# microsoft/SEAL

Hardware: AMD Instinct MI355X
Metric: CKKS multiply+relinearize+rescale ciphertexts/sec @ N=2^16, L=16 (higher is better)
Workload: dtype u64

## Files before the change

include/sealhip.h:

```cpp
#ifndef SEALHIP_H
#define SEALHIP_H

#include <stdbool.h>
#include <stddef.h>
#include <stdint.h>

#ifdef __cplusplus
extern "C" {
#endif

typedef long SHL_HRESULT;
#define SHL_S_OK ((SHL_HRESULT)0L)
#define SHL_S_FALSE ((SHL_HRESULT)1L)
#define SHL_E_POINTER ((SHL_HRESULT)0x80004003L)
#define SHL_E_INVALIDARG ((SHL_HRESULT)0x80070057L)
#define SHL_E_OUTOFMEMORY ((SHL_HRESULT)0x8007000EL)
#define SHL_E_UNEXPECTED ((SHL_HRESULT)0x8000FFFFL)
#define SHL_COR_E_IO ((SHL_HRESULT)0x80131620L)
#define SHL_COR_E_INVALIDOPERATION ((SHL_HRESULT)0x80131509L)
#define SHL_E_INVALID_INDEX ((SHL_HRESULT)0x80070585L)

#define SHL_FUNC SHL_HRESULT


// ... 217 lines not shown
SHL_FUNC Evaluator_ModReduceToNext(void *thisptr, void *encrypted, void *destination, void *pool);
SHL_FUNC Evaluator_ModReduceTo(void *thisptr, void *encrypted, uint64_t *parms_id, void *destination, void *pool);
SHL_FUNC Evaluator_TransformToNTT2(void *thisptr, void *encrypted, void *destination_ntt);
SHL_FUNC Evaluator_TransformFromNTT(void *thisptr, void *encrypted_ntt, void *destination);
SHL_FUNC Evaluator_ApplyGalois(void *thisptr, void *encrypted, uint32_t galois_elt, void *galoisKeys, void *destination, void *pool);
SHL_FUNC Evaluator_RotateRows(void *thisptr, void *encrypted, int steps, void *galoisKeys, void *destination, void *pool);
SHL_FUNC Evaluator_RotateColumns(void *thisptr, void *encrypted, void *galois_keys, void *destination, void *pool);
SHL_FUNC Evaluator_RotateVector(void *thisptr, void *encrypted, int steps, void *galoisKeys, void *destination, void *pool);
SHL_FUNC Evaluator_ComplexConjugate(void *thisptr, void *encrypted, void *galoisKeys, void *destination, void *pool);
SHL_FUNC Evaluator_ContextUsingKeyswitching(void *thisptr, bool *using_keyswitching);

SHL_FUNC Evaluator_SwitchKeyAccWords(void *thisptr, void *encrypted, uint64_t *words);
SHL_FUNC Evaluator_RelinearizePartial(void *thisptr, void *encrypted , void *relinKeys, uint64_t digit_first,
                                      uint64_t digit_count, uint64_t *device_acc);
SHL_FUNC Evaluator_RelinearizeFinish(void *thisptr, void *encrypted, uint64_t *device_acc, uint64_t parts);
SHL_FUNC Evaluator_ApplyGaloisPartial(void *thisptr, void *encrypted , uint32_t galois_elt, void *galoisKeys,
                                      uint64_t digit_first, uint64_t digit_count, uint64_t *device_acc);
SHL_FUNC Evaluator_ApplyGaloisFinish(void *thisptr, void *encrypted, uint64_t *device_acc, uint64_t parts);

SHL_FUNC Comm_GetUniqueId(uint8_t *id128);
SHL_FUNC Comm_RcclAvailable(bool *available);
SHL_FUNC Comm_Create(const uint8_t *id128, int nranks, int rank, void **comm);
SHL_FUNC Comm_Destroy(void *comm);
SHL_FUNC Comm_Info(void *comm, int *nranks, int *rank, bool *loopback);
SHL_FUNC Comm_DigitRange(void *comm, uint64_t digits, uint64_t *first, uint64_t *count);
SHL_FUNC Comm_AllReduceWords(void *comm, uint64_t *device_words, uint64_t count, void *hip_stream);
SHL_FUNC Comm_BroadcastWords(void *comm, uint64_t *device_words, uint64_t count, int root, void *hip_stream);
SHL_FUNC Evaluator_RelinearizeDigitParallel(void *thisptr, void *encrypted, void *relinKeys, void *comm, int exchange, void *destination);
SHL_FUNC Evaluator_ApplyGaloisDigitParallel(void *thisptr, void *encrypted, uint32_t galois_elt, void *galoisKeys, void *comm, int exchange,
                                            void *destination);
SHL_FUNC Evaluator_RotateVectorDigitParallel(void *thisptr, void *encrypted, int steps, void *galoisKeys, void *comm, int exchange,
                                             void *destination);
SHL_FUNC Evaluator_BroadcastKeyDigits(void *thisptr, void *kswitch_keys, uint64_t index, uint64_t *device_staging, void *comm, int root);
SHL_FUNC Evaluator_SwitchKeySlots(void *thisptr, void *encrypted, uint64_t nranks, uint64_t *slots);
SHL_FUNC Evaluator_SwitchKeyPackTargets(void *thisptr, void *encrypted, const uint64_t *device_acc, uint64_t nranks, uint64_t *device_send,
                                        uint64_t *device_special);
SHL_FUNC Evaluator_SwitchKeyFinishOwned(void *thisptr, void *encrypted, const uint64_t *device_recv, const uint64_t *device_special,
                                        uint64_t nranks, uint64_t rank, uint64_t *device_own);
SHL_FUNC Evaluator_SwitchKeyAddGathered(void *thisptr, void *encrypted, const uint64_t *device_all, uint64_t nranks);


SHL_FUNC shl_ntt_forward(void *context, uint64_t *data, uint64_t polys, uint64_t comps, uint64_t first_prime, int lazy, void *stream);
SHL_FUNC shl_ntt_inverse(void *context, uint64_t *data, uint64_t polys, uint64_t comps, uint64_t first_prime, int lazy, void *stream);
SHL_FUNC shl_dyadic_product(void *context, const uint64_t *a, const uint64_t *b, uint64_t *r, uint64_t polys, uint64_t comps, uint64_t first_prime, void *stream);
SHL_FUNC shl_reduce_items(void *context, uint64_t chain_index, const uint64_t *a, const uint64_t *plain, uint64_t *r, uint64_t size,
                          uint64_t batch, uint64_t group, uint64_t slices, uint64_t *scratch, uint64_t *slices_used, void *stream);
SHL_FUNC shl_reduce_flush_intervals(uint64_t *sum_terms, uint64_t *dot_terms);
SHL_FUNC shl_dot_items(void *context, uint64_t chain_index, const uint64_t *x, const uint64_t *y, uint64_t *r, uint64_t batch,
                       uint64_t group, uint64_t slices, uint64_t *scratch, uint64_t *slices_used, void *stream);
SHL_FUNC shl_dot_items_flush_interval(uint64_t *items);
SHL_FUNC shl_reduce_mapped(void *context, uint64_t chain_index, int kind, const uint64_t *a, uint64_t a_batch, const uint64_t *b,
                           uint64_t b_batch, uint64_t *r, uint64_t size, void *item_map, uint64_t slices, uint64_t *scratch,
                           uint64_t *slices_used, void *stream);
SHL_FUNC shl_dot_scalars(void *context, uint64_t chain_index, const uint64_t *a, const uint64_t *scalars, uint64_t *r, uint64_t size,
                         uint64_t rows, uint64_t batch, uint64_t slices, uint64_t *slices_used);
SHL_FUNC shl_dot_scalars_tile(void *context, uint64_t chain_index, const uint64_t *a, const uint64_t *scalars, uint64_t *r, uint64_t size,
                              uint64_t rows, uint64_t batch, uint64_t slices, uint64_t *slices_used, uint64_t row_tile, void *stream);
SHL_FUNC shl_dot_scalars_info(uint64_t *row_tile, uint64_t *flush);
SHL_FUNC shl_matmul_items(void *context, uint64_t chain_index, const uint64_t *x, const uint64_t *y, uint64_t *r, uint64_t rows, uint64_t inner,
                          uint64_t cols, int y_transposed, uint64_t slices, uint64_t *slices_used);
SHL_FUNC shl_matmul_items_tile(void *context, uint64_t chain_index, const uint64_t *x, const uint64_t *y, uint64_t *r, uint64_t rows,
                               uint64_t inner, uint64_t cols, int y_transposed, uint64_t slices, uint64_t *slices_used, uint64_t tile,
                               void *stream);
SHL_FUNC shl_matmul_items_info(uint64_t *tile_rows, uint64_t *tile_cols, uint64_t *flush);
SHL_FUNC shl_matmul_plain_items(void *context, uint64_t chain_index, const uint64_t *pl, const uint64_t *a, uint64_t *r, uint64_t size,
                                uint64_t rows, uint64_t inner, uint64_t cols, uint64_t flags, uint64_t slices, uint64_t *slices_used);
SHL_FUNC shl_matmul_plain_items_tile(void *context, uint64_t chain_index, const uint64_t *pl, const uint64_t *a, uint64_t *r, uint64_t size,
                                     uint64_t rows, uint64_t inner, uint64_t cols, uint64_t flags, uint64_t slices, uint64_t *slices_used,
                                     uint64_t tile, void *stream);
SHL_FUNC shl_matmul_plain_items_info(uint64_t *tile_rows, uint64_t *tile_cols, uint64_t *flush);
SHL_FUNC shl_matmul_scalars(void *context, uint64_t chain_index, const void *weights, const uint64_t *a, uint64_t *r, uint64_t size,
                            uint64_t rows, uint64_t inner, uint64_t cols, uint64_t flags, uint64_t slices, uint64_t *slices_used);
SHL_FUNC shl_matmul_scalars_tile(void *context, uint64_t chain_index, const void *weights, const uint64_t *a, uint64_t *r, uint64_t size,
                                 uint64_t rows, uint64_t inner, uint64_t cols, uint64_t flags, uint64_t slices, uint64_t *slices_used,
                                 uint64_t row_tile, void *stream);
SHL_FUNC shl_matmul_scalars_info(uint64_t *row_tile, uint64_t *narrow_row_tile, uint64_t *flush, uint64_t *narrow_flush);
SHL_FUNC shl_apply_galois(void *context, uint64_t chain_index, int ntt_form, uint32_t galois_elt, const uint64_t *in, uint64_t *out, uint64_t polys, void *stream);
SHL_FUNC shl_rns_stage(void *context, uint64_t chain_index, int which, const uint64_t *in, uint64_t *out, uint64_t polys, void *stream);
SHL_FUNC Ciphertext_Create4(void *context, uint64_t *parms_id, void *pool, void **cipher);
SHL_FUNC Ciphertext_Create5(void *context, uint64_t *parms_id, uint64_t capacity, void *pool, void **cipher);
SHL_FUNC Ciphertext_Reserve1(void *thisptr, void *context, uint64_t *parms_id, uint64_t size_capacity);
SHL_FUNC Ciphertext_Reserve2(void *thisptr, void *context, uint64_t size_capacity);
SHL_FUNC Ciphertext_Reserve3(void *thisptr, uint64_t size_capacity);
SHL_FUNC Ciphertext_SizeCapacity(void *thisptr, uint64_t *size_capacity);
SHL_FUNC Ciphertext_SetParmsId(void *thisptr, uint64_t *parms_id);
SHL_FUNC Ciphertext_Resize2(void *thisptr, void *context, uint64_t size);
SHL_FUNC Ciphertext_Resize3(void *thisptr, uint64_t size);
SHL_FUNC Ciphertext_Resize4(void *thisptr, uint64_t size, uint64_t polyModulusDegree, uint64_t coeffModCount);
SHL_FUNC Ciphertext_GetDataAt1(void *thisptr, uint64_t index, uint64_t *data);
SHL_FUNC Ciphertext_GetDataAt2(void *thisptr, uint64_t poly_index, uint64_t coeff_index, uint64_t *data);
SHL_FUNC Ciphertext_SetDataAt(void *thisptr, uint64_t index, uint64_t value);
SHL_FUNC Ciphertext_Release(void *thisptr);
SHL_FUNC KSwitchKeys_Create2(void *copy, void **kswitch_keys);
SHL_FUNC KSwitchKeys_Set(void *thisptr, void *assign);
SHL_FUNC KSwitchKeys_RawSize(void *thisptr, uint64_t *key_count);
SHL_FUNC KSwitchKeys_GetKeyList(void *thisptr, uint64_t index, uint64_t *count, void **key_list);
SHL_FUNC KSwitchKeys_ClearDataAndReserve(void *thisptr, uint64_t size);
SHL_FUNC KSwitchKeys_AddKeyList(void *thisptr, uint64_t count, void **key_list);
SHL_FUNC KSwitchKeys_GetParmsId(void *thisptr, uint64_t *parms_id);
SHL_FUNC KSwitchKeys_SetParmsId(void *thisptr, uint64_t *parms_id);
SHL_FUNC SEALContext_ParametersSet(void *thisptr, bool *params_set);
SHL_FUNC SEALContext_ParameterErrorName(void *thisptr, char *outstr, uint64_t *length);
SHL_FUNC SEALContext_ParameterErrorMessage(void *thisptr, char *outstr, uint64_t *length);
SHL_FUNC SEALContext_KeyContextData(void *thisptr, void **context_data);
SHL_FUNC SEALContext_FirstContextData(void *thisptr, void **context_data);
SHL_FUNC SEALContext_LastContextData(void *thisptr, void **context_data);
SHL_FUNC SEALContext_GetContextData(void *thisptr, uint64_t *parms_id, void **context_data);
SHL_FUNC ContextData_Destroy(void *thisptr);
SHL_FUNC ContextData_TotalCoeffModulus(void *thisptr, uint64_t *count, uint64_t *total_coeff_modulus);
SHL_FUNC ContextData_TotalCoeffModulusBitCount(void *thisptr, int *bit_count);
SHL_FUNC ContextData_Parms(void *thisptr, void **parms);
SHL_FUNC ContextData_Qualifiers(void *thisptr, void **epq);
SHL_FUNC ContextData_CoeffDivPlainModulus(void *thisptr, uint64_t *count, uint64_t *coeff_div);
SHL_FUNC ContextData_PlainUpperHalfThreshold(void *thisptr, uint64_t *puht);
SHL_FUNC ContextData_PlainUpperHalfIncrement(void *thisptr, uint64_t *count, uint64_t *puhi);
SHL_FUNC ContextData_UpperHalfThreshold(void *thisptr, uint64_t *count, uint64_t *uht);
SHL_FUNC ContextData_UpperHalfIncrement(void *thisptr, uint64_t *count, uint64_t *uhi);
SHL_FUNC ContextData_PrevContextData(void *thisptr, void **prev_data);
SHL_FUNC ContextData_NextContextData(void *thisptr, void **next_data);
SHL_FUNC ContextData_ChainIndex(void *thisptr, uint64_t *index);
SHL_FUNC ContextData_ParmsId(void *thisptr, uint64_t *parms_id);
SHL_FUNC EPQ_Destroy(void *thisptr);
SHL_FUNC EPQ_ParametersSet(void *thisptr, bool *parameters_set);
SHL_FUNC EPQ_UsingFFT(void *thisptr, bool *using_fft);
SHL_FUNC EPQ_UsingNTT(void *thisptr, bool *using_ntt);
SHL_FUNC EPQ_UsingBatching(void *thisptr, bool *using_batching);
SHL_FUNC EPQ_UsingFastPlainLift(void *thisptr, bool *using_fast_plain_lift);
SHL_FUNC EPQ_UsingDescendingModulusChain(void *thisptr, bool *using_descending_modulus_chain);
SHL_FUNC EPQ_SecLevel(void *thisptr, int *sec_level);
SHL_FUNC EncParams_Create2(void *copy, void **enc_params);
SHL_FUNC EncParams_Set(void *thisptr, void *assign);
SHL_FUNC EncParams_GetParmsId(void *thisptr, uint64_t *parms_id);
SHL_FUNC EncParams_GetPlainModulus(void *thisptr, uint64_t *plain_modulus);
SHL_FUNC EncParams_Equals(void *thisptr, void *otherptr, bool *result);
SHL_FUNC EncParams_SaveSize(void *thisptr, uint8_t compr_mode, int64_t *result);
SHL_FUNC EncParams_Save(void *thisptr, uint8_t *outptr, uint64_t size, uint8_t compr_mode, int64_t *out_bytes);
SHL_FUNC EncParams_Load(void *thisptr, uint8_t *inptr, uint64_t size, int64_t *in_bytes);
SHL_FUNC SecretKey_Create2(void *copy, void **secret_key);
SHL_FUNC SecretKey_Assign(void *thisptr, void *assign);
SHL_FUNC SecretKey_ParmsId(void *thisptr, uint64_t *parms_id);
SHL_FUNC SecretKey_SaveSize(void *thisptr, uint8_t compr_mode, int64_t *result);
SHL_FUNC SecretKey_Save(void *thisptr, uint8_t *outptr, uint64_t size, uint8_t compr_mode, int64_t *out_bytes);
SHL_FUNC PublicKey_Create2(void *copy, void **public_key);
SHL_FUNC PublicKey_Assign(void *thisptr, void *assign);
SHL_FUNC PublicKey_ParmsId(void *thisptr, uint64_t *parms_id);
SHL_FUNC PublicKey_SaveSize(void *thisptr, uint8_t compr_mode, int64_t *result);
SHL_FUNC PublicKey_Save(void *thisptr, uint8_t *outptr, uint64_t size, uint8_t compr_mode, int64_t *out_bytes);
SHL_FUNC SealHip_ReleasePool(void);
SHL_FUNC SealHip_SetStagedHostCopies(bool enabled);
SHL_FUNC SealHip_PoolStats(uint64_t *bytes_held, uint64_t *cross_stream_waits);
SHL_FUNC SealHip_InstallAbortTrace(const char *path);
SHL_FUNC SealHip_KsChunkStats(uint64_t *calls, uint64_t *chunks, uint64_t *scratch_bytes_max);
SHL_FUNC SealHip_TailStats(uint64_t *folded, uint64_t *plain, uint64_t *dropped);
SHL_FUNC SealHip_ProductStats(uint64_t *fused, uint64_t *formed, uint64_t *dropped);
SHL_FUNC SealHip_GaloisStats(uint64_t *gathered, uint64_t *permuted);
SHL_FUNC SealHip_XofStats(uint64_t *polynomials, uint64_t *replaced_words, uint64_t *host_walk_ns, uint64_t *total_ns);
SHL_FUNC shl_device_count(int *count);
SHL_FUNC shl_set_device(int device);
SHL_FUNC shl_stream_create(bool non_blocking, void **hip_stream);
SHL_FUNC shl_stream_destroy(void *hip_stream);
SHL_FUNC shl_malloc(uint64_t bytes, void **device_ptr);
SHL_FUNC shl_free(void *device_ptr);
SHL_FUNC shl_memcpy_h2d(void *device_dst, const void *host_src, uint64_t bytes);
SHL_FUNC KeyGenerator_Create1(void *context, const uint64_t *seed8, void **key_generator);
SHL_FUNC KeyGenerator_Create2(void *context, void *secret_key, const uint64_t *seed8, void **key_generator);
SHL_FUNC KeyGenerator_Destroy(void *thisptr);
SHL_FUNC KeyGenerator_SecretKey(void *thisptr, void *secret_key);
SHL_FUNC KeyGenerator_CreatePublicKey(void *thisptr, void *public_key);
SHL_FUNC KeyGenerator_CreateRelinKeys(void *thisptr, void *relin_keys);
SHL_FUNC KeyGenerator_CreateGaloisKeysFromElts(void *thisptr, uint64_t count, const uint32_t *galois_elts, void *galois_keys);
SHL_FUNC KeyGenerator_CreateGaloisKeysFromSteps(void *thisptr, uint64_t count, const int *steps, void *galois_keys);
SHL_FUNC KeyGenerator_CreateGaloisKeysAll(void *thisptr, void *galois_keys);
SHL_FUNC KeyGenerator_SeededSaveSize(void *thisptr, bool galois, uint64_t key_count, int64_t *result);
SHL_FUNC KeyGenerator_CreateRelinKeysSave(void *thisptr, uint8_t *outptr, uint64_t size, int64_t *out_bytes);
SHL_FUNC KeyGenerator_CreateGaloisKeysFromEltsSave(void *thisptr, uint64_t count, const uint32_t *galois_elts, uint8_t *outptr, uint64_t size,
                                                   int64_t *out_bytes);
SHL_FUNC KeyGenerator_KeyToHost(void *thisptr, uint32_t galois_elt, uint64_t *host_words, uint64_t capacity_words);
SHL_FUNC SecretKey_Get(void *thisptr, uint64_t *host_words);
SHL_FUNC PublicKey_Get(void *thisptr, uint64_t *host_words);
SHL_FUNC shl_memcpy_d2h(void *host_dst, const void *device_src, uint64_t bytes);
SHL_FUNC shl_device_synchronize(void);
SHL_FUNC shl_timer_create(void **timer);
SHL_FUNC shl_timer_destroy(void *timer);
SHL_FUNC shl_timer_start(void *timer, void *stream);
SHL_FUNC shl_timer_stop(void *timer, void *stream, float *milliseconds);

#ifdef __cplusplus
}
#endif
#endif
```

seal_amd/__init__.py:

```python
from .api import (CoeffModulus, PlainModulus, EncryptionParameters, SEALContext, ContextData, Ciphertext, Plaintext, KSwitchKeys,
                  RelinKeys, GaloisKeys, Evaluator, SecretKey, PublicKey, KeyGenerator, Decryptor, Encryptor, BatchEncoder, CKKSEncoder, Graph, ItemMap, DeviceBuffer, HipTimer, ntt_forward, ntt_inverse,
                  dyadic_product, apply_galois, rns_stage, device_synchronize, device_info, release_pool, pool_stats, tail_stats, product_stats, galois_stats, ks_chunk_stats, xof_stats, Stream, Comm, device_count, set_device,
                  set_staged_host_copies, install_abort_trace)
from ._native import SealHipError, InvalidArgument, LogicError, OutOfRange, DeviceError, load

__all__ = [
    "CoeffModulus", "PlainModulus", "EncryptionParameters", "SEALContext", "ContextData", "Ciphertext", "Plaintext", "KSwitchKeys",
    "RelinKeys", "GaloisKeys", "Evaluator", "SecretKey", "PublicKey", "KeyGenerator", "Decryptor", "Encryptor", "BatchEncoder", "CKKSEncoder", "Graph", "ItemMap", "DeviceBuffer", "HipTimer", "ntt_forward", "ntt_inverse",
    "dyadic_product", "apply_galois", "rns_stage", "device_synchronize", "device_info", "release_pool", "pool_stats", "tail_stats", "product_stats", "galois_stats", "ks_chunk_stats", "xof_stats", "Stream", "Comm", "device_count", "set_device", "set_staged_host_copies", "install_abort_trace", "SealHipError",
    "InvalidArgument", "LogicError", "OutOfRange", "DeviceError", "load",
]
```

seal_amd/_native.py:

```python
import ctypes as C
import os

_HERE = os.path.dirname(os.path.abspath(__file__))
DEFAULT_LIB = os.path.join(_HERE, "lib", "libsealhip.so")

S_OK = 0
E_POINTER = 0x80004003
E_INVALIDARG = 0x80070057
E_OUTOFMEMORY = 0x8007000E
E_UNEXPECTED = 0x8000FFFF
COR_E_IO = 0x80131620
COR_E_INVALIDOPERATION = 0x80131509
E_INVALID_INDEX = 0x80070585


class SealHipError(Exception):

    def __init__(self, hr, message):
        super().__init__("%s (HRESULT 0x%08X)" % (message, hr & 0xFFFFFFFF))
        self.hresult = hr & 0xFFFFFFFF
        self.message = message


class InvalidArgument(SealHipError, ValueError):
    pass


class LogicError(SealHipError, RuntimeError):
    pass


class OutOfRange(SealHipError, IndexError):
    pass


class DeviceError(SealHipError, OSError):
    pass


_ERR = {E_INVALIDARG: InvalidArgument, COR_E_INVALIDOPERATION: LogicError, E_INVALID_INDEX: OutOfRange,
        COR_E_IO: DeviceError}

SYMBOLS = """
SealHip_Version SealHip_DeviceInfo SealHip_LastError CoeffModulus_Create1 PlainModulus_Batching
EncParams_Create1 EncParams_Destroy EncParams_SetPolyModulusDegree EncParams_GetPolyModulusDegree
EncParams_SetCoeffModulus EncParams_GetCoeffModulus EncParams_SetPlainModulus2 EncParams_GetScheme
SEALContext_Create SEALContext_Destroy SEALContext_KeyParmsId SEALContext_FirstParmsId SEALContext_LastParmsId
SEALContext_UsingKeyswitching SEALContext_ChainIndex SEALContext_ParmsIdAt SEALContext_CoeffModulusAt
SEALContext_TotalCoeffModulusBitCount SEALContext_SetParmsId SEALContext_NTTRoot SEALContext_BaseBsk
Ciphertext_Create3 Ciphertext_CreateBatch Ciphertext_Create2 Ciphertext_Set Ciphertext_Destroy Ciphertext_Resize1
Ciphertext_Size Ciphertext_BatchCount Ciphertext_PolyModulusDegree Ciphertext_CoeffModulusSize Ciphertext_ParmsId
Ciphertext_IsNTTForm Ciphertext_SetIsNTTForm Ciphertext_Scale Ciphertext_SetScale Ciphertext_CorrectionFactor
Ciphertext_SetCorrectionFactor Ciphertext_IsTransparent Ciphertext_DevicePtr Ciphertext_CopyFromHost
Ciphertext_CopyToHost Ciphertext_CopyWordsToHost Ciphertext_CopyFromDevice
Ciphertext_SaveSize Ciphertext_Save Ciphertext_UnsafeLoad Ciphertext_Load Ciphertext_LoadItem Ciphertext_SaveItem
KSwitchKeys_UnsafeLoad KSwitchKeys_Load KSwitchKeys_SaveSize KSwitchKeys_Save
KeyGenerator_Create1 KeyGenerator_Create2 KeyGenerator_Destroy KeyGenerator_SecretKey KeyGenerator_CreatePublicKey
KeyGenerator_CreateRelinKeys KeyGenerator_CreateGaloisKeysFromSteps KeyGenerator_CreateGaloisKeysAll KeyGenerator_CreateGaloisKeysFromElts KeyGenerator_KeyToHost KeyGenerator_SeededSaveSize KeyGenerator_CreateRelinKeysSave KeyGenerator_CreateGaloisKeysFromEltsSave SecretKey_Get PublicKey_Get
SecretKey_Create SecretKey_Destroy SecretKey_Set SecretKey_UnsafeLoad SecretKey_Load Decryptor_Create Decryptor_Destroy
Decryptor_Decrypt Decryptor_InvariantNoiseBudget Decryptor_DecryptBatchWords Decryptor_DecryptBatch
CKKSEncoder_Create CKKSEncoder_Destroy CKKSEncoder_SlotCount CKKSEncoder_Encode1 CKKSEncoder_Encode2 CKKSEncoder_Encode3 CKKSEncoder_Encode4 CKKSEncoder_Encode5 CKKSEncoder_Decode1 CKKSEncoder_Decode2
CKKSEncoder_EncodeDevice CKKSEncoder_DecodeDevice
BatchEncoder_Create BatchEncoder_Destroy BatchEncoder_GetSlotCount BatchEncoder_Encode1 BatchEncoder_Encode2 BatchEncoder_Decode1
BatchEncoder_Decode2 BatchEncoder_EncodeDevice BatchEncoder_DecodeDevice
PublicKey_Create PublicKey_Destroy PublicKey_Set PublicKey_UnsafeLoad PublicKey_Load Encryptor_Encrypt Encryptor_EncryptZero1 Encryptor_EncryptZero2 Encryptor_EncryptZeroSymmetric2
Encryptor_Create Encryptor_Destroy Encryptor_SetSeed Encryptor_EncryptZeroSymmetric1 Encryptor_EncryptSymmetric
Encryptor_SymmetricSaveSize Encryptor_EncryptZeroSymmetricSave Encryptor_EncryptSymmetricSave
Encryptor_EncryptSymmetricDevice Encryptor_EncryptDevice
Plaintext_Create1 Plaintext_Create5 Plaintext_Destroy Plaintext_Set4 Plaintext_SetFromDevice Plaintext_CoeffCount
Plaintext_IsNTTForm Plaintext_GetParmsId Plaintext_SetParmsId Plaintext_Scale Plaintext_SetScale Plaintext_CopyToHost
Plaintext_SaveSize Plaintext_Save Plaintext_UnsafeLoad Plaintext_Load
Evaluator_AddMany Evaluator_AddPlain Evaluator_SubPlain Evaluator_MultiplyMany Evaluator_MultiplyPlain Evaluator_Exponentiate
Evaluator_TransformToNTT1 Evaluator_ModSwitchToNext2 Evaluator_ModSwitchTo2
Evaluator_AddPlainDevice Evaluator_SubPlainDevice Evaluator_MultiplyPlainDevice Evaluator_TransformPlainToNTTDevice
Evaluator_SumItems Evaluator_DotPlainDevice shl_reduce_items shl_reduce_flush_intervals
Evaluator_DotItems shl_dot_items shl_dot_items_flush_interval
ItemMap_Create ItemMap_Destroy ItemMap_Info Evaluator_SumItemsMapped Evaluator_DotPlainMapped Evaluator_DotItemsMapped shl_reduce_mapped
CKKSEncoder_EncodeScalars CKKSEncoder_EncodeIntegerScalars Evaluator_LiftScalars Evaluator_DotScalarsDevice
shl_dot_scalars shl_dot_scalars_tile shl_dot_scalars_info
Evaluator_MatMulItems shl_matmul_items shl_matmul_items_tile shl_matmul_items_info
Evaluator_MatMulPlainItems shl_matmul_plain_items shl_matmul_plain_items_tile shl_matmul_plain_items_info
Evaluator_MatMulScalarsItems shl_matmul_scalars shl_matmul_scalars_tile shl_matmul_scalars_info
KSwitchKeys_Create1 KSwitchKeys_Destroy KSwitchKeys_Size KSwitchKeys_SetKey KSwitchKeys_SetKeyFromDevice
KSwitchKeys_SetKeyDigits KSwitchKeys_HasKey KSwitchKeys_DeviceBytes RelinKeys_GetIndex GaloisKeys_GetIndex GaloisTool_GetEltFromStep
Evaluator_Create Evaluator_Destroy Evaluator_SetStream Evaluator_Synchronize Evaluator_CopyTo Evaluator_SetTransparentCheck
Evaluator_BeginCapture Evaluator_EndCapture Evaluator_LaunchGraph Graph_Destroy
Evaluator_Negate Evaluator_Add Evaluator_Sub Evaluator_Multiply Evaluator_Square Evaluator_Relinearize
Evaluator_ModSwitchToNext1 Evaluator_ModSwitchTo1 Evaluator_RescaleToNext Evaluator_RescaleTo
Evaluator_ModReduceToNext Evaluator_ModReduceTo Evaluator_TransformToNTT2 Evaluator_TransformFromNTT Evaluator_ApplyGalois
Evaluator_RotateRows Evaluator_RotateColumns Evaluator_RotateVector Evaluator_ComplexConjugate
Evaluator_ContextUsingKeyswitching
Evaluator_SwitchKeyAccWords Evaluator_RelinearizePartial Evaluator_RelinearizeFinish Evaluator_ApplyGaloisPartial
Evaluator_ApplyGaloisFinish
Comm_GetUniqueId Comm_RcclAvailable Comm_Create Comm_Destroy Comm_Info Comm_DigitRange Comm_AllReduceWords Comm_BroadcastWords
Evaluator_RelinearizeDigitParallel Evaluator_ApplyGaloisDigitParallel Evaluator_RotateVectorDigitParallel
Evaluator_BroadcastKeyDigits Evaluator_SwitchKeySlots Evaluator_SwitchKeyPackTargets Evaluator_SwitchKeyFinishOwned
Evaluator_SwitchKeyAddGathered
SealHip_ReleasePool SealHip_PoolStats SealHip_TailStats SealHip_ProductStats SealHip_GaloisStats SealHip_XofStats SealHip_KsChunkStats SealHip_SetStagedHostCopies SealHip_InstallAbortTrace shl_stream_create shl_stream_destroy shl_device_count shl_set_device
shl_ntt_forward shl_ntt_inverse shl_dyadic_product shl_apply_galois shl_rns_stage shl_malloc shl_free
shl_memcpy_h2d shl_memcpy_d2h shl_device_synchronize shl_timer_create shl_timer_destroy shl_timer_start
shl_timer_stop
Ciphertext_Create4 Ciphertext_Create5 Ciphertext_GetDataAt1 Ciphertext_GetDataAt2 Ciphertext_Release Ciphertext_Reserve1
Ciphertext_Reserve2 Ciphertext_Reserve3 Ciphertext_Resize2 Ciphertext_Resize3 Ciphertext_Resize4 Ciphertext_SetDataAt
Ciphertext_SetParmsId Ciphertext_SizeCapacity ContextData_ChainIndex ContextData_CoeffDivPlainModulus ContextData_Destroy ContextData_NextContextData
ContextData_Parms ContextData_ParmsId ContextData_PlainUpperHalfIncrement ContextData_PlainUpperHalfThreshold ContextData_PrevContextData ContextData_Qualifiers
ContextData_TotalCoeffModulus ContextData_TotalCoeffModulusBitCount ContextData_UpperHalfIncrement ContextData_UpperHalfThreshold EPQ_Destroy EPQ_ParametersSet
EPQ_SecLevel EPQ_UsingBatching EPQ_UsingDescendingModulusChain EPQ_UsingFFT EPQ_UsingFastPlainLift EPQ_UsingNTT
EncParams_Create2 EncParams_Equals EncParams_GetParmsId EncParams_GetPlainModulus EncParams_Load EncParams_Save
EncParams_SaveSize EncParams_Set KSwitchKeys_AddKeyList KSwitchKeys_ClearDataAndReserve KSwitchKeys_Create2 KSwitchKeys_GetKeyList
KSwitchKeys_GetParmsId KSwitchKeys_RawSize KSwitchKeys_Set KSwitchKeys_SetParmsId PublicKey_Assign PublicKey_Create2
PublicKey_ParmsId PublicKey_Save PublicKey_SaveSize SEALContext_FirstContextData SEALContext_GetContextData SEALContext_KeyContextData
SEALContext_LastContextData SEALContext_ParameterErrorMessage SEALContext_ParameterErrorName SEALContext_ParametersSet SecretKey_Assign SecretKey_Create2
SecretKey_ParmsId SecretKey_Save SecretKey_SaveSize
""".split()

_lib = None
_lib_path = None


def load(path=None):
    global _lib, _lib_path
    want = os.path.abspath(path or DEFAULT_LIB)
    if _lib is not None and _lib_path == want:
        return _lib
    if not os.path.exists(want):
        raise ImportError(
            "seal_amd: %s not found. Build it with `python -c 'import __graft_entry__ as g; g.build()'` "
            "(hipcc --offload-arch=gfx950). There is no CPU fallback." % want)
    lib = C.CDLL(want)
    for name in SYMBOLS:
        getattr(lib, name).restype = C.c_long
    _lib, _lib_path = lib, want
    return lib


def lib():
    return _lib if _lib is not None else load()


def check(hr):
    hr &= 0xFFFFFFFF
    if hr == S_OK:
        return
    n = C.c_uint64(0)
    lib().SealHip_LastError(None, C.byref(n))
    buf = C.create_string_buffer(max(int(n.value), 1))
    lib().SealHip_LastError(buf, C.byref(n))
    cls = _ERR.get(hr, SealHipError)
    if hr == E_OUTOFMEMORY:
        raise MemoryError(buf.value.decode())
    raise cls(hr, buf.value.decode(errors="replace"))
```

seal_amd/api.py:

```python
import ctypes as C
import os

import numpy as np

from . import _native as N

SCHEME = {"none": 0, "bfv": 1, "ckks": 2, "bgv": 3}


def _p(a):
    return a.ctypes.data_as(C.c_void_p)


class CoeffModulus:
    @staticmethod
    def Create(poly_modulus_degree, bit_sizes):
        bits = (C.c_int * len(bit_sizes))(*bit_sizes)
        out = np.zeros(len(bit_sizes), dtype=np.uint64)
        N.check(N.lib().CoeffModulus_Create1(C.c_uint64(poly_modulus_degree), C.c_uint64(len(bit_sizes)), bits, _p(out)))
        return [int(x) for x in out]


class PlainModulus:
    @staticmethod
# ... 1582 lines not shown

    def __del__(self):
        if getattr(self, "_h", None):
            N.lib().Comm_Destroy(self._h)
            self._h = None

    def loopback(self):
        v = C.c_bool()
        N.check(N.lib().Comm_Info(self._h, None, None, C.byref(v)))
        return v.value

    def digit_range(self, digits):
        a, b = C.c_uint64(), C.c_uint64()
        N.check(N.lib().Comm_DigitRange(self._h, C.c_uint64(digits), C.byref(a), C.byref(b)))
        return a.value, b.value

    def all_reduce(self, device_ptr, words, stream=None):
        N.check(N.lib().Comm_AllReduceWords(self._h, C.c_void_p(device_ptr), C.c_uint64(words), C.c_void_p(stream or 0)))

    def broadcast(self, device_ptr, words, root=0, stream=None):
        N.check(N.lib().Comm_BroadcastWords(self._h, C.c_void_p(device_ptr), C.c_uint64(words), C.c_int(root), C.c_void_p(stream or 0)))


class DeviceBuffer:

    def __init__(self, words):
        self.words = int(words)
        self._ptr = C.c_void_p()
        N.check(N.lib().shl_malloc(C.c_uint64(self.words * 8), C.byref(self._ptr)))

    def __del__(self):
        if getattr(self, "_ptr", None) and self._ptr.value:
            N.lib().shl_free(self._ptr)
            self._ptr = None

    @property
    def ptr(self):
        return self._ptr.value

    @staticmethod
    def from_numpy(a):
        a = np.ascontiguousarray(a, dtype=np.uint64)
        b = DeviceBuffer(a.size)
        N.check(N.lib().shl_memcpy_h2d(b._ptr, _p(a), C.c_uint64(a.size * 8)))
        return b

    def to_numpy(self, shape):
        out = np.zeros(shape, dtype=np.uint64)
        N.check(N.lib().shl_memcpy_d2h(_p(out), self._ptr, C.c_uint64(out.size * 8)))
        return out

    @staticmethod
    def from_array(a):
        a = np.ascontiguousarray(a)
        if a.dtype.itemsize not in (8, 16):
            raise TypeError("from_array takes 8-byte or complex128 elements, not %s" % a.dtype)
        b = DeviceBuffer(max(a.nbytes // 8, 1))
        N.check(N.lib().shl_memcpy_h2d(b._ptr, _p(a), C.c_uint64(a.nbytes)))
        return b

    @staticmethod
    def from_int32(a):
        a = np.ascontiguousarray(a, dtype=np.int32)
        b = DeviceBuffer(max((a.size + 1) // 2, 1))
        N.check(N.lib().shl_memcpy_h2d(b._ptr, _p(a), C.c_uint64(a.nbytes)))
        return b

    def to_array(self, shape, dtype=np.float64):
        out = np.zeros(shape, dtype=dtype)
        N.check(N.lib().shl_memcpy_d2h(_p(out), self._ptr, C.c_uint64(out.nbytes)))
        return out


def ntt_forward(context, buf, polys, comps, first_prime=0, lazy=False, stream=None):
    N.check(N.lib().shl_ntt_forward(context._h, C.c_void_p(buf.ptr), C.c_uint64(polys), C.c_uint64(comps),
                                    C.c_uint64(first_prime), C.c_int(int(lazy)), C.c_void_p(stream or 0)))


def ntt_inverse(context, buf, polys, comps, first_prime=0, lazy=False, stream=None):
    N.check(N.lib().shl_ntt_inverse(context._h, C.c_void_p(buf.ptr), C.c_uint64(polys), C.c_uint64(comps),
                                    C.c_uint64(first_prime), C.c_int(int(lazy)), C.c_void_p(stream or 0)))


def dyadic_product(context, a, b, r, polys, comps, first_prime=0, stream=None):
    N.check(N.lib().shl_dyadic_product(context._h, C.c_void_p(a.ptr), C.c_void_p(b.ptr), C.c_void_p(r.ptr),
                                       C.c_uint64(polys), C.c_uint64(comps), C.c_uint64(first_prime),
                                       C.c_void_p(stream or 0)))


def apply_galois(context, chain_index, ntt_form, galois_elt, src, dst, polys, stream=None):
    N.check(N.lib().shl_apply_galois(context._h, C.c_uint64(chain_index), C.c_int(int(ntt_form)), C.c_uint32(galois_elt),
                                     C.c_void_p(src.ptr), C.c_void_p(dst.ptr), C.c_uint64(polys), C.c_void_p(stream or 0)))


RNS_STAGE = {"fastbconv_m_tilde": 0, "sm_mrq": 1, "fast_floor": 2, "fastbconv_sk": 3,
             "divide_and_round_q_last": 4, "divide_and_round_q_last_ntt": 5}


def rns_stage(context, chain_index, which, src, dst, polys, stream=None):
    N.check(N.lib().shl_rns_stage(context._h, C.c_uint64(chain_index), C.c_int(RNS_STAGE[which]), C.c_void_p(src.ptr),
                                  C.c_void_p(dst.ptr), C.c_uint64(polys), C.c_void_p(stream or 0)))


class Stream:

    def __init__(self, non_blocking=True):
        self._h = C.c_void_p()
        N.check(N.lib().shl_stream_create(C.c_bool(non_blocking), C.byref(self._h)))

    @property
    def handle(self):
        return self._h.value

    def __del__(self):
        if getattr(self, "_h", None) and self._h.value:
            N.lib().shl_stream_destroy(self._h)
            self._h = None


def device_count():
    n = C.c_int()
    N.check(N.lib().shl_device_count(C.byref(n)))
    return n.value


def set_device(index):
    N.check(N.lib().shl_set_device(C.c_int(index)))


def release_pool():
    N.check(N.lib().SealHip_ReleasePool())


def set_staged_host_copies(enabled):
    N.check(N.lib().SealHip_SetStagedHostCopies(C.c_bool(enabled)))


def install_abort_trace(path):
    N.check(N.lib().SealHip_InstallAbortTrace(C.c_char_p(os.fsencode(path))))


def pool_stats():
    a, b = C.c_uint64(), C.c_uint64()
    N.check(N.lib().SealHip_PoolStats(C.byref(a), C.byref(b)))
    return a.value, b.value


def tail_stats():
    a, b, c = C.c_uint64(), C.c_uint64(), C.c_uint64()
    N.check(N.lib().SealHip_TailStats(C.byref(a), C.byref(b), C.byref(c)))
    return a.value, b.value, c.value


def product_stats():
    a, b, c = C.c_uint64(), C.c_uint64(), C.c_uint64()
    N.check(N.lib().SealHip_ProductStats(C.byref(a), C.byref(b), C.byref(c)))
    return a.value, b.value, c.value


def galois_stats():
    a, b = C.c_uint64(), C.c_uint64()
    N.check(N.lib().SealHip_GaloisStats(C.byref(a), C.byref(b)))
    return a.value, b.value


def xof_stats():
    v = [C.c_uint64() for _ in range(4)]
    N.check(N.lib().SealHip_XofStats(*[C.byref(x) for x in v]))
    return tuple(x.value for x in v)


def ks_chunk_stats():
    a, b, c = C.c_uint64(), C.c_uint64(), C.c_uint64()
    N.check(N.lib().SealHip_KsChunkStats(C.byref(a), C.byref(b), C.byref(c)))
    return a.value, b.value, c.value


def device_synchronize():
    N.check(N.lib().shl_device_synchronize())


def device_info():
    name = C.create_string_buffer(256)
    cus = C.c_int()
    mem = C.c_uint64()
    N.check(N.lib().SealHip_DeviceInfo(name, C.c_uint64(256), C.byref(cus), C.byref(mem)))
    return name.value.decode(), cus.value, mem.value


class HipTimer:

    def __init__(self):
        self._h = C.c_void_p()
        N.check(N.lib().shl_timer_create(C.byref(self._h)))

    def __del__(self):
        if getattr(self, "_h", None):
            N.lib().shl_timer_destroy(self._h)
            self._h = None

    def start(self, stream=None):
        N.check(N.lib().shl_timer_start(self._h, C.c_void_p(stream or 0)))

    def stop(self, stream=None):
        ms = C.c_float()
        N.check(N.lib().shl_timer_stop(self._h, C.c_void_p(stream or 0), C.byref(ms)))
        return ms.value
```

seal_amd/csrc/capi_kernels.cpp:

```cpp
#include "capi_common.h"
#include "batch_reduce_kernels.h"
#include <memory>

namespace
{
    template <class Launch>
    SHL_HRESULT raw_reduce(void *context, uint64_t chain_index, const char *shape_error, uint64_t grid_planes, uint64_t out_items,
                           const ItemWalk &walk, uint64_t slices, uint64_t *slices_used, const uint64_t *r, bool operands,
                           const uint64_t *scratch, Launch launch)
    {
        IfNullRet(context, SHL_E_POINTER);
        SHL_TRY
        auto c = as<Context>(context);
        auto l = c->level_by_chain_index(chain_index);
        if (!l)
            throw std::out_of_range("chain_index");
        if (shape_error)
            throw std::invalid_argument(shape_error);
        const size_t words = (size_t)l->K * c->n();
        if (!slices)
            slices = batch_reduce_slices(grid_planes * out_items * words / 2, walk);
        if (slices > walk.longest || slices > 64)
            throw std::invalid_argument("1 <= slices <= min(group or longest row, 64)");
        if (slices_used)
// ... 374 lines not shown
    }
    SHL_FUNC shl_apply_galois(
        void *context, uint64_t chain_index, int ntt_form, uint32_t galois_elt, const uint64_t *in, uint64_t *out, uint64_t polys,
        void *stream)
    {
        IfNullRet(context, SHL_E_POINTER);
        IfNullRet(in, SHL_E_POINTER);
        IfNullRet(out, SHL_E_POINTER);
        SHL_TRY
        auto c = as<Context>(context);
        auto l = c->level_by_chain_index(chain_index);
        if (!l)
            throw std::out_of_range("chain_index");
        if (!(galois_elt & 1) || galois_elt >= 2 * c->n())
            throw std::invalid_argument("Galois element is not valid");
        if (in == out)
            throw std::invalid_argument("result cannot point to the same value as operand");
        PlaneGeom g{ (unsigned)c->log_n(), l->K, (unsigned)polys };
        hip_ok(k_apply_galois(c->dev_mods(), in, out, galois_elt, ntt_form, g, 1, (hipStream_t)stream), "apply_galois");
        SHL_CATCH
    }
    SHL_FUNC shl_rns_stage(void *context, uint64_t chain_index, int which, const uint64_t *in, uint64_t *out, uint64_t polys, void *stream)
    {
        IfNullRet(context, SHL_E_POINTER);
        IfNullRet(in, SHL_E_POINTER);
        IfNullRet(out, SHL_E_POINTER);
        SHL_TRY
        auto c = as<Context>(context);
        auto l = c->level_by_chain_index(chain_index);
        if (!l)
            throw std::out_of_range("chain_index");
        hipStream_t s = (hipStream_t)stream;
        const unsigned n_log = (unsigned)c->log_n();
        if (which >= 0 && which <= 3)
        {
            if (c->scheme() != Scheme::bfv)
                throw std::logic_error("BEHZ stages exist only for BFV contexts");
            hip_ok(k_behz_stage(c->dev_mods(), l->dev, which, in, out, n_log, polys, s), "behz stage");
        }
        else if (which == 4)
        {
            if (l->K < 2)
                throw std::invalid_argument("level has a single modulus");
            hip_ok(k_bfv_modswitch(c->dev_mods(), l->dev, in, out, n_log, polys, s), "divide_and_round_q_last");
        }
        else if (which == 5)
        {
            if (l->K < 2)
                throw std::invalid_argument("level has a single modulus");
            const unsigned K = l->K;
            const size_t N = c->n();
            Scratch copy(polys * K * N), tt(polys * (K - 1) * N);
            hip_ok(hipMemcpyAsync(copy.p, in, polys * K * N * 8, hipMemcpyDeviceToDevice, s), "copy");
            uint64_t *last = copy.p + (size_t)(K - 1) * N;
            NttBatch bi{};
            bi.data = last;
            bi.outer_stride = (size_t)K * N;
            bi.ncomp = 1;
            bi.nouter = (unsigned)polys;
            bi.prime_first = K - 1;
            hip_ok(ntt_inverse(c->ntt_tables(), bi, 0, s), "intt last");
            NttBatch b{};
            b.data = tt.p;
            b.outer_stride = (size_t)(K - 1) * N;
            b.ncomp = K - 1;
            b.nouter = (unsigned)polys;
            b.src = last;
            b.src_outer_stride = (size_t)K * N;
            b.src_ncomp = 1;
            b.src_mode = 2;
            b.src_half = l->dev.half_q_last;
            b.src_q = l->dev.q_last;
            b.src_fix = l->dev.round_fix;
            hip_ok(ntt_forward(c->ntt_tables(), b, 1, s), "ntt correction");
            hip_ok(k_rescale_combine(c->dev_mods(), l->dev.inv_q_last_mod_q, copy.p, tt.p, out, n_log, K, polys, s), "combine");
            hip_ok(hipStreamSynchronize(s), "sync");
        }
        else
            throw std::invalid_argument("unknown stage");
        SHL_CATCH
    }
    SHL_FUNC SealHip_SetStagedHostCopies(bool enabled)
    {
        set_staged_host_copies(enabled);
        return SHL_S_OK;
    }
    SHL_FUNC SealHip_ReleasePool(void)
    {
        SHL_TRY
        DevicePool::global().release_all();
        SHL_CATCH
    }
    SHL_FUNC SealHip_PoolStats(uint64_t *bytes_held, uint64_t *cross_stream_waits)
    {
        SHL_TRY
        if (bytes_held)
            *bytes_held = DevicePool::global().bytes_held();
        if (cross_stream_waits)
            *cross_stream_waits = DevicePool::global().cross_stream_waits();
        SHL_CATCH
    }
    SHL_FUNC SealHip_KsChunkStats(uint64_t *calls, uint64_t *chunks, uint64_t *scratch_bytes_max)
    {
        SHL_TRY
        uint64_t w = 0;
        ks_chunk_stats(calls, chunks, &w);
        if (scratch_bytes_max)
            *scratch_bytes_max = w * 8;
        SHL_CATCH
    }
    SHL_FUNC SealHip_XofStats(uint64_t *polynomials, uint64_t *replaced_words, uint64_t *host_walk_ns, uint64_t *total_ns)
    {
        SHL_TRY
        xof_stats(polynomials, replaced_words, host_walk_ns, total_ns);
        SHL_CATCH
    }
    SHL_FUNC SealHip_ProductStats(uint64_t *fused, uint64_t *formed, uint64_t *dropped)
    {
        SHL_TRY
        uint64_t f, p, d;
        lazy_product_stats(f, p, d);
        if (fused)
            *fused = f;
        if (formed)
            *formed = p;
        if (dropped)
            *dropped = d;
        SHL_CATCH
    }
    SHL_FUNC SealHip_GaloisStats(uint64_t *gathered, uint64_t *permuted)
    {
        SHL_TRY
        uint64_t g, p;
        galois_path_stats(g, p);
        if (gathered)
            *gathered = g;
        if (permuted)
            *permuted = p;
        SHL_CATCH
    }
    SHL_FUNC SealHip_TailStats(uint64_t *folded, uint64_t *plain, uint64_t *dropped)
    {
        SHL_TRY
        uint64_t f, p, d;
        lazy_tail_stats(f, p, d);
        if (folded)
            *folded = f;
        if (plain)
            *plain = p;
        if (dropped)
            *dropped = d;
        SHL_CATCH
    }
    SHL_FUNC shl_device_count(int *count)
    {
        IfNullRet(count, SHL_E_POINTER);
        SHL_TRY
        *count = 0;
        if (hipGetDeviceCount(count) != hipSuccess)
            *count = 0;
        SHL_CATCH
    }
    SHL_FUNC shl_set_device(int device)
    {
        SHL_TRY
        hip_ok(hipSetDevice(device), "hipSetDevice");
        SHL_CATCH
    }
    SHL_FUNC shl_stream_create(bool non_blocking, void **hip_stream)
    {
        IfNullRet(hip_stream, SHL_E_POINTER);
        SHL_TRY
        hipStream_t s = nullptr;
        hip_ok(hipStreamCreateWithFlags(&s, non_blocking ? hipStreamNonBlocking : hipStreamDefault), "hipStreamCreateWithFlags");
        *hip_stream = s;
        SHL_CATCH
    }
    SHL_FUNC shl_stream_destroy(void *hip_stream)
    {
        SHL_TRY
        hip_ok(hipStreamSynchronize((hipStream_t)hip_stream), "hipStreamSynchronize");
        hip_ok(hipStreamDestroy((hipStream_t)hip_stream), "hipStreamDestroy");
        SHL_CATCH
    }
    SHL_FUNC shl_malloc(uint64_t bytes, void **device_ptr)
    {
        IfNullRet(device_ptr, SHL_E_POINTER);
        SHL_TRY
        if (hipMalloc(device_ptr, bytes) != hipSuccess)
            throw std::bad_alloc();
        SHL_CATCH
    }
    SHL_FUNC shl_free(void *device_ptr)
    {
        SHL_TRY
        hip_ok(hipFree(device_ptr), "hipFree");
        SHL_CATCH
    }
    SHL_FUNC shl_memcpy_h2d(void *device_dst, const void *host_src, uint64_t bytes)
    {
        SHL_TRY
        hip_ok(hipMemcpy(device_dst, host_src, bytes, hipMemcpyHostToDevice), "H2D");
        SHL_CATCH
    }
    SHL_FUNC shl_memcpy_d2h(void *host_dst, const void *device_src, uint64_t bytes)
    {
        SHL_TRY
        hip_ok(hipDeviceSynchronize(), "sync");
        hip_ok(hipMemcpy(host_dst, device_src, bytes, hipMemcpyDeviceToHost), "D2H");
        SHL_CATCH
    }
    SHL_FUNC shl_device_synchronize(void)
    {
        SHL_TRY
        hip_ok(hipDeviceSynchronize(), "hipDeviceSynchronize");
        SHL_CATCH
    }
    SHL_FUNC shl_timer_create(void **timer)
    {
        IfNullRet(timer, SHL_E_POINTER);
        SHL_TRY
        auto t = new Timer();
        hip_ok(hipEventCreate(&t->e0), "hipEventCreate");
        hip_ok(hipEventCreate(&t->e1), "hipEventCreate");
        *timer = t;
        SHL_CATCH
    }
    SHL_FUNC shl_timer_destroy(void *timer)
    {
        IfNullRet(timer, SHL_E_POINTER);
        auto t = as<Timer>(timer);
        (void)hipEventDestroy(t->e0);
        (void)hipEventDestroy(t->e1);
        delete t;
        return SHL_S_OK;
    }
    SHL_FUNC shl_timer_start(void *timer, void *stream)
    {
        IfNullRet(timer, SHL_E_POINTER);
        SHL_TRY
        hip_ok(hipEventRecord(as<Timer>(timer)->e0, (hipStream_t)stream), "hipEventRecord");
        SHL_CATCH
    }
    SHL_FUNC shl_timer_stop(void *timer, void *stream, float *milliseconds)
    {
        IfNullRet(timer, SHL_E_POINTER);
        IfNullRet(milliseconds, SHL_E_POINTER);
        SHL_TRY
        auto t = as<Timer>(timer);
        hip_ok(hipEventRecord(t->e1, (hipStream_t)stream), "hipEventRecord");
        hip_ok(hipEventSynchronize(t->e1), "hipEventSynchronize");
        hip_ok(hipEventElapsedTime(milliseconds, t->e0, t->e1), "hipEventElapsedTime");
        SHL_CATCH
    }
}
```

seal_amd/csrc/ntt2_device.h:

```cpp
#pragma once
#include "ntt2_kernels.h"
#include <cstdlib>
#include <type_traits>

#ifndef SEALHIP_FP_WAVES_P1
#define SEALHIP_FP_WAVES_P1 4
#endif
#ifndef SEALHIP_FP_WAVES_P2
#define SEALHIP_FP_WAVES_P2 4
#endif

namespace sealhip
{
    namespace
    {
        constexpr int kThreads = 256;
        constexpr unsigned kMaxKeyComps = 64;
#ifndef SEALHIP_KS_NT
#define SEALHIP_KS_NT 31
#endif
#ifndef SEALHIP_PRIO
#define SEALHIP_PRIO 0
#endif
        template <int WHEN>
        __device__ __forceinline__ void prio_phase()
        {
#if defined(__HIP_DEVICE_COMPILE__)
            if constexpr (SEALHIP_PRIO != 0)
                __builtin_amdgcn_s_setprio(SEALHIP_PRIO == WHEN ? 1 : 0);
#endif
        }
        template <int BIT>
        __device__ __forceinline__ uint64_t mid_ld(const uint64_t *p)
        {
#if defined(__HIP_DEVICE_COMPILE__)
            if constexpr ((SEALHIP_KS_NT & BIT) != 0)
                return __builtin_nontemporal_load(p);
#endif
            return *p;
        }
        template <int BIT>
        __device__ __forceinline__ void mid_st(uint64_t *p, uint64_t v)
        {
#if defined(__HIP_DEVICE_COMPILE__)
            if constexpr ((SEALHIP_KS_NT & BIT) != 0)
            {
                __builtin_nontemporal_store(v, p);
                return;
            }
#endif
            *p = v;
        }
        template <int BIT>
        __device__ __forceinline__ void mid_ld2(const uint64_t *p, uint64_t &a, uint64_t &b)
        {
#if defined(__HIP_DEVICE_COMPILE__)
            typedef uint64_t u64x2 __attribute__((ext_vector_type(2)));
            const u64x2 *q = reinterpret_cast<const u64x2 *>(p);
            const u64x2 v = (SEALHIP_KS_NT & BIT) != 0 ? __builtin_nontemporal_load(q) : *q;
            a = v.x;
            b = v.y;
#else
            a = p[0];
            b = p[1];
#endif
        }
        template <int BIT>
        __device__ __forceinline__ void mid_st2(uint64_t *p, uint64_t a, uint64_t b)
        {
#if defined(__HIP_DEVICE_COMPILE__)
            typedef uint64_t u64x2 __attribute__((ext_vector_type(2)));
            u64x2 *q = reinterpret_cast<u64x2 *>(p);
            const u64x2 v = { a, b };
            if constexpr ((SEALHIP_KS_NT & BIT) != 0)
                __builtin_nontemporal_store(v, q);
            else
                *q = v;
#else
            p[0] = a;
            p[1] = b;
#endif
        }
#ifdef SEALHIP_MID_WAVE_MAJOR
        __device__ __forceinline__ unsigned mid_lane(unsigned tid) { return (tid >> 6) * 1024 + (tid & 63); }
        constexpr unsigned kMidRow = 64;
#else
        __device__ __forceinline__ unsigned mid_lane(unsigned tid) { return tid; }
        constexpr unsigned kMidRow = 256;
#endif
        template <int D1>
        struct Geo
        {
            static constexpr int rA = D1 - 4;
            static constexpr int LC = 12 - D1;
            static constexpr int C = 1 << LC;
            static constexpr int CP = C + (C == 16 ? 1 : 0);
            static constexpr int ROWS = 1 << D1;
            static constexpr int TILES = 1 << (D1 - 4);
            static constexpr int n = D1 + 8;
            static constexpr size_t lds1_words = (size_t)ROWS * CP;
        };
        constexpr int kRowWords = 16 * 18;
        constexpr size_t kLds2Words = 16 * kRowWords;

        constexpr unsigned kPackWords = 13, kPackBlock = kPackWords * 16;
#ifndef SEALHIP_PACK_VEC16
#define SEALHIP_PACK_VEC16 1
#endif
        constexpr double kPackMagic = 6755399441055744.0;
        constexpr unsigned kPackLdsRow = 272;
        __device__ __forceinline__ void pack52(const double (&x)[16], uint64_t (&w)[13])
        {
            uint32_t lo[16], hi[16];
#pragma unroll
            for (int r = 0; r < 16; r++)
            {
                const uint64_t b = fp_to_bits(x[r] + kPackMagic);
                lo[r] = (uint32_t)b;
                hi[r] = (uint32_t)(b >> 32) & 0xFFFFFu;
            }
#pragma unroll
            for (int k = 0; k < 8; k++)
                w[k] = (uint64_t)lo[2 * k] | ((uint64_t)lo[2 * k + 1] << 32);
#pragma unroll
            for (int k = 0; k < 4; k++)
            {
                const uint32_t d0 = (hi[4 * k] & 0xFFFFu) | (hi[4 * k + 1] << 16), d1 = (hi[4 * k + 2] & 0xFFFFu) | (hi[4 * k + 3] << 16);
                w[8 + k] = (uint64_t)d0 | ((uint64_t)d1 << 32);
            }
            uint32_t t0 = 0, t1 = 0;
#pragma unroll
            for (int r = 0; r < 8; r++)
            {
                t0 |= (hi[r] >> 16) << (4 * r);
                t1 |= (hi[r + 8] >> 16) << (4 * r);
            }
            w[12] = (uint64_t)t0 | ((uint64_t)t1 << 32);
        }
        __device__ __forceinline__ void unpack52(const uint64_t (&w)[13], double (&x)[16])
        {
#pragma unroll
            for (int r = 0; r < 16; r++)
            {
                const uint32_t lo = (uint32_t)(w[r >> 1] >> (32 * (r & 1)));
                const uint32_t mid = (uint32_t)(w[8 + (r >> 2)] >> (16 * (r & 3))) & 0xFFFFu;
                const uint32_t top = (uint32_t)(w[12] >> (4 * r)) & 0xFu;
                const uint64_t b = (uint64_t)lo | ((uint64_t)(0x43300000u | (top << 16) | mid) << 32);
                x[r] = fp_from_bits(b) - kPackMagic;
            }
        }

        __device__ __forceinline__ int int_class(const NttTables &t, unsigned prime)
        {
            const uint64_t q = SHL_UCONST(reinterpret_cast<const uint64_t *>(&t.mods[prime]))[0];
            return (q >> 60) ? 2 : (q >> 58) ? 0 : 1;
        }
        template <class Body>
        __device__ __forceinline__ void with_int_class(const NttTables &t, unsigned prime, Body body)
        {
            const int c = int_class(t, prime);
            if (c == 0)
                body(std::integral_constant<int, 0>());
            else if (c == 1)
                body(std::integral_constant<int, 1>());
            else
                body(std::integral_constant<int, 2>());
        }
#ifndef SEALHIP_XCD_SPREAD
#define SEALHIP_XCD_SPREAD 0
#endif
        struct Blk
        {
            unsigned tile, y, z;
        };
        __device__ __forceinline__ Blk spread_blocks()
        {
#if SEALHIP_XCD_SPREAD
            const unsigned tiles = gridDim.x, slots = gridDim.y * gridDim.z;
            const unsigned L = blockIdx.x + tiles * (blockIdx.y + gridDim.y * blockIdx.z);
            const unsigned group = 8 * tiles, full = (slots / 8) * group;
            unsigned tile, slot;
            if (L < full)
            {
                const unsigned x = L & 7, r = L >> 3;
                tile = r % tiles;
                slot = (r / tiles) * 8 + x;
            }
            else
            {
                tile = L % tiles;
                slot = L / tiles;
            }
            return Blk{ tile, slot % gridDim.y, slot / gridDim.y };
#else
            return Blk{ blockIdx.x, blockIdx.y, blockIdx.z };
#endif
        }

        template <bool FP>
        __device__ __forceinline__ const typename Field<FP>::tw_t *tw_table(const NttTables &t, bool inverse, unsigned prime)
        {
            if constexpr (FP)
                return (inverse ? t.inv_d : t.fwd_d) + ((size_t)prime << t.log_n);
            else
                return (inverse ? t.inv : t.fwd) + ((size_t)prime << t.log_n);
        }

        template <int ICLS>
        __device__ __forceinline__ void int_fix_all(uint64_t (&x)[16], const Field<false>::Mod &m)
        {
#pragma unroll
            for (int a = 0; a < 16; a++)
                Field<false>::fix4<IntBounds<ICLS>::hi32>(x[a], m);
        }

        template <bool FP, int BIT, int ICLS = 0, int B = 4, class TwFn>
        __device__ __forceinline__ void stage_fwd(typename Field<FP>::elem (&x)[16], const typename Field<FP>::Mod &m, TwFn tw)
        {
            if constexpr (!FP)
            {
                if constexpr (IntBounds<ICLS>::fwd_fix_before(B))
                    int_fix_all<ICLS>(x, m);
            }
#pragma unroll
            for (int g = 0; g < (8 >> BIT); g++)
            {
                const auto w = tw(g);
#pragma unroll
                for (int k = 0; k < (1 << BIT); k++)
                {
                    const int e0 = (g << (BIT + 1)) | k;
                    if constexpr (!FP && ICLS == 2)
                        Field<FP>::bfly_fwd_guarded(x[e0], x[e0 | (1 << BIT)], w, m);
                    else
                        Field<FP>::bfly_fwd(x[e0], x[e0 | (1 << BIT)], w, m);
                }
            }
        }

        template <bool FP, int R, int ICLS = 0, int B = 4, class TwFn>
        __device__ __forceinline__ void phase_fwd(typename Field<FP>::elem (&x)[16], const typename Field<FP>::Mod &m, TwFn tw)
        {
            typedef IntBounds<ICLS> IB;
            if constexpr (R >= 1)
                stage_fwd<FP, 3, ICLS, B>(x, m, [&](int g) { return tw(0, g); });
            if constexpr (R >= 2)
                stage_fwd<FP, 2, ICLS, IB::fwd_after(B, 1)>(x, m, [&](int g) { return tw(1, g); });
            if constexpr (R >= 3)
                stage_fwd<FP, 1, ICLS, IB::fwd_after(B, 2)>(x, m, [&](int g) { return tw(2, g); });
            if constexpr (R >= 4)
                stage_fwd<FP, 0, ICLS, IB::fwd_after(B, 3)>(x, m, [&](int g) { return tw(3, g); });
        }

        template <bool FP, int R, bool FIX, int ICLS = 0, int B = 4, class TwFn>
        __device__ __forceinline__ void phase_fwd_end(typename Field<FP>::elem (&x)[16], const typename Field<FP>::Mod &m, TwFn tw)
        {
            phase_fwd<FP, R, ICLS, B>(x, m, tw);
            if constexpr (FP && FIX)
            {
#pragma unroll
                for (int a = 0; a < 16; a++)
                    Field<FP>::fix(x[a], m);
            }
        }
        template <bool FP, int ICLS, int B>
        __device__ __forceinline__ uint64_t fwd_out_lazy(typename Field<FP>::elem x, const typename Field<FP>::Mod &m)
        {
            if constexpr (!FP && B > 4)
                Field<FP>::template fix4<IntBounds<ICLS>::hi32>(x, m);
            return Field<FP>::fwd_to_lazy(x, m);
        }
        template <bool FP, int ICLS, int B>
        __device__ __forceinline__ uint64_t fwd_out_canon(typename Field<FP>::elem x, const typename Field<FP>::Mod &m)
        {
            if constexpr (!FP && ICLS != 2)
                return Field<FP>::template canon_any<IntBounds<ICLS>::hi32>(x, m);
            else
                return Field<FP>::fwd_to_canon(x, m);
        }
        template <int ICLS, int D1>
        constexpr int kP1Out = IntBounds<ICLS>::fwd_after(4, D1);
        template <int ICLS, int D1>
        constexpr int kP2Out = IntBounds<ICLS>::fwd_after(kP1Out<ICLS, D1>, 8);

        template <bool FP, int R, int FIXAT, class TwFn>
        __device__ __forceinline__ void phase_fwd_fix(typename Field<FP>::elem (&x)[16], const typename Field<FP>::Mod &m, TwFn tw)
        {
            static_assert(FP && R == 4 && FIXAT >= 1 && FIXAT <= 3, "a four-stage double-precision phase with the fix inside it");
            stage_fwd<FP, 3>(x, m, [&](int g) { return tw(0, g); });
            if constexpr (FIXAT == 1)
            {
#pragma unroll
                for (int a = 0; a < 16; a++)
                    Field<FP>::fix(x[a], m);
            }
            stage_fwd<FP, 2>(x, m, [&](int g) { return tw(1, g); });
            if constexpr (FIXAT == 2)
            {
#pragma unroll
                for (int a = 0; a < 16; a++)
                    Field<FP>::fix(x[a], m);
            }
// ... 481 lines not shown
```

seal_amd/csrc/ntt2_kernels.h:

```cpp
#pragma once
#include "ntt_kernels.h"

namespace sealhip
{
    bool ntt2_supports(int log_n);

    size_t ntt2_ring_words(const NttTables &t, const NttBatch &b);
    hipError_t ntt2_forward(const NttTables &t, const NttBatch &b, int out_lazy, uint64_t *mid, hipStream_t stream, uint64_t *ring = nullptr, size_t ring_words = 0);

    struct NttRingRun
    {
        uint64_t *data;
        size_t outer_stride;
        const uint32_t *comp_prime;
        unsigned prime_first, ncomp, c0, nc, nouter;
        int lazy;
        unsigned teams_per_comp;
        uint64_t *ring;
        size_t ring_words;
    };
    unsigned ntt2_ring_teams(unsigned nc, unsigned nouter);
    size_t ntt2_ring_run_words(unsigned nc, unsigned teams_per_comp);
    bool ntt2_ring_stream_ok(hipStream_t stream);
    hipError_t ntt2_ring_launch(const NttTables &t, const NttRingRun &run, hipStream_t stream);

    hipError_t ntt2_inverse(const NttTables &t, const NttBatch &b, int out_lazy, uint64_t *mid, hipStream_t stream);

    struct KsFusedArgs
    {
        const uint64_t *t;
        const uint64_t *target_ntt;
        const uint64_t *key;
        uint64_t *mid;
        uint64_t *acc;
        const uint32_t *targets1, *targets2;
        unsigned ntargets, n_int;
        unsigned K, L, batch;
        unsigned j0, j1, key_digit0;
        unsigned parts;
        const uint64_t *fold_c0 = nullptr, *fold_c1 = nullptr;
        const ShoupOp *fold_pm = nullptr;
        const uint64_t *fold_x = nullptr, *fold_y = nullptr;
        size_t fold_plane = 0;
        uint32_t galois_elt = 0;
        int order1 = -1;
        bool no_class_fork = false;
    };
    hipError_t ks_fused(const NttTables &t, const KsFusedArgs &k, hipStream_t stream);

    inline unsigned key_comp_units(const NttTables &t, unsigned comp)
    {
        return t.fp_host && t.fp_host[comp] ? 2u : 4u;
    }
    inline unsigned key_comp_offset_units(const NttTables &t, unsigned comp)
    {
        unsigned u = 0;
        for (unsigned c = 0; c < comp; c++)
            u += key_comp_units(t, c);
        return u;
    }
    inline unsigned key_digit_units(const NttTables &t, unsigned L)
    {
        return key_comp_offset_units(t, L);
    }
    inline size_t key_register_order_words(const NttTables &t, unsigned L, size_t digits)
    {
        return (digits * key_digit_units(t, L)) << t.log_n;
    }
    hipError_t key_to_register_order(const NttTables &t, const uint64_t *in, uint64_t *out, unsigned L, size_t digits, hipStream_t stream);
    hipError_t key_from_register_order(const NttTables &t, const uint64_t *in, uint64_t *out, unsigned L, size_t digits, hipStream_t stream);
}
```

seal_amd/csrc/ntt2_kernels.hip:

```cpp
#include "ntt2_device.h"
#include <algorithm>
#include <atomic>
#include <cstdio>
#include <mutex>
#include <cstdlib>
#include <type_traits>
#include <vector>



namespace sealhip
{
    namespace
    {

        template <bool FP, int D1, int ICLS = 0, bool PACK = false>
        __device__ __forceinline__ void fwd_p1_body(const FwdArgs &a, unsigned prime, unsigned comp, unsigned outer, uint64_t *lds, unsigned tile)
        {
            typedef Field<FP> F;
            typedef Geo<D1> G;
            const unsigned tid = threadIdx.x, cg = tile;
            const typename F::Mod m = F::make_mod(ld_uniform_mod(&a.t.mods[prime]), ld_uniform_fpd(&a.t.fpd[prime]));
            const typename F::tw_t *tab = tw_table<FP>(a.t, false, prime);
            SrcMap sm{ 0, 0, 0, 0 };
// ... 146 lines not shown
                    lds[r * kPackLdsRow + tid] = fp_to_bits(y[r]);
                __syncthreads();
#pragma unroll
                for (int e = 0; e < 16; e++)
                    x[e] = fp_from_bits(lds[(tid >> 4) * kPackLdsRow + e * 16 + (tid & 15)]);
                __syncthreads();
            }
            else
            {
#pragma unroll
            for (int e = 0; e < 16; e++)
                x[e] = F::unraw(nxt[e]);
            prio_phase<2>();
            if (outer + ostride < a.nouter)
                fetch(outer + ostride);
            prio_phase<1>();
            }
            if constexpr (HOIST_LDS)
                p2_tile<FP, D1, false, false, true, true>(x, m, tab, twa, nullptr, lds_wave, hg, tid, &pre_a, &pre_b);
            else if constexpr (HOIST)
                p2_tile<FP, D1, false, false, true>(x, m, tab, nullptr, nullptr, lds_wave, hg, tid, &pre_a, &pre_b);
            else
                p2_tile<FP, D1, false, false, false, false, false, ICLS, kP1Out<ICLS, D1>>(x, m, tab, nullptr, nullptr, lds_wave, hg, tid);
            constexpr int BOUT = kP2Out<ICLS, D1>;
            uint64_t val[16];
            const size_t row0 = ((size_t)comp << G::n) + ((size_t)(hg * 16 + (tid >> 6) * 4) << 8);
            if ((HOIST || HOIST_LDS) || a.epi == 0)
            {
#pragma unroll
                for (int e = 0; e < 16; e++)
                    val[e] = a.lazy ? fwd_out_lazy<FP, ICLS, BOUT>(x[e], m) : fwd_out_canon<FP, ICLS, BOUT>(x[e], m);
                store_rows(val, lds_wave, a.data + (size_t)outer * a.outer_stride + row0, tid);
            }
            else
            {
#pragma unroll
                for (int e = 0; e < 16; e++)
                    val[e] = fwd_out_lazy<FP, ICLS, BOUT>(x[e], m);
                const uint64_t q = a.t.mods[prime].q;
                const ShoupOp mul = a.epi_mul[comp];
                const uint64_t *A = a.epi_a + (size_t)outer * a.epi_a_stride + row0;
                if (a.epi == 1)
                {
                    uint64_t *O = a.epi_out0 + (size_t)outer * a.epi_out_stride + row0;
                    emit_rows(val, lds_wave, tid, [&](unsigned off, uint64_t tv) { O[off] = mul_shoup(A[off] + 4 * q - tv, mul.w, mul.wq, q); });
                }
                else if (a.epi == 3)
                {
                    uint64_t *O = ((outer & 1) ? a.epi_out1 : a.epi_out0) + (size_t)(outer >> 1) * a.epi_out_stride + row0;
                    emit_rows(val, lds_wave, tid, [&](unsigned off, uint64_t tv) {
                        O[off] = sub_mod(mid_ld<16>(A + off), mul_shoup(tv, mul.w, mul.wq, q), q);
                    });
                }
                else
                {
                    uint64_t *O = ((outer & 1) ? a.epi_out1 : a.epi_out0) + (size_t)(outer >> 1) * a.epi_out_stride + row0;
                    emit_rows(val, lds_wave, tid, [&](unsigned off, uint64_t tv) {
                        O[off] = add_mod(O[off], mul_shoup(A[off] + 4 * q - tv, mul.w, mul.wq, q), q);
                    });
                }
            }
            }
        }

        template <int D1, int CLS>
        __global__ void __launch_bounds__(kThreads, (CLS == 1 || CLS == 4 || CLS == 5) ? SEALHIP_FP_WAVES_P2 : 2) ntt2_fwd_p2(FwdArgs a)
        {
            HIP_DYNAMIC_SHARED(uint64_t, lds)
            const Blk blk = spread_blocks();
            const unsigned comp = blk.y + a.comp0, outer = blk.z;
            const unsigned prime = SHL_UNIFORM(a.comp_prime ? a.comp_prime[comp] : a.prime_first + comp);
            if constexpr (CLS == 5)
                fwd_p2_body<true, D1, false, true, 0, D1 == 8>(a, prime, comp, outer, lds, blk.tile);
            else if constexpr (CLS == 4)
                fwd_p2_body<true, D1, false, true>(a, prime, comp, outer, lds, blk.tile);
            else if constexpr (CLS == 3)
                fwd_p2_body<true, D1, true>(a, prime, comp, outer, lds, blk.tile);
            else if constexpr (CLS == 1)
                fwd_p2_body<true, D1>(a, prime, comp, outer, lds, blk.tile);
            else if constexpr (CLS == 0)
                with_int_class(a.t, prime, [&](auto ic) { fwd_p2_body<false, D1, false, false, decltype(ic)::value>(a, prime, comp, outer, lds, blk.tile); });
            else if (a.t.fpd[prime].qi)
                fwd_p2_body<true, D1>(a, prime, comp, outer, lds, blk.tile);
            else
                fwd_p2_body<false, D1, false, false, 2>(a, prime, comp, outer, lds, blk.tile);
        }

        struct Tail2Args
        {
            FwdArgs f;
            NttTail2 x;
        };

        template <bool FP, int D1, int ICLS>
        __device__ __forceinline__ void tail2_p1_body(const Tail2Args &t2, unsigned prime, unsigned comp, unsigned outer, uint64_t *lds, unsigned tile)
        {
            typedef Field<FP> F;
            typedef Geo<D1> G;
            const FwdArgs &a = t2.f;
            const unsigned tid = threadIdx.x, cg = tile;
            const typename F::Mod m = F::make_mod(ld_uniform_mod(&a.t.mods[prime]), ld_uniform_fpd(&a.t.fpd[prime]));
            const typename F::tw_t *tab = tw_table<FP>(a.t, false, prime);
            const int mode = t2.x.halves_added ? 3 : 2;
            const SrcMap s1{ mode, a.src_half, a.src_q, a.src_fix[comp] }, s2{ mode, t2.x.src2_half, t2.x.src2_q, t2.x.src2_fix[comp] };
            const ShoupOp pm = t2.x.pmul[comp];
            const uint64_t q = a.t.mods[prime].q;
            const unsigned c = tid & (G::C - 1), rbl = tid >> G::LC;
            const size_t col = (size_t)cg * G::C + c;
            TwRegs<FP> tw;
            p1_load_tw<FP, D1>(tw, tab, tid);
            const unsigned ostride = gridDim.z;
            for (; outer < a.nouter; outer += ostride)
            {
                const uint64_t *in1 = a.src + (size_t)outer * a.src_outer_stride + col;
                const uint64_t *in2 = ((outer & 1) ? t2.x.src2_1 : t2.x.src2_0) + (size_t)(outer >> 1) * t2.x.src2_stride + col;
                uint64_t n1[16], n2[16];
#pragma unroll
                for (int e = 0; e < 16; e++)
                {
                    const unsigned ra = e >> (4 - G::rA), rbh = e & ((1 << (4 - G::rA)) - 1);
                    const unsigned R = ra * 16 + (rbh << G::rA) + rbl;
                    n1[e] = in1[(size_t)R * 256];
                    n2[e] = in2[(size_t)R * 256];
                }
                typename F::elem x[16];
                if constexpr (FP)
                {
                    const double pinv = pm.w > q / 2 ? -(double)(q - pm.w) : (double)pm.w;
                    const double f1 = fp_from_u52(s1.fix), f2 = fp_from_u52(s2.fix);
                    const bool u_small = !(s2.src_q >> 52);
#pragma unroll
                    for (int e = 0; e < 16; e++)
                    {
                        const uint64_t r1 = mode == 3 ? n1[e] : csub(n1[e] + s1.half, s1.src_q), r2 = mode == 3 ? n2[e] : csub(n2[e] + s2.half, s2.src_q);
                        const double v = F::from_any(r1, m) + f1, u = (u_small ? fp_from_u52(r2) : F::from_any(r2, m)) + f2;
                        x[e] = fp_mulmod(v, pinv, m.q, m.qinv) + u;
                        F::fix(x[e], m);
                    }
                }
                else
                {
#pragma unroll
                    for (int e = 0; e < 16; e++)
                    {
                        const typename F::elem v = map_src<FP>(n1[e], s1, m), u = map_src<FP>(n2[e], s2, m);
                        x[e] = mul_shoup(v, pm.w, pm.wq, q) + u;
                    }
                }
                uint64_t *mid_tr = a.mid + (((size_t)outer * a.ncomp + comp) << G::n);
                p1_tile<FP, D1, 256, FP && G::rA == 4, ICLS>(x, m, tab, tw, lds, mid_tr, cg, tid);
            }
        }

        template <bool FP, int D1, int ICLS>
        __device__ __forceinline__ void tail2_p2_body(const Tail2Args &t2, unsigned prime, unsigned comp, unsigned outer, uint64_t *lds, unsigned tile)
        {
            typedef Field<FP> F;
            typedef Geo<D1> G;
            const FwdArgs &a = t2.f;
            const unsigned tid = threadIdx.x, hg = tile;
            const typename F::Mod m = F::make_mod(ld_uniform_mod(&a.t.mods[prime]), ld_uniform_fpd(&a.t.fpd[prime]));
            const typename F::tw_t *tab = tw_table<FP>(a.t, false, prime);
            const uint64_t *mid0 = a.mid + ((size_t)comp << G::n) + ((size_t)hg << 12) + mid_lane(tid);
            uint64_t *lds_wave = lds + (tid >> 6) * (4 * kRowWords);
            const uint64_t q = a.t.mods[prime].q;
            const ShoupOp mul = a.epi_mul[comp], pm = t2.x.pmul[comp];
            [[maybe_unused]] const double pm_fp = pm.w > q / 2 ? -(double)(q - pm.w) : (double)pm.w;
            [[maybe_unused]] const double mul_fp = mul.w > q / 2 ? -(double)(q - mul.w) : (double)mul.w;
            const size_t row0 = ((size_t)comp << G::n) + ((size_t)(hg * 16 + (tid >> 6) * 4) << 8);
            uint64_t nxt[16];
            auto fetch = [&](unsigned z) {
                const uint64_t *mp = mid0 + (((size_t)z * a.ncomp) << G::n);
#pragma unroll
                for (int e = 0; e < 16; e++)
                    nxt[e] = mid_ld<4>(mp + e * kMidRow);
            };
            const unsigned ostride = gridDim.z;
            fetch(outer);
            for (; outer < a.nouter; outer += ostride)
            {
                typename F::elem x[16];
#pragma unroll
                for (int e = 0; e < 16; e++)
                    x[e] = F::unraw(nxt[e]);
                if (outer + ostride < a.nouter)
                    fetch(outer + ostride);
                const uint64_t *A = a.epi_a + (size_t)outer * a.epi_a_stride + row0;
                const uint64_t *C = ((outer & 1) ? t2.x.c1 : t2.x.c0) + (size_t)(outer >> 1) * t2.x.c_stride + row0;
                const bool folded = t2.x.a_has_c;
                uint64_t av[16], cv[16];
#pragma unroll
                for (int k = 0; k < 16; k++)
                {
                    const unsigned off = (k >> 2) * 256 + (k & 3) * 64 + (tid & 63);
                    av[k] = mid_ld<16>(A + off);
                    cv[k] = folded ? 0 : mid_ld<16>(C + off);
                }
                p2_tile<FP, D1, false, false, false, false, false, ICLS, kP1Out<ICLS, D1>>(x, m, tab, nullptr, nullptr, lds_wave, hg, tid);
                uint64_t val[16];
                uint64_t *O = ((outer & 1) ? a.epi_out1 : a.epi_out0) + (size_t)(outer >> 1) * a.epi_out_stride + row0;
                if constexpr (FP)
                {
#pragma unroll
                    for (int e = 0; e < 16; e++)
                        val[e] = F::raw(x[e]);
                    emit_rows_k(val, lds_wave, tid, [&](int k, unsigned off, uint64_t tv) {
                        const double s = folded ? fp_from_u52(av[k]) : fp_mulmod(fp_from_u52(av[k]), pm_fp, m.q, m.qinv) + fp_from_u52(cv[k]);
                        const double r = fp_mulmod(s - fp_from_bits(tv), mul_fp, m.q, m.qinv);
                        O[off] = fp_to_canon(fp_fix(r, m.q, m.qinv), m);
                    });
                }
                else
                {
#pragma unroll
                    for (int e = 0; e < 16; e++)
                        val[e] = fwd_out_lazy<FP, ICLS, kP2Out<ICLS, D1>>(x[e], m);
                    emit_rows_k(val, lds_wave, tid, [&](int k, unsigned off, uint64_t tv) {
                        const uint64_t s = folded ? av[k] : add_mod(mul_shoup(av[k], pm.w, pm.wq, q), cv[k], q);
                        O[off] = mul_shoup(s + 4 * q - tv, mul.w, mul.wq, q);
                    });
                }
            }
        }

        template <int D1, int CLS>
        __global__ void __launch_bounds__(kThreads, 2) ntt2_tail2_p1(Tail2Args a)
        {
            HIP_DYNAMIC_SHARED(uint64_t, lds)
            const Blk blk = spread_blocks();
            const unsigned comp = blk.y + a.f.comp0, outer = blk.z;
            const unsigned prime = SHL_UNIFORM(a.f.prime_first + comp);
            if constexpr (CLS == 1)
                tail2_p1_body<true, D1, 0>(a, prime, comp, outer, lds, blk.tile);
            else if constexpr (CLS == 0)
                with_int_class(a.f.t, prime, [&](auto ic) { tail2_p1_body<false, D1, decltype(ic)::value>(a, prime, comp, outer, lds, blk.tile); });
            else if (a.f.t.fpd[prime].qi)
                tail2_p1_body<true, D1, 0>(a, prime, comp, outer, lds, blk.tile);
            else
                tail2_p1_body<false, D1, 2>(a, prime, comp, outer, lds, blk.tile);
        }
        template <int D1, int CLS>
        __global__ void __launch_bounds__(kThreads, 2) ntt2_tail2_p2(Tail2Args a)
        {
            HIP_DYNAMIC_SHARED(uint64_t, lds)
            const Blk blk = spread_blocks();
            const unsigned comp = blk.y + a.f.comp0, outer = blk.z;
            const unsigned prime = SHL_UNIFORM(a.f.prime_first + comp);
            if constexpr (CLS == 1)
                tail2_p2_body<true, D1, 0>(a, prime, comp, outer, lds, blk.tile);
            else if constexpr (CLS == 0)
                with_int_class(a.f.t, prime, [&](auto ic) { tail2_p2_body<false, D1, decltype(ic)::value>(a, prime, comp, outer, lds, blk.tile); });
            else if (a.f.t.fpd[prime].qi)
                tail2_p2_body<true, D1, 0>(a, prime, comp, outer, lds, blk.tile);
            else
                tail2_p2_body<false, D1, 2>(a, prime, comp, outer, lds, blk.tile);
        }

        __device__ __forceinline__ uint64_t resident_word(uint64_t v)
        {
#if defined(__HIP_DEVICE_COMPILE__)
            asm volatile("" : "+v"(v));
#endif
            return v;
        }

        template <bool FP, int D1, bool TWO, bool SMALL2>
        __device__ __forceinline__ void src_p1t_body(const Tail2Args &t2, unsigned nc, uint64_t *lds)
        {
            static_assert(!SMALL2 || (FP && TWO), "SMALL2 is a property of the double-precision launch of the folded tail");
            typedef Field<FP> F;
            typedef Geo<D1> G;
            const FwdArgs &a = t2.f;
            const unsigned tid = threadIdx.x;
            const unsigned grp = blockIdx.x;
            if (grp >= a.nouter * G::TILES)
                return;
            const unsigned cg = grp % G::TILES, outer = grp / G::TILES;
            const unsigned c = tid & (G::C - 1), rbl = tid >> G::LC;
            const size_t col = (size_t)cg * G::C + c;
            const uint64_t *in1 = a.src + (size_t)outer * a.src_outer_stride + col;
            [[maybe_unused]] const uint64_t *in2 = nullptr;
            if constexpr (TWO)
                in2 = ((outer & 1) ? t2.x.src2_1 : t2.x.src2_0) + (size_t)(outer >> 1) * t2.x.src2_stride + col;
            uint64_t r1[16];
            [[maybe_unused]] uint64_t r2[16];
#pragma unroll
            for (int e = 0; e < 16; e++)
            {
                const unsigned ra = e >> (4 - G::rA), rbh = e & ((1 << (4 - G::rA)) - 1);
                const unsigned R = ra * 16 + (rbh << G::rA) + rbl;
                r1[e] = in1[(size_t)R * 256];
                if constexpr (TWO)
                    r2[e] = in2[(size_t)R * 256];
            }
            const bool add_half = TWO ? !t2.x.halves_added : a.src_mode == 2;
            if (add_half)
            {
#pragma unroll
                for (int e = 0; e < 16; e++)
                {
                    r1[e] = csub(r1[e] + a.src_half, a.src_q);
                    if constexpr (TWO)
                        r2[e] = csub(r2[e] + t2.x.src2_half, t2.x.src2_q);
                }
            }
            if constexpr (SMALL2)
            {
#pragma unroll
                for (int e = 0; e < 16; e++)
                    r2[e] = fp_to_bits(fp_from_u52(r2[e]));
            }
#pragma nounroll
            for (unsigned it = 0; it < nc; it++)
            {
                const unsigned comp = a.comp0 + it;
                const unsigned prime = SHL_UNIFORM(a.comp_prime ? a.comp_prime[comp] : a.prime_first + comp);
                uint64_t *mid_tr = a.mid + (((size_t)outer * a.ncomp + comp) << G::n);
                auto one = [&](auto ic) {
                    constexpr int ICLS = decltype(ic)::value;
                    const typename F::Mod m = F::make_mod(ld_uniform_mod(&a.t.mods[prime]), ld_uniform_fpd(&a.t.fpd[prime]));
                    const typename F::tw_t *tab = tw_table<FP>(a.t, false, prime);
                    TwRegs<FP> tw;
                    p1_load_tw<FP, D1>(tw, tab, tid);
                    const SrcMap s1{ 3, 0, 0, a.src_fix[comp] };
                    typename F::elem x[16];
                    if constexpr (!TWO)
                    {
#pragma unroll
                        for (int e = 0; e < 16; e++)
                            x[e] = map_src<FP>(resident_word(r1[e]), s1, m);
                        p1_tile<FP, D1, 256, SEALHIP_P1_PLAIN_LEAN && FP && G::rA == 4, ICLS>(x, m, tab, tw, lds, mid_tr, cg, tid);
                    }
                    else
                    {
                        const ShoupOp pm = t2.x.pmul[comp];
                        const uint64_t q = a.t.mods[prime].q;
                        if constexpr (FP)
                        {
                            const double pinv = pm.w > q / 2 ? -(double)(q - pm.w) : (double)pm.w;
                            const double f1 = fp_from_u52(s1.fix), f2 = fp_from_u52(t2.x.src2_fix[comp]);
#pragma unroll
                            for (int e = 0; e < 16; e++)
                            {
                                const double v = F::from_any(resident_word(r1[e]), m) + f1;
                                const double u = (SMALL2 ? fp_from_bits(r2[e]) : F::from_any(resident_word(r2[e]), m)) + f2;
                                x[e] = fp_mulmod(v, pinv, m.q, m.qinv) + u;
                                F::fix(x[e], m);
                            }
                        }
                        else
                        {
                            const SrcMap s2{ 3, 0, 0, t2.x.src2_fix[comp] };
#pragma unroll
                            for (int e = 0; e < 16; e++)
                            {
                                const typename F::elem v = map_src<FP>(resident_word(r1[e]), s1, m), u = map_src<FP>(resident_word(r2[e]), s2, m);
                                x[e] = mul_shoup(v, pm.w, pm.wq, q) + u;
                            }
                        }
                        p1_tile<FP, D1, 256, FP && G::rA == 4, ICLS>(x, m, tab, tw, lds, mid_tr, cg, tid);
                    }
                };
                if constexpr (FP)
                    one(std::integral_constant<int, 0>());
                else
                    with_int_class(a.t, prime, one);
            }
        }

#ifndef SEALHIP_SRC_P1T_FP2_WGS
#define SEALHIP_SRC_P1T_FP2_WGS 2
#endif
        template <int D1, int CLS, bool TWO, bool SMALL2 = false>
        __global__ void __launch_bounds__(kThreads, SMALL2 ? SEALHIP_SRC_P1T_FP2_WGS : 2) ntt2_src_p1t(Tail2Args a, unsigned nc)
        {
            static_assert(CLS == 0 || CLS == 1, "single-class runs only");
            HIP_DYNAMIC_SHARED(uint64_t, lds)
            src_p1t_body<CLS == 1, D1, TWO, SMALL2>(a, nc, lds);
        }

        struct InvArgs
        {
            uint64_t *data;
            size_t outer_stride;
            const uint64_t *src;
            size_t src_outer_stride;
            uint64_t *mid;
            const uint32_t *comp_prime;
            int cls_hint;
            unsigned prime_first;
            unsigned ncomp;
            unsigned comp0;
            unsigned nouter;
            int lazy;
            uint64_t out_add;
            const uint64_t *prod_x, *prod_y;
            unsigned prod_batch, prod_outer0;
            uint64_t *prod_out;
            size_t prod_out_stride;
            uint32_t src_gal;
            NttTables t;
        };

        template <int ICLS>
        constexpr int kInvE1 = inv_phase_exp<ICLS>(0, 4, 0);
        template <int ICLS>
        constexpr int kInvE2 = inv_phase_exp<ICLS>(kInvE1<ICLS>, 4, 0);
        template <int ICLS>
        constexpr int kInvE3 = inv_phase_exp<ICLS>(kInvE2<ICLS>, 4, 0);

        template <bool FP, int D1, int ICLS = 2>
        __device__ __forceinline__ void inv_pa_body(const InvArgs &a, unsigned prime, unsigned comp, unsigned outer, uint64_t *lds, unsigned tile)
        {
            typedef Field<FP> F;
            typedef Geo<D1> G;
            const unsigned tid = threadIdx.x, hg = tile;
            const unsigned v = tid & 15, u = tid >> 4, ul = u & 3;
            const unsigned h = hg * 16 + u;
            const typename F::Mod m = F::make_mod(ld_uniform_mod(&a.t.mods[prime]), ld_uniform_fpd(&a.t.fpd[prime]));
            const typename F::tw_t *tab = tw_table<FP>(a.t, true, prime);
            uint64_t *lds_wave = lds + (tid >> 6) * (4 * kRowWords);
            uint64_t raw[16];
            typename F::elem x[16];
            bool have_x = false;
            const size_t rows = ((size_t)comp << G::n) + ((size_t)(hg * 16 + (tid >> 6) * 4) << 8);
            if (a.prod_x)
            {
                const unsigned go = outer + a.prod_outer0, pp = go / a.prod_batch, b = go - pp * a.prod_batch;
                const size_t plane = (size_t)a.prod_batch * a.src_outer_stride, off = (size_t)b * a.src_outer_stride + rows;
                [[maybe_unused]] const ModDesc md = ld_uniform_mod(&a.t.mods[prime]);
                uint64_t rb[16];
                load_rows(raw, lds_wave, a.prod_x + (pp == 2 ? plane : 0) + off, tid);
                load_rows(rb, lds_wave, a.prod_y + (pp == 0 ? 0 : plane) + off, tid);
                if constexpr (FP)
                {
#pragma unroll
                    for (int e = 0; e < 16; e++)
                        x[e] = fp_mulmod(fp_from_u52(raw[e]), fp_from_u52(rb[e]), m.q, m.qinv);
                    if (pp == 1)
                    {
                        uint64_t rc[16];
                        load_rows(rc, lds_wave, a.prod_x + plane + off, tid);
                        load_rows(rb, lds_wave, a.prod_y + off, tid);
#pragma unroll
                        for (int e = 0; e < 16; e++)
                            x[e] += fp_mulmod(fp_from_u52(rc[e]), fp_from_u52(rb[e]), m.q, m.qinv);
                    }
#pragma unroll
                    for (int e = 0; e < 16; e++)
                        F::fix(x[e], m);
                    if (a.prod_out)
                    {
#pragma unroll
                        for (int e = 0; e < 16; e++)
                            raw[e] = fp_to_canon(x[e], m);
                        store_rows(raw, lds_wave, a.prod_out + (size_t)outer * a.prod_out_stride + rows, tid);
                    }
                    have_x = true;
                }
                else
                {
#pragma unroll
                    for (int e = 0; e < 16; e++)
                        raw[e] = mul_mod(raw[e], rb[e], md);
                    if (pp == 1)
                    {
                        uint64_t rc[16];
                        load_rows(rc, lds_wave, a.prod_x + plane + off, tid);
                        load_rows(rb, lds_wave, a.prod_y + off, tid);
#pragma unroll
                        for (int e = 0; e < 16; e++)
                            raw[e] = add_mod(raw[e], mul_mod(rc[e], rb[e], md), md.q);
                    }
                    if (a.prod_out)
                        store_rows(raw, lds_wave, a.prod_out + (size_t)outer * a.prod_out_stride + rows, tid);
                }
            }
            else if (a.src_gal)
                load_rows_galois(raw, lds_wave, a.src + (size_t)outer * a.src_outer_stride + ((size_t)comp << G::n), (hg * 16 + (tid >> 6) * 4) << 8, a.src_gal, G::n, tid);
            else
                load_rows(raw, lds_wave, a.src + (size_t)outer * a.src_outer_stride + rows, tid);
            if (!have_x)
            {
#pragma unroll
                for (int e = 0; e < 16; e++)
                {
                    x[e] = F::from_canon(raw[e], m);
                    F::fix(x[e], m);
                }
            }
            {
                TwRegs<FP> tw;
                load_tw<FP, 4>(tw, tab, [&](int t) { return (1u << (D1 + 4 + t)) + ((h * 16 + v) << t); });
                phase_inv<FP, 4, 0, ICLS, 0>(x, m, [&](int t, int g) { return tw.get((1 << t) + g); });
            }
#pragma unroll
            for (int e = 0; e < 16; e++)
                F::fix(x[e], m);
#pragma unroll
            for (int e = 0; e < 16; e++)
                lds_wave[ul * kRowWords + v * 18 + e] = F::raw(x[e]);
            __builtin_amdgcn_wave_barrier();
#pragma unroll
            for (int e = 0; e < 16; e++)
                x[e] = F::unraw(lds_wave[ul * kRowWords + e * 18 + v]);
            {
                TwRegs<FP> tw;
                load_tw<FP, 4>(tw, tab, [&](int t) { return (1u << (D1 + t)) + (h << t); });
                phase_inv<FP, 4, 0, ICLS, kInvE1<ICLS>>(x, m, [&](int t, int g) { return tw.get((1 << t) + g); });
            }
#pragma unroll
            for (int e = 0; e < 16; e++)
                F::fix(x[e], m);
            uint64_t *mid_tr = a.mid + (((size_t)outer * a.ncomp + comp) << G::n) + ((size_t)hg << 12);
#pragma unroll
            for (int e = 0; e < 16; e++)
                mid_st<8>(mid_tr + e * 256 + tid, F::raw(x[e]));
        }

        template <int D1, int CLS>
        __global__ void __launch_bounds__(kThreads) ntt2_inv_pa(InvArgs a)
        {
            HIP_DYNAMIC_SHARED(uint64_t, lds)
            const Blk blk = spread_blocks();
            const unsigned comp = blk.y + a.comp0, outer = blk.z;
            const unsigned prime = SHL_UNIFORM(a.comp_prime ? a.comp_prime[comp] : a.prime_first + comp);
            if constexpr (CLS == 1)
                inv_pa_body<true, D1>(a, prime, comp, outer, lds, blk.tile);
            else if constexpr (CLS == 0)
                with_int_class(a.t, prime, [&](auto ic) { inv_pa_body<false, D1, decltype(ic)::value>(a, prime, comp, outer, lds, blk.tile); });
            else if (a.t.fpd[prime].qi)
                inv_pa_body<true, D1>(a, prime, comp, outer, lds, blk.tile);
            else
                inv_pa_body<false, D1, 2>(a, prime, comp, outer, lds, blk.tile);
        }

        template <bool FP, int D1, int ICLS = 2>
        __device__ __forceinline__ void inv_pb_body(const InvArgs &a, unsigned prime, unsigned comp, unsigned outer, uint64_t *lds, unsigned tile)
        {
            typedef Field<FP> F;
            typedef Geo<D1> G;
            static_assert(G::rA >= 1, "the N^-1 stage is handled in phase A");
            const unsigned tid = threadIdx.x, cg = tile;
            const unsigned c = tid & (G::C - 1), hi = tid >> G::LC;
            const typename F::Mod m = F::make_mod(ld_uniform_mod(&a.t.mods[prime]), ld_uniform_fpd(&a.t.fpd[prime]));
            const typename F::tw_t *tab = tw_table<FP>(a.t, true, prime);
            const unsigned col = cg * G::C + c;
            const uint64_t *i = a.mid + (((size_t)outer * a.ncomp + comp) << G::n) + ((size_t)(hi * 16 + (col >> 4)) << 8) + (col & 15);
            typename F::elem x[16];
#pragma unroll
            for (int rb = 0; rb < 16; rb++)
                x[rb] = F::unraw(mid_ld<8>(i + rb * 16));
            {
                TwRegs<FP> tw;
                load_tw<FP, 4>(tw, tab, [&](int t) { return (1u << (G::rA + t)) + (hi << t); });
                phase_inv<FP, 4, 0, ICLS, kInvE2<ICLS>>(x, m, [&](int t, int g) { return tw.get((1 << t) + g); });
            }
#pragma unroll
            for (int e = 0; e < 16; e++)
                F::fix(x[e], m);
#pragma unroll
            for (int rb = 0; rb < 16; rb++)
                lds[(hi * 16 + rb) * G::CP + c] = F::raw(x[rb]);
            __syncthreads();
#pragma unroll
            for (int e = 0; e < 16; e++)
            {
                const unsigned ra = e >> (4 - G::rA), rbh = e & ((1 << (4 - G::rA)) - 1);
                const unsigned R = ra * 16 + (rbh << G::rA) + hi;
                x[e] = F::unraw(lds[R * G::CP + c]);
            }
            phase_inv<FP, G::rA, 1, ICLS, kInvE3<ICLS>>(x, m, [&](int t, int g) { return ld_uniform(tab, (1u << t) + g); });
            {
                typename F::tw_t ni, nw;
                if constexpr (FP)
                {
                    ni = ld_uniform(a.t.ninv_d, 2 * prime);
                    nw = ld_uniform(a.t.ninv_d, 2 * prime + 1);
                }
                else
                {
                    ni = ld_uniform(a.t.ninv, 2 * prime);
                    nw = ld_uniform(a.t.ninv, 2 * prime + 1);
                }
                inv_last_stage<FP, G::rA, ICLS, kInvE3<ICLS>>(x, m, ni, nw);
            }
            uint64_t *o = a.data + (size_t)outer * a.outer_stride + ((size_t)comp << G::n);
#pragma unroll
            for (int e = 0; e < 16; e++)
            {
                F::fix(x[e], m);
                const unsigned ra = e >> (4 - G::rA), rbh = e & ((1 << (4 - G::rA)) - 1);
                const unsigned R = ra * 16 + (rbh << G::rA) + hi;
                uint64_t v = a.lazy ? F::inv_to_lazy(x[e], m) : F::inv_to_canon(x[e], m);
                if (a.out_add)
                    v = csub(v + a.out_add, a.t.mods[prime].q);
                mid_st<16>(o + (size_t)R * 256 + col, v);
            }
        }

        template <int D1, int CLS>
        __global__ void __launch_bounds__(kThreads) ntt2_inv_pb(InvArgs a)
        {
            HIP_DYNAMIC_SHARED(uint64_t, lds)
            const Blk blk = spread_blocks();
            const unsigned comp = blk.y + a.comp0, outer = blk.z;
            const unsigned prime = SHL_UNIFORM(a.comp_prime ? a.comp_prime[comp] : a.prime_first + comp);
            if constexpr (CLS == 1)
                inv_pb_body<true, D1>(a, prime, comp, outer, lds, blk.tile);
            else if constexpr (CLS == 0)
                with_int_class(a.t, prime, [&](auto ic) { inv_pb_body<false, D1, decltype(ic)::value>(a, prime, comp, outer, lds, blk.tile); });
            else if (a.t.fpd[prime].qi)
                inv_pb_body<true, D1>(a, prime, comp, outer, lds, blk.tile);
            else
                inv_pb_body<false, D1, 2>(a, prime, comp, outer, lds, blk.tile);
        }

        template <int D1, int TWW = 1>
        struct FusedGeo
        {
            typedef Geo<D1> G;
            static_assert(G::LC >= 6, "pass 1's phase-B row index must be wave-uniform");
            static_assert(G::lds1_words <= kLds2Words, "pass 1's exchange buffer lives in the team's pass-2 area");
            static constexpr int TEAMS = G::TILES;
            static constexpr int BS = 272;
            static constexpr size_t mid_words = (size_t)TEAMS * 16 * BS;
            static constexpr size_t xch_words = (size_t)TEAMS * kLds2Words;
            static constexpr size_t main_words = mid_words > xch_words ? mid_words : xch_words;
            static constexpr size_t lds_bytes = (main_words + (size_t)TEAMS * 240 * TWW) * 8;
        };
#ifndef SEALHIP_FINT_FWD_TWB
#define SEALHIP_FINT_FWD_TWB 0
#endif
#ifndef SEALHIP_FINT_FWD_PF13
#define SEALHIP_FINT_FWD_PF13 0
#endif
#ifndef SEALHIP_FINT_FWD_PF14
#define SEALHIP_FINT_FWD_PF14 1
#endif
#ifndef SEALHIP_FINT_FWD_WAVES
#define SEALHIP_FINT_FWD_WAVES 4
#endif
#ifndef SEALHIP_FINT_INV_TWB
#define SEALHIP_FINT_INV_TWB 1
#endif
#ifndef SEALHIP_FINT_INV_PF
#define SEALHIP_FINT_INV_PF 0
#endif
#ifndef SEALHIP_FINT_INV_WAVES
#define SEALHIP_FINT_INV_WAVES 4
#endif

        template <bool FP, int D1, int ICLS = 0>
        __device__ __forceinline__ void fwd_fused2_body(const FwdArgs &a, unsigned prime, unsigned comp, unsigned outer, uint64_t *lds)
        {
            typedef Field<FP> F;
            typedef Geo<D1> G;
            typedef FusedGeo<D1, F::tw_words> FG;
            typedef typename F::tw_t tw_t;
            constexpr bool TWB_REGS = FP || (D1 == 5 && SEALHIP_FINT_FWD_TWB == 2);
            constexpr bool TWB_EARLY = !FP && D1 == 5 && SEALHIP_FINT_FWD_TWB == 1;
#ifndef SEALHIP_FP_FWD_PF13
#define SEALHIP_FP_FWD_PF13 0
#endif
            constexpr bool PF = FP ? (D1 != 5 || SEALHIP_FP_FWD_PF13) : ((D1 == 6 && SEALHIP_FINT_FWD_PF14) || (D1 == 5 && SEALHIP_FINT_FWD_PF13));
            const unsigned team = threadIdx.x >> 8, tid = threadIdx.x & 255;
            const typename F::Mod m = F::make_mod(ld_uniform_mod(&a.t.mods[prime]), ld_uniform_fpd(&a.t.fpd[prime]));
            const tw_t *tab = tw_table<FP>(a.t, false, prime);
            uint64_t *mid = lds;
            uint64_t *xch = lds + team * kLds2Words;
            uint64_t *lds_wave = xch + (tid >> 6) * (4 * kRowWords);
            tw_t *twa = reinterpret_cast<tw_t *>(lds + FG::main_words) + team * 240;
            stage_twa<D1>(twa, tab, team, tid);
            const unsigned c = tid & (G::C - 1);
            const unsigned hi = SHL_UNIFORM(tid >> G::LC);
            TwRegs<FP> twb, unused;
            if constexpr (TWB_REGS)
            {
                const unsigned h = team * 16 + (tid >> 4), v = tid & 15;
                load_tw<FP, 4>(twb, tab, [&](int t) { return (1u << (D1 + 4 + t)) + ((h * 16 + v) << t); });
            }
            uint64_t *base = a.data + ((size_t)comp << G::n);
            const uint64_t *in_base = a.src ? a.src + ((size_t)(comp % a.src_ncomp) << G::n) : base;
            const size_t in_stride = a.src ? a.src_outer_stride : a.outer_stride;
            uint64_t nxt[16];
            auto fetch = [&](unsigned z) {
                const uint64_t *in = in_base + (size_t)z * in_stride + team * G::C + c;
#pragma unroll
                for (int e = 0; e < 16; e++)
                {
                    const unsigned ra = e >> (4 - G::rA), rbh = e & ((1 << (4 - G::rA)) - 1);
                    const unsigned R = ra * 16 + (rbh << G::rA) + hi;
                    nxt[e] = in[(size_t)R * 256];
                }
            };
            const unsigned ostride = gridDim.z;
            if constexpr (PF)
                fetch(outer);
            for (; outer < a.nouter; outer += ostride)
            {
                typename F::elem x[16];
                if constexpr (!PF)
                    fetch(outer);
#pragma unroll
                for (int e = 0; e < 16; e++)
                    x[e] = F::from_canon(nxt[e], m);
                if constexpr (PF)
                {
                    if (outer + ostride < a.nouter)
                        fetch(outer + ostride);
                }
                phase_fwd_end<FP, G::rA, true, ICLS, 4>(x, m, [&](int t, int g) { return ld_uniform(tab, (1u << t) + g); });
                __syncthreads();
#pragma unroll
                for (int e = 0; e < 16; e++)
                {
                    const unsigned ra = e >> (4 - G::rA), rbh = e & ((1 << (4 - G::rA)) - 1);
                    const unsigned R = ra * 16 + (rbh << G::rA) + hi;
                    xch[R * G::CP + c] = F::raw(x[e]);
                }
                __syncthreads();
#pragma unroll
                for (int rb = 0; rb < 16; rb++)
                    x[rb] = F::unraw(xch[(hi * 16 + rb) * G::CP + c]);
                phase_fwd_end<FP, 4, true, ICLS, IntBounds<ICLS>::fwd_after(4, G::rA)>(
                    x, m, [&](int t, int g) { return ld_uniform(tab, (1u << (G::rA + t)) + (hi << t) + g); });
                __syncthreads();
                {
                    const unsigned col = team * G::C + c;
                    uint64_t *o = mid + (size_t)(hi * 16 + (col >> 4)) * FG::BS + (col & 15);
#pragma unroll
                    for (int rb = 0; rb < 16; rb++)
                        o[rb * 16] = F::raw(x[rb]);
                }
                __syncthreads();
                {
                    const uint64_t *mp = mid + (size_t)(team * 16) * FG::BS + tid;
#pragma unroll
                    for (int e = 0; e < 16; e++)
                        x[e] = F::unraw(mp[e * FG::BS]);
                }
                if constexpr (TWB_EARLY)
                {
                    const unsigned h = team * 16 + (tid >> 4), v = tid & 15;
                    load_tw<FP, 4>(twb, tab, [&](int t) { return (1u << (D1 + 4 + t)) + ((h * 16 + v) << t); });
                }
                __syncthreads();
                if constexpr (TWB_REGS || TWB_EARLY)
                    p2_tile<FP, D1, false, false, true, true, false, ICLS, kP1Out<ICLS, D1>>(x, m, tab, twa, nullptr, lds_wave, team, tid, &unused, &twb);
                else
                    p2_tile<FP, D1, false, true, false, true, false, ICLS, kP1Out<ICLS, D1>>(x, m, tab, twa, nullptr, lds_wave, team, tid);
                uint64_t val[16];
#pragma unroll
                for (int e = 0; e < 16; e++)
                    val[e] = a.lazy ? fwd_out_lazy<FP, ICLS, kP2Out<ICLS, D1>>(x[e], m) : fwd_out_canon<FP, ICLS, kP2Out<ICLS, D1>>(x[e], m);
                store_rows(val, lds_wave, base + (size_t)outer * a.outer_stride + ((size_t)(team * 16 + (tid >> 6) * 4) << 8), tid);
            }
        }

        template <int D1, int CLS>
        __global__ void __launch_bounds__(FusedGeo<D1>::TEAMS *kThreads, CLS == 1 ? 4 : SEALHIP_FINT_FWD_WAVES) ntt2_fwd_fused2(FwdArgs a)
// ... 251 lines not shown
            auto fetch = [&](unsigned J) {
                const uint64_t *in = in0 + ((size_t)J << G::n);
#pragma unroll
                for (int e = 0; e < 16; e++)
                {
                    const unsigned ra = e >> (4 - G::rA), rbh = e & ((1 << (4 - G::rA)) - 1);
                    const unsigned R = ra * 16 + (rbh << G::rA) + rbl;
#ifdef SEALHIP_KS_NOMEM
                    nxt[e] = (uint64_t)((tid << 4) + (unsigned)e + J * 4099u + R);
#else
                    nxt[e] = in[(size_t)R * 256];
#endif
                }
            };
            const unsigned Jskip = a.skip_diag ? I : ~0u;
            unsigned J = Jskip == j0 ? j0 + 1 : j0;
            if (J < j1)
                fetch(J);
            while (J < j1)
            {
                const uint64_t src_q = a.tb.mods[J].q;
                typename F::elem x[16];
                ks1_map<FP, D1>(nxt, x, src_q, m);
                unsigned Jn = J + 1;
                if (Jn == Jskip)
                    Jn++;
                if (Jn < j1)
                    fetch(Jn);
                uint64_t *mid_tr = a.mid + ((((size_t)b * (a.K + 1) + I) * a.K + J) << G::n);
                p1_tile<FP, D1, 256, FP && kLeanKs<D1>, ICLS>(x, m, tab, tw, lds, mid_tr, cg, tid);
                J = Jn;
            }
        }

        template <bool FP, int D1>
        __global__ void __launch_bounds__(kThreads) ks1_kernel(Ks1Args a)
        {
            typedef Geo<D1> G;
            HIP_DYNAMIC_SHARED(uint64_t, lds)
            const unsigned bid = blockIdx.x;
            const unsigned low = bid & 7, rest = bid >> 3;
            const unsigned it = rest % a.ntargets, grp = (rest / a.ntargets) * 8 + low;
            if (grp >= a.batch * a.parts * G::TILES)
                return;
            const unsigned vb = grp / G::TILES, cg = grp % G::TILES;
            const unsigned b = vb % a.batch, dg = vb / a.batch;
            const unsigned jlen = (a.j1 - a.j0 + a.parts - 1) / a.parts;
            const unsigned j0 = a.j0 + dg * jlen, j1 = j0 + jlen < a.j1 ? j0 + jlen : a.j1;
            const unsigned I = SHL_UNIFORM(a.targets[2 * it]), prime = SHL_UNIFORM(a.targets[2 * it + 1]);
            if constexpr (FP)
                ks1_body<FP, D1>(a, lds, I, prime, b, cg, j0, j1);
            else
                with_int_class(a.tb, prime, [&](auto ic) { ks1_body<FP, D1, decltype(ic)::value>(a, lds, I, prime, b, cg, j0, j1); });
        }

        template <bool FP, int D1, bool SMALL = false>
        __global__ void __launch_bounds__(kThreads, 2) ks1t_kernel(Ks1Args a)
        {
            static_assert(FP || !SMALL, "SMALL is a property of the double-precision launch");
            typedef Field<FP> F;
            typedef Geo<D1> G;
            HIP_DYNAMIC_SHARED(uint64_t, lds)
            const unsigned tid = threadIdx.x;
            const unsigned ndig = a.j1 - a.j0;
            const unsigned grp = blockIdx.x;
            if (grp >= a.batch * ndig * G::TILES)
                return;
            const unsigned cg = grp % G::TILES, bj = grp / G::TILES;
            const unsigned J = a.j0 + bj % ndig, b = bj / ndig;
            const unsigned c = tid & (G::C - 1), rbl = tid >> G::LC;
            const uint64_t *in = a.t + (((size_t)b * a.K + J) << G::n) + cg * G::C + c;
            uint64_t raw[16];
#pragma unroll
            for (int e = 0; e < 16; e++)
            {
                const unsigned ra = e >> (4 - G::rA), rbh = e & ((1 << (4 - G::rA)) - 1);
                const unsigned R = ra * 16 + (rbh << G::rA) + rbl;
                raw[e] = in[(size_t)R * 256];
            }
            const uint64_t src_q = a.tb.mods[J].q;
            const bool as_doubles = SMALL || (FP && !(src_q >> 52));
            if (as_doubles)
            {
#pragma unroll
                for (int e = 0; e < 16; e++)
                    raw[e] = fp_to_bits(fp_from_u52(raw[e]));
            }
#pragma nounroll
            for (unsigned it = 0; it < a.ntargets; it++)
            {
                const unsigned I = SHL_UNIFORM(a.targets[2 * it]), prime = SHL_UNIFORM(a.targets[2 * it + 1]);
                if (a.skip_diag && I == J)
                    continue;
                uint64_t *mid_tr = a.mid + ((((size_t)b * (a.K + 1) + I) * a.K + J) << G::n);
                auto one = [&](auto ic) {
                    constexpr int ICLS = decltype(ic)::value;
                    const typename F::Mod m = F::make_mod(ld_uniform_mod(&a.tb.mods[prime]), ld_uniform_fpd(&a.tb.fpd[prime]));
                    const typename F::tw_t *tab = tw_table<FP>(a.tb, false, prime);
                    TwRegs<FP> tw;
                    p1_load_tw<FP, D1>(tw, tab, tid);
                    typename F::elem x[16];
                    if constexpr (FP)
                    {
                        if (as_doubles)
                        {
#pragma unroll
                            for (int e = 0; e < 16; e++)
                                x[e] = fp_from_bits(raw[e]);
                            if (!kLeanKs<D1> || (double)src_q > kLeanEntry * m.q)
                            {
#pragma unroll
                                for (int e = 0; e < 16; e++)
                                    F::fix(x[e], m);
                            }
                        }
                        else if constexpr (!SMALL)
                            ks1_map<FP, D1>(raw, x, src_q, m);
                    }
                    else
                        ks1_map<FP, D1>(raw, x, src_q, m);
                    p1_tile<FP, D1, 256, FP && kLeanKs<D1>, ICLS>(x, m, tab, tw, lds, mid_tr, cg, tid);
                };
                if constexpr (FP)
                    one(std::integral_constant<int, 0>());
                else
                    with_int_class(a.tb, prime, one);
            }
        }

        struct Ks2Args
        {
            const uint64_t *mid;
            const uint64_t *target;
            const uint64_t *key;
            size_t key_digit_words;
            uint64_t *acc;
            const uint32_t *targets;
            unsigned ntargets;
            unsigned K, L;
            unsigned batch;
            unsigned j0, j1, key_digit0;
            unsigned parts;
            const uint64_t *fold_c0, *fold_c1;
            const ShoupOp *fold_pm;
            const uint64_t *fold_x, *fold_y;
            size_t fold_plane;
            uint32_t gal;
            NttTables tb;
        };

#ifndef SEALHIP_KS2_INT_TWB3
#define SEALHIP_KS2_INT_TWB3 1
#endif
        template <bool FP, int D1, int ICLS = 0>
        __device__ __forceinline__ void ks2_body(const Ks2Args &a, uint64_t *lds, unsigned I, unsigned prime, unsigned koff, unsigned b, unsigned hg,
                                                 unsigned j0, unsigned j1, uint64_t *acc_part)
        {
            typedef Field<FP> F;
            typedef Geo<D1> G;
            const unsigned tid = threadIdx.x;
            const typename F::Mod m = F::make_mod(ld_uniform_mod(&a.tb.mods[prime]), ld_uniform_fpd(&a.tb.fpd[prime]));
            const typename F::tw_t *tab = tw_table<FP>(a.tb, false, prime);

            uint64_t *lds_wave = lds + (tid >> 6) * (4 * kRowWords);
            const typename F::tw_t *twa = nullptr, *twb = nullptr;
            if constexpr (!FP)
            {
                typename F::tw_t *la = reinterpret_cast<typename F::tw_t *>(lds + kLds2Words);
                if (tid < 240)
                {
                    const unsigned t = 31 - __builtin_clz(tid / 16 + 1);
                    const unsigned r = tid - ((16u << t) - 16u);
                    la[tid] = tab[(1u << (D1 + t)) + ((hg * 16) << t) + r];
                }
                twa = la;
#if SEALHIP_KS2_INT_TWB3
                typename F::tw_t *lb = la + 240;
#pragma unroll
                for (int g = 0; g < 8; g++)
                    lb[g * 256 + tid] = tab[(1u << (D1 + 7)) + ((hg * 256 + tid) << 3) + g];
                twb = lb;
#endif
                __syncthreads();
            }
            if constexpr (FP)
            {
                typename F::tw_t *la = reinterpret_cast<typename F::tw_t *>(lds + kLds2Words);
                typename F::tw_t *lb = la + 240;
                if (tid < 240)
                {
                    const unsigned t = 31 - __builtin_clz(tid / 16 + 1);
                    const unsigned r = tid - ((16u << t) - 16u);
                    la[tid] = tab[(1u << (D1 + t)) + ((hg * 16) << t) + r];
                }
#pragma unroll
                for (int t = 0; t < 4; t++)
#pragma unroll
                    for (int g = 0; g < (1 << t); g++)
                        lb[((256u << t) - 256u) + g * 256 + tid] = tab[(1u << (D1 + 4 + t)) + ((hg * 256 + tid) << t) + g];
                twa = la;
                twb = lb;
                __syncthreads();
            }

            typedef typename std::conditional<FP, typename F::Acc, uint64_t>::type acc_t;
            constexpr unsigned kAccRun = ICLS == 2 ? 1 : IntBounds<ICLS>::lim / 4 - 1;
            acc_t acc0[16], acc1[16];
#pragma unroll
            for (int e = 0; e < 16; e++)
            {
                if constexpr (FP)
                {
                    acc0[e] = F::acc_zero();
                    acc1[e] = F::acc_zero();
                }
                else
                {
                    acc0[e] = 0;
                    acc1[e] = 0;
                }
            }
            const size_t N = (size_t)1 << G::n;
            const uint64_t *mid0 = a.mid + ((((size_t)b * (a.K + 1) + I) * a.K) << G::n) + ((size_t)hg << 12);
            const uint64_t *mid0_lane = mid0 + mid_lane(tid);
            const bool diag_prod = a.fold_x && !a.target && I < a.K;
            const bool has_diag = (a.target || diag_prod) && I < a.K;
            const size_t diag_off = (((size_t)b * a.K + I) << G::n) + ((size_t)hg << 12);
            const UniformView diag_view = uniform_view(diag_prod ? a.fold_x + a.fold_plane + diag_off : has_diag ? a.target + diag_off : a.mid);
            uint64_t nxt[16];
            auto fetch = [&](unsigned J) {
                if (has_diag && J == I)
                {
                    if (a.gal)
                    {
                        const uint64_t *poly = a.target + (((size_t)b * a.K + I) << G::n);
#pragma unroll
                        for (int e = 0; e < 16; e++)
                            nxt[e] = poly[galois_src_index((hg << 12) + tid * 16 + e, a.gal, G::n)];
                    }
                    else
                    {
#pragma unroll
                        for (int e = 0; e < 16; e += 2)
                            view_load128(diag_view, tid * 128, e * 8, nxt[e], nxt[e + 1]);
                    }
                }
                else if constexpr (FP)
                {
                    const UniformView mv = uniform_view(mid0 + ((size_t)J << G::n));
#pragma unroll
                    for (int e = 0; e < 16; e++)
                    {
#ifdef SEALHIP_KS_NOMEM
                        nxt[e] = fp_to_bits((double)(int)((tid * 16 + e + J * 4099u) & 0xFFFFF) - 524288.0);
#else
                        if constexpr ((SEALHIP_KS_NT & 2) != 0)
                            nxt[e] = view_load64_nt(mv, mid_lane(tid) * 8, e * (kMidRow * 8));
                        else
                            nxt[e] = view_load64(mv, mid_lane(tid) * 8, e * (kMidRow * 8));
#endif
                    }
                }
                else
                {
                    const uint64_t *mp = mid0_lane + ((size_t)J << G::n);
#pragma unroll
                    for (int e = 0; e < 16; e++)
                    {
#ifdef SEALHIP_KS_NOMEM
                        nxt[e] = ((uint64_t)(tid * 16 + e + J * 4099u) * 0x9E3779B97F4A7C15ull) >> 6;
#else
                        nxt[e] = mid_ld<4>(mp + e * kMidRow);
#endif
                    }
                }
            };
#ifndef SEALHIP_KS2_INT_PF
#define SEALHIP_KS2_INT_PF 1
#endif
            constexpr bool PF = FP || SEALHIP_KS2_INT_PF;
            if constexpr (PF)
            {
                if (j0 < j1)
                    fetch(j0);
            }
            for (unsigned J = j0; J < j1; J++)
            {
                typename F::elem x[16];
                const bool is_diag = has_diag && J == I;
                if constexpr (!PF)
                    fetch(J);
                if (is_diag && diag_prod)
                {
                    const UniformView yv = uniform_view(a.fold_y + a.fold_plane + diag_off);
                    uint64_t yw[16];
#pragma unroll
                    for (int e = 0; e < 16; e += 2)
                        view_load128(yv, tid * 128, e * 8, yw[e], yw[e + 1]);
                    [[maybe_unused]] const ModDesc mdd = ld_uniform_mod(&a.tb.mods[prime]);
#pragma unroll
                    for (int e = 0; e < 16; e++)
                    {
                        if constexpr (FP)
                        {
                            x[e] = fp_mulmod(fp_from_u52(nxt[e]), fp_from_u52(yw[e]), m.q, m.qinv);
                            F::fix(x[e], m);
                        }
                        else
                            x[e] = F::from_canon(mul_mod(nxt[e], yw[e], mdd), m);
                    }
                }
                else if (is_diag)
                {
#pragma unroll
                    for (int e = 0; e < 16; e++)
                        x[e] = F::from_canon(nxt[e], m);
                }
                else
                {
#pragma unroll
                    for (int e = 0; e < 16; e++)
                        x[e] = F::unraw(nxt[e]);
                }
                const size_t kslab = (size_t)(J - a.key_digit0) * a.key_digit_words + (size_t)koff * N;
                typename F::key_t kr0[16], kr1[16];
                prio_phase<2>();
                if constexpr (FP)
                {
                    const UniformView kv = uniform_view(a.key + kslab + ((size_t)hg << 13));
#pragma unroll
                    for (int e = 0; e < 16; e++)
                    {
                        uint64_t w0, w1;
#ifdef SEALHIP_KS_NOMEM
                        w0 = fp_to_bits((double)(int)((tid * 7 + e * 31 + J) & 0xFFFFF) - 500000.0), w1 = fp_to_bits((double)(int)((tid * 3 + e * 17 + J) & 0xFFFFF) - 400000.0);
#else
                        view_load128(kv, tid * 16, e * 4096, w0, w1);
#endif
                        kr0[e] = fp_from_bits(w0);
                        kr1[e] = fp_from_bits(w1);
                    }
                    if (J + 1 < j1)
                        fetch(J + 1);
                }
                else if constexpr (PF)
                {
                    if (J + 1 < j1)
                        fetch(J + 1);
                }
                prio_phase<1>();
                if (!is_diag)
                {
                    p2_tile<FP, D1, FP, true, false, !FP, FP && kLeanKs<D1>, ICLS, kP1Out<ICLS, D1>, !FP && SEALHIP_KS2_INT_TWB3>(x, m, tab, twa, twb, lds_wave, hg, tid);
                }
                if constexpr (FP)
                {
#pragma unroll
                    for (int e = 0; e < 16; e++)
                    {
                        F::mac(acc0[e], x[e], kr0[e], m);
                        F::mac(acc1[e], x[e], kr1[e], m);
                    }
                }
                else
                {
                    const ShoupOp *p0 = reinterpret_cast<const ShoupOp *>(a.key + kslab) + ((size_t)hg << 12) + tid;
                    const ShoupOp *p1 = p0 + N;
#pragma unroll
                    for (int e = 0; e < 16; e++)
                    {
#ifdef SEALHIP_KS_NOMEM
                        const ShoupOp w0{ (uint64_t)(tid * 7 + e * 31 + J) * 0x9E3779B97F4A7C15ull >> 5, (uint64_t)(tid + e) * 0xD1B54A32D192ED03ull }, w1{ w0.wq >> 4, w0.w << 3 };
#else
                        const ShoupOp w0 = p0[e * 256], w1 = p1[e * 256];
#endif
                        if constexpr (ICLS == 2)
                        {
                            acc0[e] = F::guard(acc0[e] + F::mul_lazy(x[e], w0, m), m);
                            acc1[e] = F::guard(acc1[e] + F::mul_lazy(x[e], w1, m), m);
                        }
                        else
                        {
                            acc0[e] = F::mul_rem(x[e], w0, F::mul_hi_approx(x[e], w0), acc0[e], m);
                            acc1[e] = F::mul_rem(x[e], w1, F::mul_hi_approx(x[e], w1), acc1[e], m);
                        }
                    }
                }
                if constexpr (FP)
                {
                    if ((J - j0) % 7 == 6)
                    {
#pragma unroll
                        for (int e = 0; e < 16; e++)
                        {
                            F::acc_fix(acc0[e], m);
                            F::acc_fix(acc1[e], m);
                        }
                    }
                }
                else if constexpr (ICLS != 2)
                {
                    if ((J - j0) % kAccRun == kAccRun - 1)
                    {
#pragma unroll
                        for (int e = 0; e < 16; e++)
                        {
                            F::template fix4<IntBounds<ICLS>::hi32>(acc0[e], m);
                            F::template fix4<IntBounds<ICLS>::hi32>(acc1[e], m);
                        }
                    }
                }
            }
            uint64_t val[16];
            uint64_t *out = acc_part + ((((size_t)b * 2 + 0) * (a.K + 1) + I) << G::n) + ((size_t)(hg * 16 + (tid >> 6) * 4) << 8);
            auto sum_to_canon = [&](const acc_t &s) {
                if constexpr (FP)
                    return F::acc_to_canon(s, m);
                else if constexpr (ICLS == 2)
                    return csub(s, m.q);
                else
                    return F::template canon_any<IntBounds<ICLS>::hi32>(s, m);
            };
            if (a.fold_x && I < a.K)
            {
                const size_t crow = ((((size_t)b * a.K + I) << G::n)) + ((size_t)(hg * 16 + (tid >> 6) * 4) << 8);
                const uint64_t *X0 = a.fold_x + crow, *X1 = X0 + a.fold_plane, *Y0 = a.fold_y + crow, *Y1 = Y0 + a.fold_plane;
                const ShoupOp pm = a.fold_pm[I];
                const uint64_t q = a.tb.mods[prime].q;
                [[maybe_unused]] const ModDesc md = ld_uniform_mod(&a.tb.mods[prime]);
                auto load16 = [&](const uint64_t *P, uint64_t (&v)[16]) {
#pragma unroll
                    for (int k = 0; k < 16; k++)
                        v[k] = mid_ld<16>(P + (k >> 2) * 256 + (k & 3) * 64 + (tid & 63));
                };
                uint64_t p0[16], p1[16];
                uint64_t *out1 = out + ((size_t)(a.K + 1) << G::n);
                if constexpr (FP)
                {
                    const double pmd = pm.w > q / 2 ? -(double)(q - pm.w) : (double)pm.w;
                    double cd[16];
                    load16(X0, p0);
                    load16(Y0, p1);
#pragma unroll
                    for (int k = 0; k < 16; k++)
                        cd[k] = fp_mulmod(fp_from_u52(p0[k]), fp_from_u52(p1[k]), m.q, m.qinv);
#pragma unroll
                    for (int e = 0; e < 16; e++)
                        val[e] = fp_to_bits(fp_mulmod(fp_fix(acc0[e], m.q, m.qinv), pmd, m.q, m.qinv));
                    emit_rows_k(val, lds_wave, tid, [&](int k, unsigned off, uint64_t sv) {
                        mid_st<16>(out + off, fp_to_canon(fp_fix(fp_from_bits(sv) + cd[k], m.q, m.qinv), m));
                    });
                    load16(Y1, p1);
#pragma unroll
                    for (int k = 0; k < 16; k++)
                        cd[k] = fp_mulmod(fp_from_u52(p0[k]), fp_from_u52(p1[k]), m.q, m.qinv);
                    load16(X1, p0);
                    load16(Y0, p1);
#pragma unroll
                    for (int k = 0; k < 16; k++)
                        cd[k] += fp_mulmod(fp_from_u52(p0[k]), fp_from_u52(p1[k]), m.q, m.qinv);
#pragma unroll
                    for (int e = 0; e < 16; e++)
                        val[e] = fp_to_bits(fp_mulmod(fp_fix(acc1[e], m.q, m.qinv), pmd, m.q, m.qinv));
                    emit_rows_k(val, lds_wave, tid, [&](int k, unsigned off, uint64_t sv) {
                        mid_st<16>(out1 + off, fp_to_canon(fp_fix(fp_from_bits(sv) + cd[k], m.q, m.qinv), m));
                    });
                    return;
                }
                uint64_t cv[16];
                load16(X0, p0);
                load16(Y0, p1);
#pragma unroll
                for (int k = 0; k < 16; k++)
                    cv[k] = mul_mod(p0[k], p1[k], md);
#pragma unroll
                for (int e = 0; e < 16; e++)
                    val[e] = sum_to_canon(acc0[e]);
                emit_rows_k(val, lds_wave, tid, [&](int k, unsigned off, uint64_t sv) {
                    mid_st<16>(out + off, add_mod(mul_shoup(sv, pm.w, pm.wq, q), cv[k], q));
                });
                load16(Y1, p1);
#pragma unroll
                for (int k = 0; k < 16; k++)
                    cv[k] = mul_mod(p0[k], p1[k], md);
                load16(X1, p0);
                load16(Y0, p1);
#pragma unroll
                for (int k = 0; k < 16; k++)
                    cv[k] = add_mod(cv[k], mul_mod(p0[k], p1[k], md), q);
#pragma unroll
                for (int e = 0; e < 16; e++)
                    val[e] = sum_to_canon(acc1[e]);
                emit_rows_k(val, lds_wave, tid, [&](int k, unsigned off, uint64_t sv) {
                    mid_st<16>(out1 + off, add_mod(mul_shoup(sv, pm.w, pm.wq, q), cv[k], q));
                });
                return;
            }
            if (a.fold_c0 && I < a.K)
            {
                const size_t crow = ((((size_t)b * a.K + I) << G::n)) + ((size_t)(hg * 16 + (tid >> 6) * 4) << 8);
                const uint64_t *C0 = a.fold_c0 + crow, *C1 = a.fold_c1 ? a.fold_c1 + crow : nullptr;
                const ShoupOp pm = a.fold_pm[I];
                const uint64_t q = a.tb.mods[prime].q;
                uint64_t cv0[16], cv1[16];
#pragma unroll
                for (int k = 0; k < 16; k++)
                {
                    const unsigned off = (k >> 2) * 256 + (k & 3) * 64 + (tid & 63);
                    if (a.gal)
                        cv0[k] = mid_ld<16>(a.fold_c0 + (((size_t)b * a.K + I) << G::n) + galois_src_index(((hg * 16 + (tid >> 6) * 4) << 8) + off, a.gal, G::n));
                    else
                        cv0[k] = mid_ld<16>(C0 + off);
                    cv1[k] = C1 ? mid_ld<16>(C1 + off) : 0;
                }
                uint64_t *out1 = out + ((size_t)(a.K + 1) << G::n);
                if constexpr (FP)
                {
                    const double pmd = pm.w > q / 2 ? -(double)(q - pm.w) : (double)pm.w;
#pragma unroll
                    for (int e = 0; e < 16; e++)
                        val[e] = fp_to_bits(fp_mulmod(fp_fix(acc0[e], m.q, m.qinv), pmd, m.q, m.qinv));
                    emit_rows_k(val, lds_wave, tid, [&](int k, unsigned off, uint64_t sv) {
                        mid_st<16>(out + off, fp_to_canon(fp_fix(fp_from_bits(sv) + fp_from_u52(cv0[k]), m.q, m.qinv), m));
                    });
#pragma unroll
                    for (int e = 0; e < 16; e++)
                        val[e] = fp_to_bits(fp_mulmod(fp_fix(acc1[e], m.q, m.qinv), pmd, m.q, m.qinv));
                    emit_rows_k(val, lds_wave, tid, [&](int k, unsigned off, uint64_t sv) {
                        mid_st<16>(out1 + off, fp_to_canon(fp_fix(fp_from_bits(sv) + fp_from_u52(cv1[k]), m.q, m.qinv), m));
                    });
                    return;
                }
#pragma unroll
                for (int e = 0; e < 16; e++)
                    val[e] = sum_to_canon(acc0[e]);
                emit_rows_k(val, lds_wave, tid, [&](int k, unsigned off, uint64_t sv) {
                    mid_st<16>(out + off, add_mod(mul_shoup(sv, pm.w, pm.wq, q), cv0[k], q));
                });
#pragma unroll
                for (int e = 0; e < 16; e++)
                    val[e] = sum_to_canon(acc1[e]);
                emit_rows_k(val, lds_wave, tid, [&](int k, unsigned off, uint64_t sv) {
                    mid_st<16>(out1 + off, add_mod(mul_shoup(sv, pm.w, pm.wq, q), cv1[k], q));
                });
                return;
            }
#pragma unroll
            for (int e = 0; e < 16; e++)
                val[e] = sum_to_canon(acc0[e]);
            store_rows(val, lds_wave, out, tid);
#pragma unroll
            for (int e = 0; e < 16; e++)
                val[e] = sum_to_canon(acc1[e]);
            store_rows(val, lds_wave, out + ((size_t)(a.K + 1) << G::n), tid);
        }

        template <int D1, int CLS>
#ifndef SEALHIP_KS2_INT_WAVES
#define SEALHIP_KS2_INT_WAVES 2
#endif
        __global__ void __launch_bounds__(kThreads, CLS == 0 ? SEALHIP_KS2_INT_WAVES : 2) ks2_kernel(Ks2Args a)
        {
            typedef Geo<D1> G;
            HIP_DYNAMIC_SHARED(uint64_t, lds)
            const unsigned ntile = a.ntargets * G::TILES;
            const unsigned bid = blockIdx.x;
            const unsigned xcd = bid & 7, rest = bid >> 3;
            const unsigned vbatch = a.batch * a.parts;
            const unsigned vb = rest % vbatch, tile_hi = rest / vbatch;
            const unsigned b = vb % a.batch, dg = vb / a.batch;
            const unsigned jlen = (a.j1 - a.j0 + a.parts - 1) / a.parts;
            const unsigned j0 = a.j0 + dg * jlen, j1 = j0 + jlen < a.j1 ? j0 + jlen : a.j1;
            uint64_t *acc_part = a.acc + (((size_t)dg * a.batch * 2 * (a.K + 1)) << G::n);
            const unsigned tile = tile_hi * 8 + xcd;
            if (tile >= ntile)
                return;
            const unsigned it = tile / G::TILES, hg = tile % G::TILES;
            const unsigned I = SHL_UNIFORM(a.targets[4 * it]), prime = SHL_UNIFORM(a.targets[4 * it + 1]), koff = SHL_UNIFORM(a.targets[4 * it + 3]);
            if constexpr (CLS == 1)
                ks2_body<true, D1>(a, lds, I, prime, koff, b, hg, j0, j1, acc_part);
            else
                with_int_class(a.tb, prime, [&](auto ic) { ks2_body<false, D1, decltype(ic)::value>(a, lds, I, prime, koff, b, hg, j0, j1, acc_part); });
        }

        __device__ __forceinline__ void key_offsets(unsigned *off, const FpDesc *fpd, unsigned L)
        {
            if (threadIdx.x == 0)
            {
                unsigned u = 0;
                for (unsigned c = 0; c < L; c++)
                {
                    off[c] = u;
                    u += fpd[c].qi ? 2u : 4u;
                }
                off[L] = u;
            }
            __syncthreads();
        }
        __global__ void __launch_bounds__(kThreads) key_layout_kernel(
            const uint64_t *in, uint64_t *out, const FpDesc *fpd, const ModDesc *mods, unsigned L, unsigned n_log, size_t polys)
        {
            __shared__ unsigned off[kMaxKeyComps + 1];
            key_offsets(off, fpd, L);
            const size_t N = (size_t)1 << n_log;
            const size_t total = polys * L * N;
            for (size_t i = blockIdx.x * (size_t)kThreads + threadIdx.x; i < total; i += (size_t)gridDim.x * kThreads)
            {
                const size_t p = i & (N - 1), slab = i >> n_log;
                const unsigned comp = (unsigned)(slab % L);
                const size_t poly = slab / L, digit = poly >> 1;
                const unsigned k = (unsigned)(poly & 1);
                const size_t hg = p >> 12;
                const unsigned e = (unsigned)(p >> 8) & 15, tid = (unsigned)p & 255;
                size_t nat = (hg << 12) + ((size_t)(tid >> 4) << 8) + ((tid & 15) << 4) + e;
                const uint64_t v = in[(slab << n_log) + nat];
                uint64_t *o = out + ((digit * off[L] + off[comp]) << n_log);
                if (fpd[comp].qi)
                {
                    double d = fp_from_u52(v);
                    if (v > fpd[comp].qi / 2)
                        d -= fpd[comp].q;
                    o[2 * p + k] = fp_to_bits(d);
                }
                else
                {
                    typedef unsigned __int128 u128;
                    const ModDesc md = mods[comp];
                    const u128 vr = (u128)v * md.ratio_hi + (((u128)v * md.ratio_lo) >> 64);
                    uint64_t est = vr > (u128)~(uint64_t)0 ? ~(uint64_t)0 : (uint64_t)vr;
                    u128 rem = ((u128)v << 64) - (u128)est * md.q;
                    while (rem >= md.q)
                    {
                        rem -= md.q;
                        est++;
                    }
                    o += (size_t)k << (n_log + 1);
                    o[2 * p] = v;
                    o[2 * p + 1] = est;
                }
            }
        }

        __global__ void __launch_bounds__(kThreads) key_unlayout_kernel(
            const uint64_t *in, uint64_t *out, const FpDesc *fpd, unsigned L, unsigned n_log, size_t polys)
        {
            __shared__ unsigned off[kMaxKeyComps + 1];
            key_offsets(off, fpd, L);
            const size_t N = (size_t)1 << n_log;
            const size_t total = polys * L * N;
            for (size_t i = blockIdx.x * (size_t)kThreads + threadIdx.x; i < total; i += (size_t)gridDim.x * kThreads)
            {
                const size_t p = i & (N - 1), slab = i >> n_log;
                const unsigned comp = (unsigned)(slab % L);
                const size_t poly = slab / L, digit = poly >> 1;
                const unsigned k = (unsigned)(poly & 1);
                const size_t hg = p >> 12;
                const unsigned e = (unsigned)(p >> 8) & 15, tid = (unsigned)p & 255;
                const size_t nat = (hg << 12) + ((size_t)(tid >> 4) << 8) + ((tid & 15) << 4) + e;
                const uint64_t *o = in + ((digit * off[L] + off[comp]) << n_log);
                uint64_t v;
                if (fpd[comp].qi)
                {
                    double d = fp_from_bits(o[2 * p + k]);
                    if (d < 0)
                        d += fpd[comp].q;
                    v = (uint64_t)d;
                }
                else
                    v = o[((size_t)k << (n_log + 1)) + 2 * p];
                out[(slab << n_log) + nat] = v;
            }
        }

        struct CompRun
        {
            unsigned c0, nc;
            int cls;
        };
        std::vector<CompRun> comp_runs(const NttTables &t, const uint32_t *comp_prime, unsigned prime_first, unsigned ncomp, int cls_hint = -1)
        {
            std::vector<CompRun> runs;
            if (comp_prime && (cls_hint == 0 || cls_hint == 1))
            {
                runs.push_back(CompRun{ 0, ncomp, cls_hint });
                return runs;
            }
            static const bool split = !shl_ab_getenv("SEALHIP_NTT_NOSPLIT");
            unsigned c = 0;
            while (c < ncomp)
            {
                int cls = 2;
                unsigned e = ncomp;
                if (split && !comp_prime && t.fp_host)
                {
                    cls = t.fp_host[prime_first + c] ? 1 : 0;
                    e = c + 1;
                    while (e < ncomp && (t.fp_host[prime_first + e] ? 1 : 0) == cls)
                        e++;
                }
                runs.push_back(CompRun{ c, e - c, cls });
                c = e;
            }
            return runs;
        }

        struct SideStream
        {
            hipStream_t stream = nullptr;
            hipEvent_t fork = nullptr, join = nullptr;
            bool ok = false;
            SideStream()
            {
                ok = !shl_ab_getenv("SEALHIP_NTT_NOFORK") && hipStreamCreateWithFlags(&stream, hipStreamNonBlocking) == hipSuccess &&
                     hipEventCreateWithFlags(&fork, hipEventDisableTiming) == hipSuccess &&
                     hipEventCreateWithFlags(&join, hipEventDisableTiming) == hipSuccess;
            }
        };
        SideStream &side_stream()
        {
            static thread_local SideStream s;
            return s;
        }
        template <class RunFn>
        hipError_t launch_runs(const std::vector<CompRun> &runs, hipStream_t s, RunFn run, bool may_fork = true)
        {
            size_t longest = 0;
            for (size_t i = 1; i < runs.size(); i++)
                if (runs[i].nc > runs[longest].nc)
                    longest = i;
            SideStream &ss = side_stream();
            const bool fork = may_fork && runs.size() > 1 && ss.ok;
            hipError_t e;
            if (fork)
            {
                if ((e = hipEventRecord(ss.fork, s)) != hipSuccess || (e = hipStreamWaitEvent(ss.stream, ss.fork, 0)) != hipSuccess)
                    return e;
                for (size_t i = 0; i < runs.size(); i++)
                    if (i != longest && (e = run(runs[i], ss.stream)) != hipSuccess)
                        return e;
                if ((e = hipEventRecord(ss.join, ss.stream)) != hipSuccess)
                    return e;
            }
            for (size_t i = 0; i < runs.size(); i++)
                if ((!fork || i == longest) && (e = run(runs[i], s)) != hipSuccess)
                    return e;
            if (fork && (e = hipStreamWaitEvent(s, ss.join, 0)) != hipSuccess)
                return e;
            return hipSuccess;
        }

#ifndef SEALHIP_FUSED_FORK14
#define SEALHIP_FUSED_FORK14 1
#endif
        inline bool fused_int()
        {
            static const bool on = !shl_ab_getenv("SEALHIP_NTT_NOFUSED_INT");
            return on;
        }

#ifndef SEALHIP_SRC_P1T_MIN_WGS
#define SEALHIP_SRC_P1T_MIN_WGS 512
#endif
        inline bool src_resident(unsigned tiles, unsigned nouter, const CompRun &r)
        {
            static const char *order_env = std::getenv("SEALHIP_TAIL_P1_ORDER");
            static const char *min_env = shl_ab_getenv("SEALHIP_TAIL_P1_MIN_WGS");
            static const bool trace = shl_ab_getenv("SEALHIP_TAIL_P1_TRACE") != nullptr;
            static const size_t min_wgs = min_env ? (size_t)std::atol(min_env) : (size_t)SEALHIP_SRC_P1T_MIN_WGS;
            bool yes = false;
            if (r.cls != 0 && r.cls != 1)
                yes = false;
            else if (order_env && (order_env[0] == '0' || order_env[0] == '1'))
                yes = order_env[0] == '1';
            else
                yes = r.nc > 1 && (size_t)tiles * nouter >= min_wgs;
            if (trace)
                std::fprintf(stderr, "[tail] pass 1 %s (%u tiles x %u items, %u targets of class %d)\n", yes ? "source-resident" : "target-resident",
                             tiles, nouter, r.nc, r.cls);
            return yes;
        }
        template <int D1, bool TWO>
        hipError_t launch_src_p1t(const Tail2Args &g, const CompRun &r, unsigned nouter, hipStream_t st)
        {
            typedef Geo<D1> G;
            const size_t l1 = G::rA > 0 ? G::lds1_words * 8 : 8;
            const dim3 grid(G::TILES * nouter);
            if (r.cls == 1 && TWO && !(g.x.src2_q >> 52))
                hipLaunchKernelGGL((ntt2_src_p1t<D1, 1, TWO, TWO>), grid, dim3(kThreads), l1, st, g, r.nc);
            else if (r.cls == 1)
                hipLaunchKernelGGL((ntt2_src_p1t<D1, 1, TWO>), grid, dim3(kThreads), l1, st, g, r.nc);
            else
                hipLaunchKernelGGL((ntt2_src_p1t<D1, 0, TWO>), grid, dim3(kThreads), l1, st, g, r.nc);
            return hipGetLastError();
        }

        template <int D1>
        hipError_t launch_fwd(const FwdArgs &a, unsigned nouter, hipStream_t s)
        {
            typedef Geo<D1> G;
            unsigned per = G::TILES * a.ncomp;
#ifndef SEALHIP_NTT_WG_TARGET
#define SEALHIP_NTT_WG_TARGET 8192
#endif
            unsigned chunks = (SEALHIP_NTT_WG_TARGET + per - 1) / per;
            if (const char *f = shl_ab_getenv("SEALHIP_NTT_CHUNKS"))
                chunks = (unsigned)std::atoi(f) ? (unsigned)std::atoi(f) : 1;
            if (chunks > nouter)
                chunks = nouter;
            if (chunks > 65535)
                chunks = 65535;
            size_t l1 = G::rA > 0 ? G::lds1_words * 8 : 8;
            bool fused = false;
            unsigned fchunks = 1;
            if constexpr (D1 == 5 || D1 == 6)
            {
                static const bool fused_ok = !shl_ab_getenv("SEALHIP_NTT_NOFUSED");
                if (fused_ok && (!a.src || a.src_mode == 0) && a.epi == 0)
                {
                    static bool raised = false;
                    if (!raised)
                    {
                        if (hipFuncSetAttribute(reinterpret_cast<const void *>(&ntt2_fwd_fused2<D1, 1>), hipFuncAttributeMaxDynamicSharedMemorySize, (int)FusedGeo<D1>::lds_bytes) != hipSuccess ||
                            hipFuncSetAttribute(reinterpret_cast<const void *>(&ntt2_fwd_fused2<D1, 0>), hipFuncAttributeMaxDynamicSharedMemorySize, (int)(FusedGeo<D1, 2>::lds_bytes)) != hipSuccess)
                            return hipErrorInvalidValue;
                        raised = true;
                    }
                    fused = true;
                    const unsigned want = D1 == 5 ? 2048 : 1024;
                    fchunks = (want + a.ncomp - 1) / a.ncomp;
                    if (const char *f = std::getenv("SEALHIP_NTT_FCHUNKS"))
                        fchunks = (unsigned)std::atoi(f) ? (unsigned)std::atoi(f) : 1;
                    if (fchunks > nouter)
                        fchunks = nouter;
                    if (fchunks > 65535)
                        fchunks = 65535;
                }
            }
            return launch_runs(comp_runs(a.t, a.comp_prime, a.prime_first, a.ncomp, a.cls_hint), s, [&](const CompRun &r, hipStream_t st) {
                FwdArgs g = a;
                g.comp0 = r.c0;
#ifndef SEALHIP_MID_PACK
#define SEALHIP_MID_PACK 1
#endif
                g.mid_pack = SEALHIP_MID_PACK && D1 == 8 && r.cls == 1 && a.epi == 0 && chunks < nouter ? 1 : 0;
                if constexpr (D1 == 5 || D1 == 6)
                {
                    if (fused && r.cls == 1)
                    {
                        hipLaunchKernelGGL((ntt2_fwd_fused2<D1, 1>), dim3(1, r.nc, fchunks), dim3(FusedGeo<D1>::TEAMS * kThreads), FusedGeo<D1>::lds_bytes, st, g);
                        return hipGetLastError();
                    }
                    if (fused && r.cls == 0 && fused_int())
                    {
                        constexpr size_t lds_int = FusedGeo<D1, 2>::lds_bytes;
                        hipLaunchKernelGGL((ntt2_fwd_fused2<D1, 0>), dim3(1, r.nc, fchunks), dim3(FusedGeo<D1>::TEAMS * kThreads), lds_int, st, g);
                        return hipGetLastError();
                    }
                }
                dim3 grid(G::TILES, r.nc, chunks);
                if constexpr (D1 == 8)
                {
                    if (r.cls == 1 && !a.src && a.epi == 0 && a.ring)
                    {
                        const unsigned z = ntt2_ring_teams(r.nc, nouter);
                        if (z && ntt2_ring_run_words(r.nc, z) <= a.ring_words && ntt2_ring_stream_ok(st))
                        {
                            const NttRingRun run{ a.data, a.outer_stride, a.comp_prime, a.prime_first, a.ncomp, r.c0, r.nc, nouter, a.lazy, z, a.ring, a.ring_words };
                            return ntt2_ring_launch(a.t, run, st);
                        }
                    }
                }
                if constexpr (D1 == 8)
                {
                    if (g.mid_pack)
                    {
                        hipLaunchKernelGGL((ntt2_fwd_p1<D1, 5>), grid, dim3(kThreads), l1, st, g);
                        hipError_t ep = hipGetLastError();
                        if (ep != hipSuccess)
                            return ep;
                        hipLaunchKernelGGL((ntt2_fwd_p2<D1, 5>), grid, dim3(kThreads), (kLds2Words + 240) * 8, st, g);
                        return hipGetLastError();
                    }
                }
                if (a.src && (a.src_mode == 2 || a.src_mode == 3) && a.src_ncomp == 1 && src_resident(G::TILES, nouter, r))
                {
                    hipError_t e1 = launch_src_p1t<D1, false>(Tail2Args{ g, NttTail2{} }, r, nouter, st);
                    if (e1 != hipSuccess)
                        return e1;
                }
                else if (r.cls == 1)
                    hipLaunchKernelGGL((ntt2_fwd_p1<D1, 1>), grid, dim3(kThreads), l1, st, g);
                else if (r.cls == 0)
                    hipLaunchKernelGGL((ntt2_fwd_p1<D1, 0>), grid, dim3(kThreads), l1, st, g);
                else
                    hipLaunchKernelGGL((ntt2_fwd_p1<D1, 2>), grid, dim3(kThreads), l1, st, g);
                hipError_t e = hipGetLastError();
                if (e != hipSuccess)
                    return e;
                static const int p2_hoist = shl_ab_getenv("SEALHIP_P2_HOIST") ? std::atoi(shl_ab_getenv("SEALHIP_P2_HOIST")) : 4;
                if (r.cls == 1 && a.epi == 0 && chunks < nouter && p2_hoist == 4)
                    hipLaunchKernelGGL((ntt2_fwd_p2<D1, 4>), grid, dim3(kThreads), (kLds2Words + 240) * 8, st, g);
                else if (r.cls == 1 && a.epi == 0 && chunks < nouter && p2_hoist == 3)
                    hipLaunchKernelGGL((ntt2_fwd_p2<D1, 3>), grid, dim3(kThreads), kLds2Words * 8, st, g);
                else if (r.cls == 1)
                    hipLaunchKernelGGL((ntt2_fwd_p2<D1, 1>), grid, dim3(kThreads), kLds2Words * 8, st, g);
                else if (r.cls == 0)
                    hipLaunchKernelGGL((ntt2_fwd_p2<D1, 0>), grid, dim3(kThreads), kLds2Words * 8, st, g);
                else
                    hipLaunchKernelGGL((ntt2_fwd_p2<D1, 2>), grid, dim3(kThreads), kLds2Words * 8, st, g);
                return hipGetLastError();
            }, !(fused && fused_int()) || (D1 == 6 && SEALHIP_FUSED_FORK14));
        }

        template <int D1>
        hipError_t launch_tail2(const Tail2Args &a, unsigned nouter, hipStream_t s)
        {
            typedef Geo<D1> G;
            unsigned per = G::TILES * a.f.ncomp;
#ifndef SEALHIP_TAIL2_WG_TARGET
#define SEALHIP_TAIL2_WG_TARGET 4096
#endif
            unsigned chunks = (SEALHIP_TAIL2_WG_TARGET + per - 1) / per;
            if (chunks > nouter)
                chunks = nouter;
            if (chunks > 65535)
                chunks = 65535;
            const size_t l1 = G::rA > 0 ? G::lds1_words * 8 : 8;
            return launch_runs(comp_runs(a.f.t, nullptr, a.f.prime_first, a.f.ncomp), s, [&](const CompRun &r, hipStream_t st) {
                Tail2Args g = a;
                g.f.comp0 = r.c0;
                dim3 grid(G::TILES, r.nc, chunks);
                if (src_resident(G::TILES, nouter, r))
                {
                    hipError_t e1 = launch_src_p1t<D1, true>(g, r, nouter, st);
                    if (e1 != hipSuccess)
                        return e1;
                }
                else if (r.cls == 1)
                    hipLaunchKernelGGL((ntt2_tail2_p1<D1, 1>), grid, dim3(kThreads), l1, st, g);
                else if (r.cls == 0)
                    hipLaunchKernelGGL((ntt2_tail2_p1<D1, 0>), grid, dim3(kThreads), l1, st, g);
                else
                    hipLaunchKernelGGL((ntt2_tail2_p1<D1, 2>), grid, dim3(kThreads), l1, st, g);
                hipError_t e = hipGetLastError();
                if (e != hipSuccess)
                    return e;
                if (r.cls == 1)
                    hipLaunchKernelGGL((ntt2_tail2_p2<D1, 1>), grid, dim3(kThreads), kLds2Words * 8, st, g);
                else if (r.cls == 0)
                    hipLaunchKernelGGL((ntt2_tail2_p2<D1, 0>), grid, dim3(kThreads), kLds2Words * 8, st, g);
                else
                    hipLaunchKernelGGL((ntt2_tail2_p2<D1, 2>), grid, dim3(kThreads), kLds2Words * 8, st, g);
                return hipGetLastError();
            });
        }

        template <int D1>
        hipError_t launch_inv(const InvArgs &a, unsigned nouter, hipStream_t s)
        {
            typedef Geo<D1> G;
            bool fused = false;
            unsigned fchunks = 1;
            if constexpr (D1 == 5 || D1 == 6)
            {
                static const bool fused_ok = !shl_ab_getenv("SEALHIP_NTT_NOFUSED");
                if (fused_ok && !a.prod_x && !a.src_gal)
                {
                    static bool raised = false;
                    if (!raised)
                    {
                        if (hipFuncSetAttribute(reinterpret_cast<const void *>(&ntt2_inv_fused2<D1, 1>), hipFuncAttributeMaxDynamicSharedMemorySize, (int)FusedGeo<D1>::lds_bytes) != hipSuccess ||
                            hipFuncSetAttribute(reinterpret_cast<const void *>(&ntt2_inv_fused2<D1, 0>), hipFuncAttributeMaxDynamicSharedMemorySize, (int)(FusedGeo<D1, 2>::lds_bytes)) != hipSuccess)
                            return hipErrorInvalidValue;
                        raised = true;
                    }
                    fused = true;
                    const unsigned want = D1 == 5 ? 2048 : 1024;
                    fchunks = (want + a.ncomp - 1) / a.ncomp;
                    if (D1 == 5 && nouter / 4 > fchunks)
                        fchunks = nouter / 4;
                    if (const char *f = std::getenv("SEALHIP_NTT_FCHUNKS"))
                        fchunks = (unsigned)std::atoi(f) ? (unsigned)std::atoi(f) : 1;
                    if (fchunks > nouter)
                        fchunks = nouter;
                    if (fchunks > 65535)
                        fchunks = 65535;
                }
            }
            return launch_runs(comp_runs(a.t, a.comp_prime, a.prime_first, a.ncomp, a.cls_hint), s, [&](const CompRun &r, hipStream_t st) {
                InvArgs g = a;
                g.comp0 = r.c0;
                g.nouter = nouter;
                if constexpr (D1 == 5 || D1 == 6)
                {
                    if (fused && r.cls == 1)
                    {
                        hipLaunchKernelGGL((ntt2_inv_fused2<D1, 1>), dim3(1, r.nc, fchunks), dim3(FusedGeo<D1>::TEAMS * kThreads), FusedGeo<D1>::lds_bytes, st, g);
                        return hipGetLastError();
                    }
                    if (fused && r.cls == 0 && fused_int())
                    {
                        constexpr size_t lds_int = FusedGeo<D1, 2>::lds_bytes;
                        hipLaunchKernelGGL((ntt2_inv_fused2<D1, 0>), dim3(1, r.nc, fchunks), dim3(FusedGeo<D1>::TEAMS * kThreads), lds_int, st, g);
                        return hipGetLastError();
                    }
                }
                dim3 grid(G::TILES, r.nc, nouter);
                if (r.cls == 1)
                    hipLaunchKernelGGL((ntt2_inv_pa<D1, 1>), grid, dim3(kThreads), kLds2Words * 8, st, g);
                else if (r.cls == 0)
                    hipLaunchKernelGGL((ntt2_inv_pa<D1, 0>), grid, dim3(kThreads), kLds2Words * 8, st, g);
                else
                    hipLaunchKernelGGL((ntt2_inv_pa<D1, 2>), grid, dim3(kThreads), kLds2Words * 8, st, g);
                hipError_t e = hipGetLastError();
                if (e != hipSuccess)
                    return e;
                static const char *skip_env = shl_ab_getenv("SEALHIP_AB_SKIP_INV_PB");
                static long skip_after = skip_env ? std::atol(skip_env) : -1;
                static std::atomic<long> inv_launches{ 0 };
                if (skip_after >= 0 && inv_launches.fetch_add(1) >= skip_after)
                    return (hipError_t)hipSuccess;
                if (r.cls == 1)
                    hipLaunchKernelGGL((ntt2_inv_pb<D1, 1>), grid, dim3(kThreads), G::lds1_words * 8, st, g);
                else if (r.cls == 0)
                    hipLaunchKernelGGL((ntt2_inv_pb<D1, 0>), grid, dim3(kThreads), G::lds1_words * 8, st, g);
                else
                    hipLaunchKernelGGL((ntt2_inv_pb<D1, 2>), grid, dim3(kThreads), G::lds1_words * 8, st, g);
                return hipGetLastError();
            }, !(fused && fused_int()) || (D1 == 6 && SEALHIP_FUSED_FORK14));
        }

        template <int D1>
        hipError_t launch_ks(const Ks1Args &a1, const Ks2Args &a2, unsigned batch, unsigned n_int, hipStream_t s, int order1, bool no_class_fork)
        {
            typedef Geo<D1> G;
            if (a1.ntargets == 0)
                return hipSuccess;
            const size_t l1 = G::rA > 0 ? G::lds1_words * 8 : 8;
            const unsigned vbatch = batch * a1.parts;
            const unsigned groups = vbatch * G::TILES;
            const unsigned n_fp = a1.ntargets - n_int;
            const size_t l2_fp = kLds2Words * 8 + (240 + 3840) * sizeof(double);
            const size_t l2_int = kLds2Words * 8 + (240 + (SEALHIP_KS2_INT_TWB3 ? 2048 : 0)) * sizeof(ShoupOp);
            if (n_int && l2_int > 65536)
            {
                static bool raised_int = false;
                if (!raised_int)
                {
                    if (hipFuncSetAttribute(reinterpret_cast<const void *>(&ks2_kernel<D1, 0>), hipFuncAttributeMaxDynamicSharedMemorySize, (int)l2_int) != hipSuccess)
                        return hipErrorInvalidValue;
                    raised_int = true;
                }
            }
            if (n_fp && l2_fp > 65536)
            {
                static bool raised = false;
                if (!raised)
                {
                    if (hipFuncSetAttribute(reinterpret_cast<const void *>(&ks2_kernel<D1, 1>), hipFuncAttributeMaxDynamicSharedMemorySize, (int)l2_fp) != hipSuccess)
                        return hipErrorInvalidValue;
                    raised = true;
                }
            }
            auto run_class = [&](bool fp, hipStream_t st) -> hipError_t {
                const unsigned t0 = fp ? n_int : 0, nt = fp ? n_fp : n_int;
                if (!nt)
                    return hipSuccess;
                Ks1Args c1 = a1;
                c1.targets = a1.targets + 2 * t0;
                c1.ntargets = nt;
                const dim3 g1(((groups + 7) / 8) * nt * 8);
                static const char *order_env = shl_ab_getenv("SEALHIP_KS1_ORDER");
                const unsigned g1t = batch * (a1.j1 - a1.j0) * G::TILES;
                const bool digit_resident = order_env ? order_env[0] == '1' : order1 >= 0 ? (order1 == 1 && a1.parts == 1) : (a1.parts == 1 && g1t >= 4096);
                if (digit_resident && fp)
                {
                    const unsigned char *small = a1.tb.fp_host;
                    for (unsigned ja = a1.j0; ja < a1.j1;)
                    {
                        const bool sm = small && small[ja];
                        unsigned jb = ja + 1;
                        while (jb < a1.j1 && (small && small[jb]) == sm)
                            jb++;
                        Ks1Args cr = c1;
                        cr.j0 = ja;
                        cr.j1 = jb;
                        const dim3 gr(batch * (jb - ja) * G::TILES);
                        if (sm)
                            hipLaunchKernelGGL((ks1t_kernel<true, D1, true>), gr, dim3(kThreads), l1, st, cr);
                        else
                            hipLaunchKernelGGL((ks1t_kernel<true, D1, false>), gr, dim3(kThreads), l1, st, cr);
                        ja = jb;
                    }
                }
                else if (digit_resident)
                    hipLaunchKernelGGL((ks1t_kernel<false, D1>), dim3(g1t), dim3(kThreads), l1, st, c1);
                else if (fp)
                    hipLaunchKernelGGL((ks1_kernel<true, D1>), g1, dim3(kThreads), l1, st, c1);
                else
                    hipLaunchKernelGGL((ks1_kernel<false, D1>), g1, dim3(kThreads), l1, st, c1);
                hipError_t e = hipGetLastError();
                if (e != hipSuccess)
                    return e;
                Ks2Args c2 = a2;
                c2.targets = a2.targets + 4 * t0;
                c2.ntargets = nt;
                const unsigned ntile = nt * G::TILES;
                if (fp)
                    hipLaunchKernelGGL((ks2_kernel<D1, 1>), dim3(((ntile + 7) / 8) * vbatch * 8), dim3(kThreads), l2_fp, st, c2);
                else
                    hipLaunchKernelGGL((ks2_kernel<D1, 0>), dim3(((ntile + 7) / 8) * vbatch * 8), dim3(kThreads), l2_int, st, c2);
                return hipGetLastError();
            };
            SideStream &ss = side_stream();
            static const bool fork_ok = !shl_ab_getenv("SEALHIP_KS_NOFORK");
            hipError_t e;
            if (n_int && n_fp && ss.ok && fork_ok && !no_class_fork)
            {
                if ((e = hipEventRecord(ss.fork, s)) != hipSuccess || (e = hipStreamWaitEvent(ss.stream, ss.fork, 0)) != hipSuccess)
                    return e;
                if ((e = run_class(false, ss.stream)) != hipSuccess || (e = hipEventRecord(ss.join, ss.stream)) != hipSuccess)
                    return e;
                if ((e = run_class(true, s)) != hipSuccess)
                    return e;
                return hipStreamWaitEvent(s, ss.join, 0);
            }
            if ((e = run_class(false, s)) != hipSuccess)
                return e;
            return run_class(true, s);
        }
    }

    bool ntt2_supports(int log_n)
    {
        return log_n >= 13 && log_n <= 16;
    }

    size_t ntt2_ring_words(const NttTables &t, const NttBatch &b)
    {
        if (t.log_n != 16 || b.src || b.epi || b.tail2 || b.ncomp == 0 || b.nouter == 0)
            return 0;
        if (!ntt2_ring_teams(1, b.nouter))
            return 0;
        size_t words = 0;
        for (const CompRun &r : comp_runs(t, b.comp_prime, b.prime_first, b.ncomp, b.cls_hint))
            if (r.cls == 1)
            {
                const unsigned z = ntt2_ring_teams(r.nc, b.nouter);
                if (z)
                    words = std::max(words, ntt2_ring_run_words(r.nc, z));
            }
        return words;
    }

    hipError_t ntt2_forward(const NttTables &t, const NttBatch &b, int out_lazy, uint64_t *mid, hipStream_t stream, uint64_t *ring, size_t ring_words)
    {
        if (b.ncomp == 0 || b.nouter == 0)
            return hipSuccess;
        FwdArgs a;
        a.ring = ring;
        a.ring_words = ring ? ring_words : 0;
        a.data = b.data;
        a.outer_stride = b.outer_stride;
        a.mid = mid;
        a.src = b.src;
        a.src_outer_stride = b.src_outer_stride;
        a.src_ncomp = b.src_ncomp ? b.src_ncomp : 1;
        a.src_mode = b.src ? b.src_mode : 0;
        a.src_half = b.src_half;
        a.src_q = b.src_q;
        a.src_fix = b.src_fix;
        a.comp_prime = b.comp_prime;
        a.cls_hint = b.cls_hint;
        a.prime_first = b.prime_first;
        a.ncomp = b.ncomp;
        a.comp0 = 0;
        a.nouter = b.nouter;
        a.lazy = out_lazy;
        a.epi = b.epi;
        a.epi_a = b.epi_a;
        a.epi_a_stride = b.epi_a_stride;
        a.epi_mul = b.epi_mul;
        a.epi_out0 = b.epi_out0;
        a.epi_out1 = b.epi_out1;
        a.epi_out_stride = b.epi_out_stride;
        a.mid_pack = 0;
        a.t = t;
        if (b.tail2)
        {
            if (!b.src || (b.src_mode != 2 && b.src_mode != 3) || b.comp_prime || !b.epi_a || !b.epi_mul || !b.epi_out0 || !b.epi_out1)
                return hipErrorInvalidValue;
            Tail2Args t2{ a, *b.tail2 };
            switch (t.log_n)
            {
            case 13:
                return launch_tail2<5>(t2, b.nouter, stream);
            case 14:
                return launch_tail2<6>(t2, b.nouter, stream);
            case 15:
                return launch_tail2<7>(t2, b.nouter, stream);
            case 16:
                return launch_tail2<8>(t2, b.nouter, stream);
            default:
                return hipErrorInvalidValue;
            }
        }
        switch (t.log_n)
        {
        case 13:
            return launch_fwd<5>(a, b.nouter, stream);
        case 14:
            return launch_fwd<6>(a, b.nouter, stream);
        case 15:
            return launch_fwd<7>(a, b.nouter, stream);
        case 16:
            return launch_fwd<8>(a, b.nouter, stream);
        default:
            return hipErrorInvalidValue;
        }
    }

    hipError_t ntt2_inverse(const NttTables &t, const NttBatch &b, int out_lazy, uint64_t *mid, hipStream_t stream)
    {
        if (b.ncomp == 0 || b.nouter == 0)
            return hipSuccess;
        InvArgs a;
        a.data = b.data;
        a.outer_stride = b.outer_stride;
        a.src = b.src ? b.src : b.data;
        a.src_outer_stride = b.src ? b.src_outer_stride : b.outer_stride;
        a.mid = mid;
        a.comp_prime = b.comp_prime;
        a.cls_hint = b.cls_hint;
        a.prime_first = b.prime_first;
        a.ncomp = b.ncomp;
        a.comp0 = 0;
        a.nouter = 0;
        a.lazy = out_lazy;
        if (b.out_add && out_lazy)
            return hipErrorInvalidValue;
        a.out_add = b.out_add;
        a.prod_x = b.prod_x;
        a.prod_y = b.prod_y;
        a.prod_batch = b.prod_batch;
        a.prod_outer0 = b.prod_outer0;
        a.prod_out = b.prod_out;
        a.prod_out_stride = b.prod_out_stride;
        a.src_gal = b.src_galois_elt;
        if (b.src_galois_elt && (!b.src || b.prod_x || !(b.src_galois_elt & 1)))
            return hipErrorInvalidValue;
        if (b.prod_x && (!b.prod_y || !b.prod_batch || (size_t)b.nouter + b.prod_outer0 > (size_t)3 * b.prod_batch || !b.src_outer_stride))
            return hipErrorInvalidValue;
        if (b.prod_x && !b.prod_outer0 && b.nouter != 3 * b.prod_batch)
            return hipErrorInvalidValue;
        if (b.prod_out && (!b.prod_x || !b.prod_out_stride))
            return hipErrorInvalidValue;
        if (b.prod_x)
            a.src_outer_stride = b.src_outer_stride;
        a.t = t;
        const unsigned zmax = 65535;
        for (unsigned z0 = 0; z0 < b.nouter; z0 += zmax)
        {
            unsigned nz = b.nouter - z0 < zmax ? b.nouter - z0 : zmax;
            InvArgs az = a;
            az.prod_outer0 = b.prod_outer0 + z0;
            if (az.prod_out)
                az.prod_out = a.prod_out + (size_t)z0 * a.prod_out_stride;
            az.data = a.data + (size_t)z0 * a.outer_stride;
            az.src = a.src + (size_t)z0 * a.src_outer_stride;
            az.mid = a.mid + (((size_t)z0 * a.ncomp) << t.log_n);
            hipError_t e;
            switch (t.log_n)
            {
            case 13:
                e = launch_inv<5>(az, nz, stream);
                break;
            case 14:
                e = launch_inv<6>(az, nz, stream);
                break;
            case 15:
                e = launch_inv<7>(az, nz, stream);
                break;
            case 16:
                e = launch_inv<8>(az, nz, stream);
                break;
            default:
                return hipErrorInvalidValue;
            }
// ... 90 lines not shown
```

Baseline: 10350.

## Add packed 52-bit intermediate for N=2^16 NTT mid buffers, reorder ks2 loads

Adds a packed 13-word-per-16-value representation of the double-precision NTT intermediate between pass 1 and pass 2 of the folded tail and the inverse NTT. Each value is shuffled through LDS and packed at 52 bits to cut mid-buffer traffic. The packed paths are gated behind the SEALHIP_PACK_TAIL_MID and SEALHIP_PACK_INV_MID environment switches, which are off by default, and counters are exported through a new stats API. Separately, the ks2 epilogue's X1/Y1 loads are reordered under a default-on macro so the accumulator is written rather than added on the first product.

```diff
diff --git a/include/sealhip.h b/include/sealhip.h
--- a/include/sealhip.h
+++ b/include/sealhip.h
@@ -393,6 +393,7 @@
 SHL_FUNC SealHip_InstallAbortTrace(const char *path);
 SHL_FUNC SealHip_KsChunkStats(uint64_t *calls, uint64_t *chunks, uint64_t *scratch_bytes_max);
 SHL_FUNC SealHip_TailStats(uint64_t *folded, uint64_t *plain, uint64_t *dropped);
+SHL_FUNC SealHip_PackStats(uint64_t *tail_mid, uint64_t *inv_mid);
 SHL_FUNC SealHip_ProductStats(uint64_t *fused, uint64_t *formed, uint64_t *dropped);
 SHL_FUNC SealHip_GaloisStats(uint64_t *gathered, uint64_t *permuted);
 SHL_FUNC SealHip_XofStats(uint64_t *polynomials, uint64_t *replaced_words, uint64_t *host_walk_ns, uint64_t *total_ns);
diff --git a/seal_amd/__init__.py b/seal_amd/__init__.py
--- a/seal_amd/__init__.py
+++ b/seal_amd/__init__.py
@@ -1,12 +1,12 @@
 from .api import (CoeffModulus, PlainModulus, EncryptionParameters, SEALContext, ContextData, Ciphertext, Plaintext, KSwitchKeys,
                   RelinKeys, GaloisKeys, Evaluator, SecretKey, PublicKey, KeyGenerator, Decryptor, Encryptor, BatchEncoder, CKKSEncoder, Graph, ItemMap, DeviceBuffer, HipTimer, ntt_forward, ntt_inverse,
-                  dyadic_product, apply_galois, rns_stage, device_synchronize, device_info, release_pool, pool_stats, tail_stats, product_stats, galois_stats, ks_chunk_stats, xof_stats, Stream, Comm, device_count, set_device,
+                  dyadic_product, apply_galois, rns_stage, device_synchronize, device_info, release_pool, pool_stats, tail_stats, pack_stats, product_stats, galois_stats, ks_chunk_stats, xof_stats, Stream, Comm, device_count, set_device,
                   set_staged_host_copies, install_abort_trace)
 from ._native import SealHipError, InvalidArgument, LogicError, OutOfRange, DeviceError, load
 
 __all__ = [
     "CoeffModulus", "PlainModulus", "EncryptionParameters", "SEALContext", "ContextData", "Ciphertext", "Plaintext", "KSwitchKeys",
     "RelinKeys", "GaloisKeys", "Evaluator", "SecretKey", "PublicKey", "KeyGenerator", "Decryptor", "Encryptor", "BatchEncoder", "CKKSEncoder", "Graph", "ItemMap", "DeviceBuffer", "HipTimer", "ntt_forward", "ntt_inverse",
-    "dyadic_product", "apply_galois", "rns_stage", "device_synchronize", "device_info", "release_pool", "pool_stats", "tail_stats", "product_stats", "galois_stats", "ks_chunk_stats", "xof_stats", "Stream", "Comm", "device_count", "set_device", "set_staged_host_copies", "install_abort_trace", "SealHipError",
+    "dyadic_product", "apply_galois", "rns_stage", "device_synchronize", "device_info", "release_pool", "pool_stats", "tail_stats", "pack_stats", "product_stats", "galois_stats", "ks_chunk_stats", "xof_stats", "Stream", "Comm", "device_count", "set_device", "set_staged_host_copies", "install_abort_trace", "SealHipError",
     "InvalidArgument", "LogicError", "OutOfRange", "DeviceError", "load",
 ]
diff --git a/seal_amd/_native.py b/seal_amd/_native.py
--- a/seal_amd/_native.py
+++ b/seal_amd/_native.py
@@ -96,7 +96,7 @@
 Evaluator_RelinearizeDigitParallel Evaluator_ApplyGaloisDigitParallel Evaluator_RotateVectorDigitParallel
 Evaluator_BroadcastKeyDigits Evaluator_SwitchKeySlots Evaluator_SwitchKeyPackTargets Evaluator_SwitchKeyFinishOwned
 Evaluator_SwitchKeyAddGathered
-SealHip_ReleasePool SealHip_PoolStats SealHip_TailStats SealHip_ProductStats SealHip_GaloisStats SealHip_XofStats SealHip_KsChunkStats SealHip_SetStagedHostCopies SealHip_InstallAbortTrace shl_stream_create shl_stream_destroy shl_device_count shl_set_device
+SealHip_ReleasePool SealHip_PoolStats SealHip_TailStats SealHip_PackStats SealHip_ProductStats SealHip_GaloisStats SealHip_XofStats SealHip_KsChunkStats SealHip_SetStagedHostCopies SealHip_InstallAbortTrace shl_stream_create shl_stream_destroy shl_device_count shl_set_device
 shl_ntt_forward shl_ntt_inverse shl_dyadic_product shl_apply_galois shl_rns_stage shl_malloc shl_free
 shl_memcpy_h2d shl_memcpy_d2h shl_device_synchronize shl_timer_create shl_timer_destroy shl_timer_start
 shl_timer_stop
diff --git a/seal_amd/api.py b/seal_amd/api.py
--- a/seal_amd/api.py
+++ b/seal_amd/api.py
@@ -1758,6 +1758,12 @@
     return a.value, b.value, c.value
 
 
+def pack_stats():
+    a, b = C.c_uint64(), C.c_uint64()
+    N.check(N.lib().SealHip_PackStats(C.byref(a), C.byref(b)))
+    return a.value, b.value
+
+
 def product_stats():
     a, b, c = C.c_uint64(), C.c_uint64(), C.c_uint64()
     N.check(N.lib().SealHip_ProductStats(C.byref(a), C.byref(b), C.byref(c)))
diff --git a/seal_amd/csrc/capi_kernels.cpp b/seal_amd/csrc/capi_kernels.cpp
--- a/seal_amd/csrc/capi_kernels.cpp
+++ b/seal_amd/csrc/capi_kernels.cpp
@@ -550,6 +550,17 @@
             *dropped = d;
         SHL_CATCH
     }
+    SHL_FUNC SealHip_PackStats(uint64_t *tail_mid, uint64_t *inv_mid)
+    {
+        SHL_TRY
+        uint64_t t, i;
+        ntt2_pack_stats(t, i);
+        if (tail_mid)
+            *tail_mid = t;
+        if (inv_mid)
+            *inv_mid = i;
+        SHL_CATCH
+    }
     SHL_FUNC shl_device_count(int *count)
     {
         IfNullRet(count, SHL_E_POINTER);
diff --git a/seal_amd/csrc/ntt2_device.h b/seal_amd/csrc/ntt2_device.h
--- a/seal_amd/csrc/ntt2_device.h
+++ b/seal_amd/csrc/ntt2_device.h
@@ -115,6 +115,13 @@
 #pragma unroll
             for (int r = 0; r < 16; r++)
             {
+#if defined(SEALHIP_CHECK_BOUNDS) && !defined(__HIP_DEVICE_COMPILE__)
+                if (!(x[r] >= -2251799813685248.0 && x[r] < 2251799813685248.0 && x[r] == __builtin_rint(x[r])))
+                {
+                    std::fprintf(stderr, "sealhip: pack52 bound 2^51 violated (%g) at %s:%d\n", x[r], __FILE__, __LINE__);
+                    std::abort();
+                }
+#endif
                 const uint64_t b = fp_to_bits(x[r] + kPackMagic);
                 lo[r] = (uint32_t)b;
                 hi[r] = (uint32_t)(b >> 32) & 0xFFFFFu;
@@ -148,6 +155,46 @@
                 const uint64_t b = (uint64_t)lo | ((uint64_t)(0x43300000u | (top << 16) | mid) << 32);
                 x[r] = fp_from_bits(b) - kPackMagic;
             }
+        }
+        template <int BIT>
+        __device__ __forceinline__ void pack_store(uint64_t *blk, unsigned c, const uint64_t (&w)[13])
+        {
+#if SEALHIP_PACK_VEC16
+#pragma unroll
+            for (int j = 0; j < 6; j++)
+                mid_st2<BIT>(blk + j * 32 + c * 2, w[2 * j], w[2 * j + 1]);
+            mid_st<BIT>(blk + 192 + c, w[12]);
+#else
+#pragma unroll
+            for (int k = 0; k < 13; k++)
+                mid_st<BIT>(blk + k * 16 + c, w[k]);
+#endif
+        }
+        template <int BIT>
+        __device__ __forceinline__ void pack_load(const uint64_t *blk, unsigned c, uint64_t (&w)[13])
+        {
+#if SEALHIP_PACK_VEC16
+#pragma unroll
+            for (int j = 0; j < 6; j++)
+                mid_ld2<BIT>(blk + j * 32 + c * 2, w[2 * j], w[2 * j + 1]);
+            w[12] = mid_ld<BIT>(blk + 192 + c);
+#else
+#pragma unroll
+            for (int k = 0; k < 13; k++)
+                w[k] = mid_ld<BIT>(blk + k * 16 + c);
+#endif
+        }
+        __device__ __forceinline__ void pack_hand_over(const double (&y)[16], double (&x)[16], uint64_t *lds, unsigned tid)
+        {
+            __syncthreads();
+#pragma unroll
+            for (int r = 0; r < 16; r++)
+                lds[r * kPackLdsRow + tid] = fp_to_bits(y[r]);
+            __syncthreads();
+#pragma unroll
+            for (int e = 0; e < 16; e++)
+                x[e] = fp_from_bits(lds[(tid >> 4) * kPackLdsRow + e * 16 + (tid & 15)]);
+            __syncthreads();
         }
 
         __device__ __forceinline__ int int_class(const NttTables &t, unsigned prime)
diff --git a/seal_amd/csrc/ntt2_kernels.h b/seal_amd/csrc/ntt2_kernels.h
--- a/seal_amd/csrc/ntt2_kernels.h
+++ b/seal_amd/csrc/ntt2_kernels.h
@@ -4,6 +4,8 @@
 namespace sealhip
 {
     bool ntt2_supports(int log_n);
+
+    void ntt2_pack_stats(uint64_t &tail_mid, uint64_t &inv_mid);
 
     size_t ntt2_ring_words(const NttTables &t, const NttBatch &b);
     hipError_t ntt2_forward(const NttTables &t, const NttBatch &b, int out_lazy, uint64_t *mid, hipStream_t stream, uint64_t *ring = nullptr, size_t ring_words = 0);
diff --git a/seal_amd/csrc/ntt2_kernels.hip b/seal_amd/csrc/ntt2_kernels.hip
--- a/seal_amd/csrc/ntt2_kernels.hip
+++ b/seal_amd/csrc/ntt2_kernels.hip
@@ -322,11 +322,12 @@
             }
         }
 
-        template <bool FP, int D1, int ICLS>
+        template <bool FP, int D1, int ICLS, bool PACK = false>
         __device__ __forceinline__ void tail2_p2_body(const Tail2Args &t2, unsigned prime, unsigned comp, unsigned outer, uint64_t *lds, unsigned tile)
         {
             typedef Field<FP> F;
             typedef Geo<D1> G;
+            static_assert(!PACK || (FP && D1 == 8), "the packed intermediate is defined for the double-precision pass at N = 2^16");
             const FwdArgs &a = t2.f;
             const unsigned tid = threadIdx.x, hg = tile;
             const typename F::Mod m = F::make_mod(ld_uniform_mod(&a.t.mods[prime]), ld_uniform_fpd(&a.t.fpd[prime]));
@@ -340,21 +341,47 @@
             const size_t row0 = ((size_t)comp << G::n) + ((size_t)(hg * 16 + (tid >> 6) * 4) << 8);
             uint64_t nxt[16];
             auto fetch = [&](unsigned z) {
-                const uint64_t *mp = mid0 + (((size_t)z * a.ncomp) << G::n);
-#pragma unroll
-                for (int e = 0; e < 16; e++)
-                    nxt[e] = mid_ld<4>(mp + e * kMidRow);
+                if constexpr (PACK)
+                {
+                    uint64_t w[13];
+                    pack_load<4>(a.mid + (((size_t)z * a.ncomp + comp) << G::n) + (size_t)(hg * 16 + (tid >> 4)) * kPackBlock, tid & 15, w);
+#pragma unroll
+                    for (int k = 0; k < 13; k++)
+                        nxt[k] = w[k];
+                }
+                else
+                {
+                    const uint64_t *mp = mid0 + (((size_t)z * a.ncomp) << G::n);
+#pragma unroll
+                    for (int e = 0; e < 16; e++)
+                        nxt[e] = mid_ld<4>(mp + e * kMidRow);
+                }
             };
             const unsigned ostride = gridDim.z;
             fetch(outer);
             for (; outer < a.nouter; outer += ostride)
             {
                 typename F::elem x[16];
-#pragma unroll
-                for (int e = 0; e < 16; e++)
-                    x[e] = F::unraw(nxt[e]);
-                if (outer + ostride < a.nouter)
-                    fetch(outer + ostride);
+                if constexpr (PACK)
+                {
+                    uint64_t w[13];
+#pragma unroll
+                    for (int k = 0; k < 13; k++)
+                        w[k] = nxt[k];
+                    if (outer + ostride < a.nouter)
+                        fetch(outer + ostride);
+                    double y[16];
+                    unpack52(w, y);
+                    pack_hand_over(y, x, lds, tid);
+                }
+                else
+                {
+#pragma unroll
+                    for (int e = 0; e < 16; e++)
+                        x[e] = F::unraw(nxt[e]);
+                    if (outer + ostride < a.nouter)
+                        fetch(outer + ostride);
+                }
                 const uint64_t *A = a.epi_a + (size_t)outer * a.epi_a_stride + row0;
                 const uint64_t *C = ((outer & 1) ? t2.x.c1 : t2.x.c0) + (size_t)(outer >> 1) * t2.x.c_stride + row0;
                 const bool folded = t2.x.a_has_c;
@@ -416,7 +443,9 @@
             const Blk blk = spread_blocks();
             const unsigned comp = blk.y + a.f.comp0, outer = blk.z;
             const unsigned prime = SHL_UNIFORM(a.f.prime_first + comp);
-            if constexpr (CLS == 1)
+            if constexpr (CLS == 5)
+                tail2_p2_body<true, D1, 0, D1 == 8>(a, prime, comp, outer, lds, blk.tile);
+            else if constexpr (CLS == 1)
                 tail2_p2_body<true, D1, 0>(a, prime, comp, outer, lds, blk.tile);
             else if constexpr (CLS == 0)
                 with_int_class(a.f.t, prime, [&](auto ic) { tail2_p2_body<false, D1, decltype(ic)::value>(a, prime, comp, outer, lds, blk.tile); });
@@ -434,10 +463,11 @@
             return v;
         }
 
-        template <bool FP, int D1, bool TWO, bool SMALL2>
+        template <bool FP, int D1, bool TWO, bool SMALL2, bool PACK = false>
         __device__ __forceinline__ void src_p1t_body(const Tail2Args &t2, unsigned nc, uint64_t *lds)
         {
             static_assert(!SMALL2 || (FP && TWO), "SMALL2 is a property of the double-precision launch of the folded tail");
+            static_assert(!PACK || (SMALL2 && D1 == 8), "the packed intermediate is defined for the folded tail's double-precision pass at N = 2^16");
             typedef Field<FP> F;
             typedef Geo<D1> G;
             const FwdArgs &a = t2.f;
@@ -528,7 +558,7 @@
                                 x[e] = mul_shoup(v, pm.w, pm.wq, q) + u;
                             }
                         }
-                        p1_tile<FP, D1, 256, FP && G::rA == 4, ICLS>(x, m, tab, tw, lds, mid_tr, cg, tid);
+                        p1_tile<FP, D1, 256, FP && G::rA == 4, ICLS, PACK>(x, m, tab, tw, lds, mid_tr, cg, tid);
                     }
                 };
                 if constexpr (FP)
@@ -541,12 +571,12 @@
 #ifndef SEALHIP_SRC_P1T_FP2_WGS
 #define SEALHIP_SRC_P1T_FP2_WGS 2
 #endif
-        template <int D1, int CLS, bool TWO, bool SMALL2 = false>
+        template <int D1, int CLS, bool TWO, bool SMALL2 = false, bool PACK = false>
         __global__ void __launch_bounds__(kThreads, SMALL2 ? SEALHIP_SRC_P1T_FP2_WGS : 2) ntt2_src_p1t(Tail2Args a, unsigned nc)
         {
             static_assert(CLS == 0 || CLS == 1, "single-class runs only");
             HIP_DYNAMIC_SHARED(uint64_t, lds)
-            src_p1t_body<CLS == 1, D1, TWO, SMALL2>(a, nc, lds);
+            src_p1t_body<CLS == 1, D1, TWO, SMALL2, PACK>(a, nc, lds);
         }
 
         struct InvArgs
@@ -579,7 +609,7 @@
         template <int ICLS>
         constexpr int kInvE3 = inv_phase_exp<ICLS>(kInvE2<ICLS>, 4, 0);
 
-        template <bool FP, int D1, int ICLS = 2>
+        template <bool FP, int D1, int ICLS = 2, bool PACK = false>
         __device__ __forceinline__ void inv_pa_body(const InvArgs &a, unsigned prime, unsigned comp, unsigned outer, uint64_t *lds, unsigned tile)
         {
             typedef Field<FP> F;
@@ -683,6 +713,23 @@
             for (int e = 0; e < 16; e++)
                 F::fix(x[e], m);
             uint64_t *mid_tr = a.mid + (((size_t)outer * a.ncomp + comp) << G::n) + ((size_t)hg << 12);
+            if constexpr (PACK)
+            {
+                static_assert(!PACK || (FP && D1 == 8), "the packed intermediate is defined for the double-precision pass at N = 2^16");
+                __syncthreads();
+#pragma unroll
+                for (int e = 0; e < 16; e++)
+                    lds[e * kPackLdsRow + tid] = F::raw(x[e]);
+                __syncthreads();
+                double y[16];
+#pragma unroll
+                for (int r = 0; r < 16; r++)
+                    y[r] = fp_from_bits(lds[u * kPackLdsRow + r * 16 + v]);
+                uint64_t w[13];
+                pack52(y, w);
+                pack_store<8>(a.mid + (((size_t)outer * a.ncomp + comp) << G::n) + (size_t)(hg * 16 + u) * kPackBlock, v, w);
+                return;
+            }
 #pragma unroll
             for (int e = 0; e < 16; e++)
                 mid_st<8>(mid_tr + e * 256 + tid, F::raw(x[e]));
@@ -695,7 +742,9 @@
             const Blk blk = spread_blocks();
             const unsigned comp = blk.y + a.comp0, outer = blk.z;
             const unsigned prime = SHL_UNIFORM(a.comp_prime ? a.comp_prime[comp] : a.prime_first + comp);
-            if constexpr (CLS == 1)
+            if constexpr (CLS == 5)
+                inv_pa_body<true, D1, 2, D1 == 8>(a, prime, comp, outer, lds, blk.tile);
+            else if constexpr (CLS == 1)
                 inv_pa_body<true, D1>(a, prime, comp, outer, lds, blk.tile);
             else if constexpr (CLS == 0)
                 with_int_class(a.t, prime, [&](auto ic) { inv_pa_body<false, D1, decltype(ic)::value>(a, prime, comp, outer, lds, blk.tile); });
@@ -705,7 +754,7 @@
                 inv_pa_body<false, D1, 2>(a, prime, comp, outer, lds, blk.tile);
         }
 
-        template <bool FP, int D1, int ICLS = 2>
+        template <bool FP, int D1, int ICLS = 2, bool PACK = false>
         __device__ __forceinline__ void inv_pb_body(const InvArgs &a, unsigned prime, unsigned comp, unsigned outer, uint64_t *lds, unsigned tile)
         {
             typedef Field<FP> F;
@@ -718,9 +767,19 @@
             const unsigned col = cg * G::C + c;
             const uint64_t *i = a.mid + (((size_t)outer * a.ncomp + comp) << G::n) + ((size_t)(hi * 16 + (col >> 4)) << 8) + (col & 15);
             typename F::elem x[16];
-#pragma unroll
-            for (int rb = 0; rb < 16; rb++)
-                x[rb] = F::unraw(mid_ld<8>(i + rb * 16));
+            if constexpr (PACK)
+            {
+                static_assert(!PACK || (FP && D1 == 8), "the packed intermediate is defined for the double-precision pass at N = 2^16");
+                uint64_t w[13];
+                pack_load<8>(a.mid + (((size_t)outer * a.ncomp + comp) << G::n) + (size_t)(hi * 16 + cg) * kPackBlock, c, w);
+                unpack52(w, x);
+            }
+            else
+            {
+#pragma unroll
+                for (int rb = 0; rb < 16; rb++)
+                    x[rb] = F::unraw(mid_ld<8>(i + rb * 16));
+            }
             {
                 TwRegs<FP> tw;
                 load_tw<FP, 4>(tw, tab, [&](int t) { return (1u << (G::rA + t)) + (hi << t); });
@@ -776,7 +835,9 @@
             const Blk blk = spread_blocks();
             const unsigned comp = blk.y + a.comp0, outer = blk.z;
             const unsigned prime = SHL_UNIFORM(a.comp_prime ? a.comp_prime[comp] : a.prime_first + comp);
-            if constexpr (CLS == 1)
+            if constexpr (CLS == 5)
+                inv_pb_body<true, D1, 2, D1 == 8>(a, prime, comp, outer, lds, blk.tile);
+            else if constexpr (CLS == 1)
                 inv_pb_body<true, D1>(a, prime, comp, outer, lds, blk.tile);
             else if constexpr (CLS == 0)
                 with_int_class(a.t, prime, [&](auto ic) { inv_pb_body<false, D1, decltype(ic)::value>(a, prime, comp, outer, lds, blk.tile); });
@@ -1334,6 +1395,9 @@
 #ifndef SEALHIP_KS2_INT_TWB3
 #define SEALHIP_KS2_INT_TWB3 1
 #endif
+#ifndef SEALHIP_KS2_Y0_ONCE
+#define SEALHIP_KS2_Y0_ONCE 1
+#endif
         template <bool FP, int D1, int ICLS = 0>
         __device__ __forceinline__ void ks2_body(const Ks2Args &a, uint64_t *lds, unsigned I, unsigned prime, unsigned koff, unsigned b, unsigned hg,
                                                  unsigned j0, unsigned j1, uint64_t *acc_part)
@@ -1632,6 +1696,16 @@
                     emit_rows_k(val, lds_wave, tid, [&](int k, unsigned off, uint64_t sv) {
                         mid_st<16>(out + off, fp_to_canon(fp_fix(fp_from_bits(sv) + cd[k], m.q, m.qinv), m));
                     });
+#if SEALHIP_KS2_Y0_ONCE
+                    load16(X1, val);
+#pragma unroll
+                    for (int k = 0; k < 16; k++)
+                        cd[k] = fp_mulmod(fp_from_u52(val[k]), fp_from_u52(p1[k]), m.q, m.qinv);
+                    load16(Y1, p1);
+#pragma unroll
+                    for (int k = 0; k < 16; k++)
+                        cd[k] = fp_mulmod(fp_from_u52(p0[k]), fp_from_u52(p1[k]), m.q, m.qinv) + cd[k];
+#else
                     load16(Y1, p1);
 #pragma unroll
                     for (int k = 0; k < 16; k++)
@@ -1641,6 +1715,7 @@
 #pragma unroll
                     for (int k = 0; k < 16; k++)
                         cd[k] += fp_mulmod(fp_from_u52(p0[k]), fp_from_u52(p1[k]), m.q, m.qinv);
+#endif
 #pragma unroll
                     for (int e = 0; e < 16; e++)
                         val[e] = fp_to_bits(fp_mulmod(fp_fix(acc1[e], m.q, m.qinv), pmd, m.q, m.qinv));
@@ -1661,6 +1736,16 @@
                 emit_rows_k(val, lds_wave, tid, [&](int k, unsigned off, uint64_t sv) {
                     mid_st<16>(out + off, add_mod(mul_shoup(sv, pm.w, pm.wq, q), cv[k], q));
                 });
+#if SEALHIP_KS2_Y0_ONCE
+                load16(X1, val);
+#pragma unroll
+                for (int k = 0; k < 16; k++)
+                    cv[k] = mul_mod(val[k], p1[k], md);
+                load16(Y1, p1);
+#pragma unroll
+                for (int k = 0; k < 16; k++)
+                    cv[k] = add_mod(mul_mod(p0[k], p1[k], md), cv[k], q);
+#else
                 load16(Y1, p1);
 #pragma unroll
                 for (int k = 0; k < 16; k++)
@@ -1670,6 +1755,7 @@
 #pragma unroll
                 for (int k = 0; k < 16; k++)
                     cv[k] = add_mod(cv[k], mul_mod(p0[k], p1[k], md), q);
+#endif
 #pragma unroll
                 for (int e = 0; e < 16; e++)
                     val[e] = sum_to_canon(acc1[e]);
@@ -1961,12 +2047,27 @@
                              tiles, nouter, r.nc, r.cls);
             return yes;
         }
+        std::atomic<uint64_t> g_pack_tail_mid{ 0 }, g_pack_inv_mid{ 0 };
+        inline bool pack_switch(const char *name)
+        {
+            const char *v = std::getenv(name);
+            return v && v[0] == '1';
+        }
+
         template <int D1, bool TWO>
-        hipError_t launch_src_p1t(const Tail2Args &g, const CompRun &r, unsigned nouter, hipStream_t st)
+        hipError_t launch_src_p1t(const Tail2Args &g, const CompRun &r, unsigned nouter, hipStream_t st, bool pack = false)
         {
             typedef Geo<D1> G;
             const size_t l1 = G::rA > 0 ? G::lds1_words * 8 : 8;
             const dim3 grid(G::TILES * nouter);
+            if constexpr (D1 == 8 && TWO)
+            {
+                if (pack)
+                {
+                    hipLaunchKernelGGL((ntt2_src_p1t<D1, 1, true, true, true>), grid, dim3(kThreads), l1, st, g, r.nc);
+                    return hipGetLastError();
+                }
+            }
             if (r.cls == 1 && TWO && !(g.x.src2_q >> 52))
                 hipLaunchKernelGGL((ntt2_src_p1t<D1, 1, TWO, TWO>), grid, dim3(kThreads), l1, st, g, r.nc);
             else if (r.cls == 1)
@@ -2112,9 +2213,13 @@
                 Tail2Args g = a;
                 g.f.comp0 = r.c0;
                 dim3 grid(G::TILES, r.nc, chunks);
-                if (src_resident(G::TILES, nouter, r))
-                {
-                    hipError_t e1 = launch_src_p1t<D1, true>(g, r, nouter, st);
+                const bool resident = src_resident(G::TILES, nouter, r);
+                const bool pack = D1 == 8 && r.cls == 1 && resident && !(a.x.src2_q >> 52) && pack_switch("SEALHIP_PACK_TAIL_MID");
+                if (pack)
+                    g_pack_tail_mid.fetch_add(1);
+                if (resident)
+                {
+                    hipError_t e1 = launch_src_p1t<D1, true>(g, r, nouter, st, pack);
                     if (e1 != hipSuccess)
                         return e1;
                 }
@@ -2127,7 +2232,14 @@
                 hipError_t e = hipGetLastError();
                 if (e != hipSuccess)
                     return e;
-                if (r.cls == 1)
+                if constexpr (D1 == 8)
+                {
+                    if (pack)
+                        hipLaunchKernelGGL((ntt2_tail2_p2<D1, 5>), grid, dim3(kThreads), kLds2Words * 8, st, g);
+                }
+                if (pack)
+                    ;
+                else if (r.cls == 1)
                     hipLaunchKernelGGL((ntt2_tail2_p2<D1, 1>), grid, dim3(kThreads), kLds2Words * 8, st, g);
                 else if (r.cls == 0)
                     hipLaunchKernelGGL((ntt2_tail2_p2<D1, 0>), grid, dim3(kThreads), kLds2Words * 8, st, g);
@@ -2188,7 +2300,19 @@
                     }
                 }
                 dim3 grid(G::TILES, r.nc, nouter);
-                if (r.cls == 1)
+                bool pack = false;
+                if constexpr (D1 == 8)
+                {
+                    pack = r.cls == 1 && pack_switch("SEALHIP_PACK_INV_MID");
+                    if (pack)
+                    {
+                        g_pack_inv_mid.fetch_add(1);
+                        hipLaunchKernelGGL((ntt2_inv_pa<D1, 5>), grid, dim3(kThreads), kLds2Words * 8, st, g);
+                    }
+                }
+                if (pack)
+                    ;
+                else if (r.cls == 1)
                     hipLaunchKernelGGL((ntt2_inv_pa<D1, 1>), grid, dim3(kThreads), kLds2Words * 8, st, g);
                 else if (r.cls == 0)
                     hipLaunchKernelGGL((ntt2_inv_pa<D1, 0>), grid, dim3(kThreads), kLds2Words * 8, st, g);
@@ -2202,7 +2326,14 @@
                 static std::atomic<long> inv_launches{ 0 };
                 if (skip_after >= 0 && inv_launches.fetch_add(1) >= skip_after)
                     return (hipError_t)hipSuccess;
-                if (r.cls == 1)
+                if constexpr (D1 == 8)
+                {
+                    if (pack)
+                        hipLaunchKernelGGL((ntt2_inv_pb<D1, 5>), grid, dim3(kThreads), G::lds1_words * 8, st, g);
+                }
+                if (pack)
+                    ;
+                else if (r.cls == 1)
                     hipLaunchKernelGGL((ntt2_inv_pb<D1, 1>), grid, dim3(kThreads), G::lds1_words * 8, st, g);
                 else if (r.cls == 0)
                     hipLaunchKernelGGL((ntt2_inv_pb<D1, 0>), grid, dim3(kThreads), G::lds1_words * 8, st, g);
@@ -2316,6 +2447,12 @@
     bool ntt2_supports(int log_n)
     {
         return log_n >= 13 && log_n <= 16;
+    }
+
+    void ntt2_pack_stats(uint64_t &tail_mid, uint64_t &inv_mid)
+    {
+        tail_mid = g_pack_tail_mid.load();
+        inv_mid = g_pack_inv_mid.load();
     }
 
     size_t ntt2_ring_words(const NttTables &t, const NttBatch &b)
```

New measurement: 10420, median of 6. About the same (+0.7%).
